# ZhangHH233/Retinal_OCT_Image_Segmentation_via_Deep_Learning

Measured on AMD Instinct MI355X. Metric: B-scans/sec (train fwd+bwd) at batch 32, 512x1024, higher is better.
Workload: dtype bf16; 1 GPU; SOTAS/Layers_Segment UNet(1,8,init_features=32) train step, 512x1024, batch 32/GPU (BASELINE configs[1]); global_batch=32, parallelism=dp1, hip_graph=False

## Files before the change

include/oct_hip.h:

```cpp
#ifndef OCT_HIP_H
#define OCT_HIP_H

#include <stddef.h>
#include <stdint.h>

#ifdef __cplusplus
extern "C" {
#endif

#define OCT_VERSION 220

#define OCT_DT_BF16 0
#define OCT_DT_F32 1

#define OCT_OK 0
#define OCT_IMG_SHIFT_ALL 2
#define OCT_E_INVALID (-22)
#define OCT_E_LAUNCH (-5)
#define OCT_E_NODEVICE (-19)

#define OCT_XF_NONE 0
#define OCT_XF_AFFINE_RELU 1
#define OCT_XF_AFFINE 2

#define OCT_IN_PLAIN 0
#define OCT_IN_S2D 1
#define OCT_OUT_PLAIN 0
#define OCT_OUT_D2S 1

#define OCT_PACK_CONV_FPROP 0
#define OCT_PACK_CONV_DGRAD 1
#define OCT_PACK_DECONV_FPROP 2
#define OCT_PACK_DECONV_DGRAD 3
#define OCT_PACK_1X1_DGRAD 4
#define OCT_PACK_1X1_FPROP 5
#define OCT_PACK_CONV3D_FPROP 6
#define OCT_PACK_CONV3D_DGRAD 7
#define OCT_PACK_DECONV3D_FPROP 8
#define OCT_PACK_DECONV3D_DGRAD 9

const char* oct_version_string(void);
int oct_version(void);
int oct_get_last_error(char* buf, size_t len);
int oct_device_count(void);

typedef struct OctConvDesc {
  int dtype;
  int n, h, w;
  int c0, c1;
  int cout;
  int taps;
  int xform0, xform1;
  int in_mode, out_mode;
  int split;
  int want_stats;
  int kh, kw;
  int depth;
  int out_img_mul, out_img_add;
} OctConvDesc;

typedef struct OctConvArgs {
  const void* x0; const void* x1;
  const float* scale0; const float* shift0;
  const float* scale1; const float* shift1;
  const void* wpacked;
  const float* bias;
  void* y0; void* y1;
  float* stat_partials;
} OctConvArgs;

int oct_conv_stat_blocks(const OctConvDesc* d);
size_t oct_packed_weight_elems(int rows, int taps, int kch);
int oct_pack_weights(int mode, int dtype, const float* w, void* wpacked, int cout, int cin, void* stream);
int oct_pack_weights_kk(int mode, int dtype, const float* w, void* wpacked, int cout, int cin, int kh, int kw,
                        void* stream);
int oct_pack_weights3d(int mode, int dtype, const float* w, void* wpacked, int cout, int cin, int kdi, void* stream);
#define OCT_PACK_BATCH_MAX 96
typedef struct OctPackJob {
  int mode, cout, cin, reserved;
  const float* w;
  void* wpacked;
} OctPackJob;
int oct_pack_weights_batch(int dtype, int count, const OctPackJob* jobs, void* stream);
int oct_conv_forward(const OctConvDesc* d, const OctConvArgs* a, void* stream);

typedef struct OctWgradDesc {
  int dtype;
  int n, h, w;
  int c0, c1;
  int cout;
  int taps;
  int xform0, xform1;
  int dy_mode;
  int kh, kw;
  int depth;
  int in_img_shift;
  int dy_img_mul, dy_img_add;
  int partials;
} OctWgradDesc;
typedef struct OctWgradArgs {
  const void* x0; const void* x1;
  const float* scale0; const float* shift0;
  const float* scale1; const float* shift1;
  const void* dy;
  float* dwp;
  float* dbias;
  const void* dy_y; const float* dy_coef; const float* dy_scale; const float* dy_shift;
  float* dbias_partials;
} OctWgradArgs;
int oct_conv_wgrad(const OctWgradDesc* d, const OctWgradArgs* a, void* stream);
int oct_conv_wgrad_partials(const OctWgradDesc* d);
int oct_reduce_bias_partials(const float* part, int nparts, int rows, int channels, float* dbias, int accumulate,
                             void* stream);
int oct_conv_wgrad_fused_apply_ok(const OctWgradDesc* d);
int oct_conv_wgrad_all_depth_taps_ok(const OctWgradDesc* d);
typedef struct OctConvBwdFusedArgs {
  const void* x;
  const float* scale; const float* shift;
  const float* mean; const float* invstd;
  const void* dy;
  const void* wpacked;
  void* dx;
  float* dwp;
  float* partials;
} OctConvBwdFusedArgs;
int oct_conv_backward_fused_ok(const OctWgradDesc* d);
int oct_conv_backward_fused_blocks(const OctWgradDesc* d);
int oct_conv_backward_fused(const OctWgradDesc* d, const OctConvBwdFusedArgs* a, void* stream);
int oct_unpack_wgrad(int mode, const float* dwp, float* grad, int cout, int cin, int accumulate, void* stream);
int oct_unpack_wgrad_kk(const float* dwp, float* grad, int cout, int cin, int kh, int kw, int accumulate, void* stream);
int oct_unpack_wgrad3d(int mode, const float* dwp, float* grad, int cout, int cin, int kdi, int accumulate, void* stream);
typedef struct OctUnpackJob {
  int mode, cout, cin, accumulate;
  int nparts, reserved;
  const float* dwp;
  float* grad;
} OctUnpackJob;
int oct_unpack_wgrad_batch(int count, const OctUnpackJob* jobs, void* stream);

int oct_bn_finalize(const float* partials, int nblocks, int c, double count,
                    const float* gamma, const float* beta, float eps, float momentum,
                    float* running_mean, float* running_var,
                    float* mean, float* invstd, float* scale, float* shift, const float* conv_bias,
                    void* stream);
int oct_bn_eval_coeffs(int c, const float* gamma, const float* beta, const float* running_mean,
                       const float* running_var, float eps, float* scale, float* shift,
                       const float* conv_bias, void* stream);

int oct_bn_relu_pool_fwd(int dtype, const void* y, const float* scale, const float* shift,
                         void* pooled, int n, int h, int w, int c, void* stream);
int oct_bn_relu_fwd(int dtype, const void* y, const float* scale, const float* shift,
                    void* out, size_t npix, int c, void* stream);

int oct_dact_bn_reduce(int dtype, const void* da, const void* dpool, const void* y,
                       const float* scale, const float* shift, const float* mean,
                       const float* invstd, void* g, float* partials, int n, int h, int w, int c,
                       void* stream);
int oct_dact_bn_reduce_blocks(int n, int h, int w, int c, int has_pool);
int oct_bn_bwd_apply_pool_ok(int dtype, int n, int h, int w, int c);
int oct_bn_bwd_apply_pool(int dtype, const void* da, const void* dpool, const void* y, const float* scale,
                          const float* shift, const float* coef, void* dy, int n, int h, int w, int c, void* stream);
int oct_bn_bwd_finalize(const float* partials, int nblocks, int c, double count,
                        const float* gamma, const float* mean, const float* invstd,
                        float* dgamma, float* dbeta, float* coef , int accumulate,
                        void* stream);
int oct_bn_bwd_apply(int dtype, void* g, const void* y, const float* coef, const float* scale,
                     const float* shift, size_t npix, int c, void* stream);
int oct_bn_bwd_apply_to(int dtype, void* dst, const void* g, const void* y, const float* coef, const float* scale,
                        const float* shift, size_t npix, int c, void* stream);
int oct_rowdot_ok(int c, int k);
int oct_rowdot_blocks(size_t npix, int c);
int oct_rowdot_fwd(int dtype, const void* x, const float* w, void* y, float* stats, size_t npix, int c, int k, void* stream);
int oct_rowdot_bwd_data(int dtype, const void* dy, const float* w, void* dx, size_t npix, int c, int k, void* stream);
int oct_rowdot_bwd_weight(int dtype, const void* dy, const void* x, float* dw, float* partials, size_t npix, int c, int k,
                          int accumulate, void* stream);
int oct_rowdot_bwd_weight_bias(int dtype, const void* dy, const void* x, float* dw, float* dbias, float* partials, size_t npix, int c,
                               int k, int accumulate, void* stream);

int oct_channel_sum(int dtype, const void* x, float* out, size_t npix, int c, int accumulate,
                    void* stream);

typedef struct OctHeadDesc {
  int dtype;
  int n, h, w;
  int feat;
  int classes;
} OctHeadDesc;
#define OCT_MAX_CLASSES 16
#define OCT_HEAD_LOSS_SLOTS (2 + 3 * OCT_MAX_CLASSES)
int oct_head_blocks(const OctHeadDesc* d);
int oct_head_forward(const OctHeadDesc* d, const void* y, const float* scale, const float* shift,
                     const float* w , const float* b, const int64_t* target,
                     float* probs, int64_t* argmax, float* logits ,
                     double* loss_partials, void* stream);
int oct_head_loss_finalize(const OctHeadDesc* d, const double* loss_partials, int nblocks,
                           float w_ce, float w_dice, float dice_eps, float* loss_out,
                           float* dice_coef, void* stream);
int oct_head_dlogits(const OctHeadDesc* d, const void* y, const float* scale, const float* shift,
                     const float* w, const float* b, const int64_t* target, const float* dice_coef,
                     float w_ce, const float* dprobs, void* dlogits, void* stream);

int oct_head_backward_fused(const OctHeadDesc* d, const void* y, const float* scale, const float* shift,
                            const float* mean, const float* invstd, const float* w, const float* b,
                            const int64_t* target, const float* dice_coef, float w_ce,
                            const float* dprobs, void* dlogits, void* da, float* partials,
                            float* dbias, float* dweight, double* loss_partials, void* stream);

#define OCT_SEG_NHWC 0
#define OCT_SEG_NCHW 1
int oct_seg_loss_blocks(size_t npix, int classes);
int oct_seg_loss_forward(const OctHeadDesc* d, int layout, const void* logits, const int64_t* target,
                         int64_t* argmax, double* loss_partials, void* stream);
int oct_seg_loss_backward(const OctHeadDesc* d, int layout, const void* logits, const int64_t* target,
                          const float* dice_coef, float w_ce, const float* dloss, void* dlogits,
                          double* loss_partials, void* stream);

int oct_seg_loss_weight_sum(const OctHeadDesc* d, const int64_t* target, const float* class_weight,
                            const float* pixel_weight, int has_ignore, int64_t ignore_index,
                            double* partials, double* wsum, void* stream);
int oct_seg_loss_forward_weighted(const OctHeadDesc* d, int layout, const void* logits,
                                  const int64_t* target, const float* class_weight,
                                  const float* pixel_weight, int has_ignore, int64_t ignore_index,
                                  double* loss_partials, void* stream);
int oct_seg_loss_backward_weighted(const OctHeadDesc* d, int layout, const void* logits,
                                   const int64_t* target, const float* class_weight,
                                   const float* pixel_weight, int has_ignore, int64_t ignore_index,
                                   const double* wsum, const float* dice_coef, float w_ce,
                                   const float* dloss, void* dlogits, double* loss_partials,
                                   void* stream);
int oct_seg_loss_finalize_weighted(const OctHeadDesc* d, const double* loss_partials, int nblocks,
                                   float w_ce, float w_dice, float dice_eps, float* loss_out,
                                   float* dice_coef, double* wsum_out, void* stream);

int oct_bce_loss_weight_sum(const OctHeadDesc* d, const uint8_t* target, const float* pixel_weight,
                            int has_ignore, int ignore_value, double* partials, double* wsum,
                            void* stream);
int oct_bce_loss_forward(const OctHeadDesc* d, int layout, const void* logits, const uint8_t* target,
                         const float* pos_weight, const float* pixel_weight, int has_ignore,
                         int ignore_value, int want_dice, float tau, uint8_t* mask,
                         double* loss_partials, void* stream);
int oct_bce_loss_backward(const OctHeadDesc* d, int layout, const void* logits, const uint8_t* target,
                          const float* pos_weight, const float* pixel_weight, int has_ignore,
                          int ignore_value, const double* wsum, const float* dice_coef, float w_bce,
                          const float* dloss, void* dlogits, double* loss_partials, void* stream);

int oct_nchw_to_nhwc(int dtype, const float* x, void* out, int n, int c, int h, int w, void* stream);
int oct_nhwc_to_nchw(int dtype, const void* x, float* out, int n, int c, int h, int w, void* stream);
int oct_sgd_step(float* p, const float* g, float* buf, size_t n, float lr, float momentum,
                 float weight_decay, float grad_scale, int first, void* stream);

int oct_adam_step(float* p, const float* g, float* m, float* v, size_t n, float lr, float beta1,
                  float beta2, float eps, float weight_decay, int decoupled, float step_size,
                  float inv_sqrt_bc2, float grad_scale, const float* dev_scale,
                  const uint8_t* decay_mask, void* stream);
int oct_sgd_step_scaled(float* p, const float* g, float* buf, size_t n, float lr, float momentum,
                        float weight_decay, float grad_scale, int first, const float* dev_scale,
                        const uint8_t* decay_mask, void* stream);
int oct_grad_norm_blocks(size_t n);
int oct_grad_norm(const float* g, size_t n, float grad_scale, float max_norm, double* partials,
                  float* out, void* stream);

#define OCT_ACT_NONE 0
#define OCT_ACT_RELU 1
#define OCT_ACT_SIGMOID 2
int oct_affine_act_fwd(int dtype, const void* y, const float* scale, const float* shift,
                       const void* res, int act, void* out, size_t npix, int c, void* stream);
int oct_affine_res_act_fwd(int dtype, const void* y, const float* scale, const float* shift, const void* res,
                           const float* res_shift, int act, void* out, size_t npix, int c, void* stream);
int oct_act_bwd(int dtype, const void* dout, const void* out, int act, void* dz, size_t n, void* stream);
int oct_maxpool_fwd(int dtype, const void* a, void* out, int n, int h, int w, int c, int k, void* stream);
int oct_maxpool_bwd(int dtype, const void* a, const void* dout, void* da, int n, int h, int w, int c,
                    int k, void* stream);
int oct_bilinear_up_fwd(int dtype, const void* x, void* out, int n, int h, int w, int c, int factor,
                        void* stream);
int oct_bilinear_up_bwd(int dtype, const void* dout, void* dx, int n, int h, int w, int c, int factor,
                        void* stream);
int oct_bilinear_resize_fwd(int dtype, const void* x, void* out, int n, int h, int w, int c, int ho, int wo,
                            void* stream);
int oct_bilinear_resize_bwd(int dtype, const void* dout, void* dx, int n, int h, int w, int c, int ho, int wo,
                            void* stream);
int oct_depth_to_space(int dtype, const void* in, const float* bias, void* out, int n, int h, int w,
                       int cout, int s, void* stream);
int oct_space_to_depth(int dtype, const void* in, void* out, int n, int h, int w, int cout, int s,
                       void* stream);
int oct_gate_fwd(int dtype, const void* x, const void* p, void* out, size_t npix, int c, void* stream);
int oct_gate_bwd(int dtype, const void* dout, const void* x, const void* p, void* dx, void* dp,
                 size_t npix, int c, void* stream);

int oct_affine_prelu_fwd(int dtype, const void* y, const float* scale, const float* shift, const float* alpha,
                         void* out, size_t npix, int c, void* stream);
int oct_affine_prelu_bwd(int dtype, const void* dout, const void* y, const float* scale, const float* shift,
                         const float* alpha, void* dz, float* dalpha, size_t npix, int c, void* stream);
int oct_prelu_bn_fused_ok(int dtype, int c);
int oct_dact_bn_reduce_prelu(int dtype, const void* da, const void* y, const float* scale, const float* shift, const float* alpha,
                             const float* mean, const float* invstd, float* partials, float* dalpha, int n, int h, int w, int c,
                             void* stream);
int oct_bn_bwd_apply_prelu_to(int dtype, void* dst, const void* da, const void* y, const float* coef, const float* scale,
                              const float* shift, const float* alpha, size_t npix, int c, void* stream);
int oct_maxpool_idx_fwd(int dtype, const void* a, void* out, int64_t* idx, int n, int h, int w, int c, int k, void* stream);
int oct_index_scatter(int dtype, const void* v, const int64_t* idx, void* out, int n, size_t npool, size_t plane, int c,
                      void* stream);
int oct_index_gather(int dtype, const void* x, const int64_t* idx, void* v, int n, size_t npool, size_t plane, int c,
                     void* stream);
int oct_maxpool_code_fwd(int dtype, const void* a, void* out, unsigned char* code, int n, int h, int w, int c, int k, void* stream);
int oct_window_scatter(int dtype, const void* v, const unsigned char* code, void* out, int n, int hp, int wp, int c, int k, void* stream);
int oct_window_gather(int dtype, const void* x, const unsigned char* code, void* v, int n, int hp, int wp, int c, int k, void* stream);

int oct_depth_pool_fwd(int dtype, const void* p2, void* out, size_t nslab, size_t m, void* stream);
int oct_depth_pool_bwd(int dtype, const void* p2, const void* dout, void* dp2, size_t nslab, size_t m, void* stream);

int oct_confusion_counts(const void* y_true, const void* y_pred, int elem, size_t n,
                         int64_t* out_i ,
                         double* out_f , void* stream);

int oct_class_confusion_counts(const void* y_true, const void* y_pred, int elem, size_t n, int classes,
                               int64_t* out , uint64_t* scratch ,
                               void* stream);

int oct_sqdiff_sum(const void* y_true, const void* y_pred, int elem, size_t n, double* out, void* stream);
int oct_column_absdiff_sum(const void* y_true, const void* y_pred, int elem, int unsigned_wrap, size_t rows,
                           size_t cols, double* out, void* stream);

#define OCT_EVAL_PRED_U8 0
#define OCT_EVAL_PRED_I64 1
#define OCT_EVAL_PRED_NHWC_BF16 2
#define OCT_EVAL_PRED_NHWC_F32 3
#define OCT_EVAL_PRED_NCHW_F32 4
#define OCT_EVAL_STATE_EXTRA 4
typedef struct {
  int images, h, w, classes;
  int target_elem;
  int pred_kind;
  int has_ignore;
  int64_t ignore_index;
} OctSegEvalDesc;
int oct_seg_eval_update(const OctSegEvalDesc* d, const void* target, const void* pred, int64_t* state, void* stream);

#ifdef __cplusplus
}
#endif
#endif
```

retinal_oct_image_segmentation_via_deep_learning_amd/_lib.py:

```python
from __future__ import annotations

import ctypes as C
import os
import subprocess
import threading

PKG_DIR = os.path.dirname(os.path.abspath(__file__))
LIB_PATH = os.environ.get("OCT_HIP_LIB") or os.path.join(PKG_DIR, "liboct_hip.so")
CSRC_DIR = os.path.join(PKG_DIR, "csrc")

DT_BF16, DT_F32 = 0, 1
XF_NONE, XF_AFFINE_RELU, XF_AFFINE = 0, 1, 2
IN_PLAIN, IN_S2D = 0, 1
IMG_SHIFT_ALL = 2
ACT_NONE, ACT_RELU, ACT_SIGMOID = 0, 1, 2
ACT_PRELU = 3
OUT_PLAIN, OUT_D2S = 0, 1
PACK_CONV_FPROP, PACK_CONV_DGRAD, PACK_DECONV_FPROP, PACK_DECONV_DGRAD, PACK_1X1_DGRAD, PACK_1X1_FPROP = range(6)
PACK_CONV3D_FPROP, PACK_CONV3D_DGRAD, PACK_DECONV3D_FPROP, PACK_DECONV3D_DGRAD = 6, 7, 8, 9
MAX_CLASSES = 16
HEAD_LOSS_SLOTS = 2 + 3 * MAX_CLASSES
SEG_NHWC, SEG_NCHW = 0, 1

c_void_p, c_int, c_size_t, c_float, c_double = C.c_void_p, C.c_int, C.c_size_t, C.c_float, C.c_double


class PackJob(C.Structure):
    _fields_ = [("mode", c_int), ("cout", c_int), ("cin", c_int), ("reserved", c_int), ("w", c_void_p),
                ("wpacked", c_void_p)]


class UnpackJob(C.Structure):
    _fields_ = [("mode", c_int), ("cout", c_int), ("cin", c_int), ("accumulate", c_int), ("nparts", c_int),
                ("reserved", c_int), ("dwp", c_void_p), ("grad", c_void_p)]


PACK_BATCH_MAX = 96


class ConvDesc(C.Structure):
    _fields_ = [(k, c_int) for k in (
        "dtype", "n", "h", "w", "c0", "c1", "cout", "taps", "xform0", "xform1", "in_mode", "out_mode",
        "split", "want_stats", "kh", "kw", "depth", "out_img_mul", "out_img_add")]


class ConvArgs(C.Structure):
    _fields_ = [(k, c_void_p) for k in (
        "x0", "x1", "scale0", "shift0", "scale1", "shift1", "wpacked", "bias", "y0", "y1", "stat_partials")]


class WgradDesc(C.Structure):
    _fields_ = [(k, c_int) for k in (
        "dtype", "n", "h", "w", "c0", "c1", "cout", "taps", "xform0", "xform1", "dy_mode", "kh", "kw", "depth",
        "in_img_shift", "dy_img_mul", "dy_img_add", "partials")]


class WgradArgs(C.Structure):
    _fields_ = [(k, c_void_p) for k in ("x0", "x1", "scale0", "shift0", "scale1", "shift1", "dy", "dwp", "dbias",
                                                "dy_y", "dy_coef", "dy_scale", "dy_shift", "dbias_partials")]


class ConvBwdFusedArgs(C.Structure):
    _fields_ = [(k, c_void_p) for k in ("x", "scale", "shift", "mean", "invstd", "dy", "wpacked", "dx", "dwp", "partials")]


class HeadDesc(C.Structure):
    _fields_ = [(k, c_int) for k in ("dtype", "n", "h", "w", "feat", "classes")]


class SegEvalDesc(C.Structure):
    _fields_ = [(k, c_int) for k in ("images", "h", "w", "classes", "target_elem", "pred_kind", "has_ignore")] + \
               [("ignore_index", C.c_int64)]


EVAL_PRED_U8, EVAL_PRED_I64, EVAL_PRED_NHWC_BF16, EVAL_PRED_NHWC_F32, EVAL_PRED_NCHW_F32 = range(5)
EVAL_STATE_EXTRA = 4


SIGNATURES = {
    "oct_version_string": (C.c_char_p, []),
    "oct_version": (c_int, []),
    "oct_get_last_error": (c_int, [C.c_char_p, c_size_t]),
    "oct_device_count": (c_int, []),
    "oct_conv_stat_blocks": (c_int, [C.POINTER(ConvDesc)]),
    "oct_packed_weight_elems": (c_size_t, [c_int, c_int, c_int]),
    "oct_pack_weights": (c_int, [c_int, c_int, c_void_p, c_void_p, c_int, c_int, c_void_p]),
    "oct_pack_weights3d": (c_int, [c_int, c_int, c_void_p, c_void_p, c_int, c_int, c_int, c_void_p]),
    "oct_unpack_wgrad3d": (c_int, [c_int, c_void_p, c_void_p, c_int, c_int, c_int, c_int, c_void_p]),
    "oct_depth_pool_fwd": (c_int, [c_int, c_void_p, c_void_p, c_size_t, c_size_t, c_void_p]),
    "oct_depth_pool_bwd": (c_int, [c_int, c_void_p, c_void_p, c_void_p, c_size_t, c_size_t, c_void_p]),
    "oct_pack_weights_kk": (c_int, [c_int, c_int, c_void_p, c_void_p, c_int, c_int, c_int, c_int, c_void_p]),
    "oct_unpack_wgrad_kk": (c_int, [c_void_p, c_void_p, c_int, c_int, c_int, c_int, c_int, c_void_p]),
    "oct_affine_prelu_fwd": (c_int, [c_int, c_void_p, c_void_p, c_void_p, c_void_p, c_void_p, c_size_t, c_int, c_void_p]),
    "oct_affine_prelu_bwd": (c_int, [c_int, c_void_p, c_void_p, c_void_p, c_void_p, c_void_p, c_void_p, c_void_p, c_size_t,
                                     c_int, c_void_p]),
    "oct_maxpool_idx_fwd": (c_int, [c_int, c_void_p, c_void_p, c_void_p, c_int, c_int, c_int, c_int, c_int, c_void_p]),
    "oct_index_scatter": (c_int, [c_int, c_void_p, c_void_p, c_void_p, c_int, c_size_t, c_size_t, c_int, c_void_p]),
    "oct_index_gather": (c_int, [c_int, c_void_p, c_void_p, c_void_p, c_int, c_size_t, c_size_t, c_int, c_void_p]),
    "oct_prelu_bn_fused_ok": (c_int, [c_int, c_int]),
    "oct_dact_bn_reduce_prelu": (c_int, [c_int, c_void_p, c_void_p, c_void_p, c_void_p, c_void_p, c_void_p, c_void_p, c_void_p, c_void_p,
                                         c_int, c_int, c_int, c_int, c_void_p]),
    "oct_bn_bwd_apply_prelu_to": (c_int, [c_int, c_void_p, c_void_p, c_void_p, c_void_p, c_void_p, c_void_p, c_void_p, c_size_t, c_int,
                                          c_void_p]),
    "oct_maxpool_code_fwd": (c_int, [c_int, c_void_p, c_void_p, c_void_p, c_int, c_int, c_int, c_int, c_int, c_void_p]),
    "oct_window_scatter": (c_int, [c_int, c_void_p, c_void_p, c_void_p, c_int, c_int, c_int, c_int, c_int, c_void_p]),
    "oct_window_gather": (c_int, [c_int, c_void_p, c_void_p, c_void_p, c_int, c_int, c_int, c_int, c_int, c_void_p]),
    "oct_pack_weights_batch": (c_int, [c_int, c_int, C.POINTER(PackJob), c_void_p]),
    "oct_conv_forward": (c_int, [C.POINTER(ConvDesc), C.POINTER(ConvArgs), c_void_p]),
    "oct_conv_wgrad": (c_int, [C.POINTER(WgradDesc), C.POINTER(WgradArgs), c_void_p]),
    "oct_conv_wgrad_fused_apply_ok": (c_int, [C.POINTER(WgradDesc)]),
    "oct_conv_wgrad_all_depth_taps_ok": (c_int, [C.POINTER(WgradDesc)]),
    "oct_conv_backward_fused_ok": (c_int, [C.POINTER(WgradDesc)]),
    "oct_conv_backward_fused_blocks": (c_int, [C.POINTER(WgradDesc)]),
    "oct_conv_backward_fused": (c_int, [C.POINTER(WgradDesc), C.POINTER(ConvBwdFusedArgs), c_void_p]),
    "oct_conv_wgrad_partials": (c_int, [C.POINTER(WgradDesc)]),
    "oct_reduce_bias_partials": (c_int, [c_void_p, c_int, c_int, c_int, c_void_p, c_int, c_void_p]),
    "oct_unpack_wgrad": (c_int, [c_int, c_void_p, c_void_p, c_int, c_int, c_int, c_void_p]),
    "oct_unpack_wgrad_batch": (c_int, [c_int, C.POINTER(UnpackJob), c_void_p]),
    "oct_bn_finalize": (c_int, [c_void_p, c_int, c_int, c_double, c_void_p, c_void_p, c_float, c_float,
                                c_void_p, c_void_p, c_void_p, c_void_p, c_void_p, c_void_p, c_void_p, c_void_p]),
    "oct_bn_eval_coeffs": (c_int, [c_int, c_void_p, c_void_p, c_void_p, c_void_p, c_float, c_void_p, c_void_p,
                                   c_void_p, c_void_p]),
    "oct_bn_relu_pool_fwd": (c_int, [c_int, c_void_p, c_void_p, c_void_p, c_void_p, c_int, c_int, c_int, c_int,
                                     c_void_p]),
    "oct_bn_relu_fwd": (c_int, [c_int, c_void_p, c_void_p, c_void_p, c_void_p, c_size_t, c_int, c_void_p]),
    "oct_dact_bn_reduce": (c_int, [c_int, c_void_p, c_void_p, c_void_p, c_void_p, c_void_p, c_void_p, c_void_p,
                                   c_void_p, c_void_p, c_int, c_int, c_int, c_int, c_void_p]),
    "oct_dact_bn_reduce_blocks": (c_int, [c_int, c_int, c_int, c_int, c_int]),
    "oct_bn_bwd_apply_pool_ok": (c_int, [c_int, c_int, c_int, c_int, c_int]),
    "oct_bn_bwd_apply_pool": (c_int, [c_int, c_void_p, c_void_p, c_void_p, c_void_p, c_void_p, c_void_p, c_void_p,
                                      c_int, c_int, c_int, c_int, c_void_p]),
    "oct_bn_bwd_finalize": (c_int, [c_void_p, c_int, c_int, c_double, c_void_p, c_void_p, c_void_p, c_void_p,
                                    c_void_p, c_void_p, c_int, c_void_p]),
    "oct_bn_bwd_apply": (c_int, [c_int, c_void_p, c_void_p, c_void_p, c_void_p, c_void_p, c_size_t, c_int,
                                 c_void_p]),
    "oct_bn_bwd_apply_to": (c_int, [c_int, c_void_p, c_void_p, c_void_p, c_void_p, c_void_p, c_void_p, c_size_t, c_int,
                                    c_void_p]),
    "oct_channel_sum": (c_int, [c_int, c_void_p, c_void_p, c_size_t, c_int, c_int, c_void_p]),
    "oct_rowdot_ok": (c_int, [c_int, c_int]),
    "oct_rowdot_blocks": (c_int, [c_size_t, c_int]),
    "oct_rowdot_fwd": (c_int, [c_int, c_void_p, c_void_p, c_void_p, c_void_p, c_size_t, c_int, c_int, c_void_p]),
    "oct_rowdot_bwd_data": (c_int, [c_int, c_void_p, c_void_p, c_void_p, c_size_t, c_int, c_int, c_void_p]),
    "oct_rowdot_bwd_weight": (c_int, [c_int, c_void_p, c_void_p, c_void_p, c_void_p, c_size_t, c_int, c_int, c_int, c_void_p]),
    "oct_rowdot_bwd_weight_bias": (c_int, [c_int, c_void_p, c_void_p, c_void_p, c_void_p, c_void_p, c_size_t, c_int, c_int, c_int,
                                           c_void_p]),
    "oct_head_blocks": (c_int, [C.POINTER(HeadDesc)]),
    "oct_head_forward": (c_int, [C.POINTER(HeadDesc), c_void_p, c_void_p, c_void_p, c_void_p, c_void_p, c_void_p,
                                 c_void_p, c_void_p, c_void_p, c_void_p, c_void_p]),
    "oct_head_loss_finalize": (c_int, [C.POINTER(HeadDesc), c_void_p, c_int, c_float, c_float, c_float, c_void_p,
                                       c_void_p, c_void_p]),
    "oct_head_dlogits": (c_int, [C.POINTER(HeadDesc), c_void_p, c_void_p, c_void_p, c_void_p, c_void_p, c_void_p,
                                 c_void_p, c_float, c_void_p, c_void_p, c_void_p]),
    "oct_head_backward_fused": (c_int, [C.POINTER(HeadDesc), c_void_p, c_void_p, c_void_p, c_void_p, c_void_p, c_void_p,
                                        c_void_p, c_void_p, c_void_p, c_float, c_void_p, c_void_p, c_void_p, c_void_p,
                                        c_void_p, c_void_p, c_void_p, c_void_p]),
    "oct_seg_loss_blocks": (c_int, [c_size_t, c_int]),
    "oct_seg_loss_forward": (c_int, [C.POINTER(HeadDesc), c_int, c_void_p, c_void_p, c_void_p, c_void_p, c_void_p]),
    "oct_seg_loss_backward": (c_int, [C.POINTER(HeadDesc), c_int, c_void_p, c_void_p, c_void_p, c_float, c_void_p, c_void_p,
                                      c_void_p, c_void_p]),
    "oct_seg_loss_weight_sum": (c_int, [C.POINTER(HeadDesc), c_void_p, c_void_p, c_void_p, c_int, C.c_int64, c_void_p, c_void_p,
                                        c_void_p]),
    "oct_seg_loss_forward_weighted": (c_int, [C.POINTER(HeadDesc), c_int, c_void_p, c_void_p, c_void_p, c_void_p, c_int,
                                              C.c_int64, c_void_p, c_void_p]),
    "oct_seg_loss_backward_weighted": (c_int, [C.POINTER(HeadDesc), c_int, c_void_p, c_void_p, c_void_p, c_void_p, c_int,
                                               C.c_int64, c_void_p, c_void_p, c_float, c_void_p, c_void_p, c_void_p, c_void_p]),
    "oct_seg_loss_finalize_weighted": (c_int, [C.POINTER(HeadDesc), c_void_p, c_int, c_float, c_float, c_float, c_void_p,
                                               c_void_p, c_void_p, c_void_p]),
    "oct_bce_loss_weight_sum": (c_int, [C.POINTER(HeadDesc), c_void_p, c_void_p, c_int, c_int, c_void_p, c_void_p, c_void_p]),
    "oct_bce_loss_forward": (c_int, [C.POINTER(HeadDesc), c_int, c_void_p, c_void_p, c_void_p, c_void_p, c_int, c_int, c_int,
                                     c_float, c_void_p, c_void_p, c_void_p]),
    "oct_bce_loss_backward": (c_int, [C.POINTER(HeadDesc), c_int, c_void_p, c_void_p, c_void_p, c_void_p, c_int, c_int,
                                      c_void_p, c_void_p, c_float, c_void_p, c_void_p, c_void_p, c_void_p]),
    "oct_nchw_to_nhwc": (c_int, [c_int, c_void_p, c_void_p, c_int, c_int, c_int, c_int, c_void_p]),
    "oct_nhwc_to_nchw": (c_int, [c_int, c_void_p, c_void_p, c_int, c_int, c_int, c_int, c_void_p]),
    "oct_sgd_step": (c_int, [c_void_p, c_void_p, c_void_p, c_size_t, c_float, c_float, c_float, c_float, c_int,
                             c_void_p]),
    "oct_adam_step": (c_int, [c_void_p, c_void_p, c_void_p, c_void_p, c_size_t, c_float, c_float, c_float, c_float, c_float,
                              c_int, c_float, c_float, c_float, c_void_p, c_void_p, c_void_p]),
    "oct_sgd_step_scaled": (c_int, [c_void_p, c_void_p, c_void_p, c_size_t, c_float, c_float, c_float, c_float, c_int,
                                    c_void_p, c_void_p, c_void_p]),
    "oct_grad_norm_blocks": (c_int, [c_size_t]),
    "oct_grad_norm": (c_int, [c_void_p, c_size_t, c_float, c_float, c_void_p, c_void_p, c_void_p]),
    "oct_affine_act_fwd": (c_int, [c_int, c_void_p, c_void_p, c_void_p, c_void_p, c_int, c_void_p, c_size_t, c_int,
                                   c_void_p]),
    "oct_affine_res_act_fwd": (c_int, [c_int, c_void_p, c_void_p, c_void_p, c_void_p, c_void_p, c_int, c_void_p, c_size_t,
                                       c_int, c_void_p]),
    "oct_act_bwd": (c_int, [c_int, c_void_p, c_void_p, c_int, c_void_p, c_size_t, c_void_p]),
    "oct_maxpool_fwd": (c_int, [c_int, c_void_p, c_void_p, c_int, c_int, c_int, c_int, c_int, c_void_p]),
    "oct_maxpool_bwd": (c_int, [c_int, c_void_p, c_void_p, c_void_p, c_int, c_int, c_int, c_int, c_int, c_void_p]),
    "oct_bilinear_up_fwd": (c_int, [c_int, c_void_p, c_void_p, c_int, c_int, c_int, c_int, c_int, c_void_p]),
    "oct_bilinear_up_bwd": (c_int, [c_int, c_void_p, c_void_p, c_int, c_int, c_int, c_int, c_int, c_void_p]),
    "oct_bilinear_resize_fwd": (c_int, [c_int, c_void_p, c_void_p, c_int, c_int, c_int, c_int, c_int, c_int, c_void_p]),
    "oct_bilinear_resize_bwd": (c_int, [c_int, c_void_p, c_void_p, c_int, c_int, c_int, c_int, c_int, c_int, c_void_p]),
    "oct_depth_to_space": (c_int, [c_int, c_void_p, c_void_p, c_void_p, c_int, c_int, c_int, c_int, c_int, c_void_p]),
    "oct_space_to_depth": (c_int, [c_int, c_void_p, c_void_p, c_int, c_int, c_int, c_int, c_int, c_void_p]),
    "oct_gate_fwd": (c_int, [c_int, c_void_p, c_void_p, c_void_p, c_size_t, c_int, c_void_p]),
    "oct_gate_bwd": (c_int, [c_int, c_void_p, c_void_p, c_void_p, c_void_p, c_void_p, c_size_t, c_int, c_void_p]),
    "oct_confusion_counts": (c_int, [c_void_p, c_void_p, c_int, c_size_t, c_void_p, c_void_p, c_void_p]),
    "oct_class_confusion_counts": (c_int, [c_void_p, c_void_p, c_int, c_size_t, c_int, c_void_p, c_void_p, c_void_p]),
    "oct_sqdiff_sum": (c_int, [c_void_p, c_void_p, c_int, c_size_t, c_void_p, c_void_p]),
    "oct_column_absdiff_sum": (c_int, [c_void_p, c_void_p, c_int, c_int, c_size_t, c_size_t, c_void_p, c_void_p]),
    "oct_seg_eval_update": (c_int, [C.POINTER(SegEvalDesc), c_void_p, c_void_p, c_void_p, c_void_p]),
}

_lib = None
_lock = threading.Lock()
param_generation = [0]


class OctError(RuntimeError):
    pass


def build(verbose: bool = False) -> str:
    cmd = ["make", "-C", CSRC_DIR, "-j8"]
    res = subprocess.run(cmd, capture_output=True, text=True)
    if verbose or res.returncode != 0:
        print(res.stdout[-4000:])
        print(res.stderr[-4000:])
    if res.returncode != 0:
        raise OctError("building liboct_hip.so failed (see output above)")
    return LIB_PATH


def lib():
    global _lib
    if _lib is not None:
        return _lib
    with _lock:
        if _lib is None:
            if not os.path.exists(LIB_PATH):
                raise OctError(
                    f"{LIB_PATH} is missing: the HIP extension has not been built "
                    "(run `python __graft_entry__.py` or `make -C .../csrc`). There is no CPU fallback.")
            handle = C.CDLL(LIB_PATH)
            for name, (res, args) in SIGNATURES.items():
                fn = getattr(handle, name)
                fn.restype = res
                fn.argtypes = args
            _lib = handle
    return _lib


def last_error() -> str:
    buf = C.create_string_buffer(512)
    lib().oct_get_last_error(buf, 512)
    return buf.value.decode("utf-8", "replace")


def check(rc: int, what: str = "") -> None:
    if rc != 0:
        raise OctError(f"{what or 'liboct_hip'} failed with code {rc}: {last_error()}")


def ptr(t) -> int | None:
    return None if t is None else t.data_ptr()
```

retinal_oct_image_segmentation_via_deep_learning_amd/csrc/common.h:

```cpp
#pragma once
#include <hip/hip_runtime.h>
#include <stdint.h>
#include <stddef.h>
#include "../../include/oct_hip.h"

typedef __bf16 bf16_t;
typedef float f32x16 __attribute__((ext_vector_type(16)));
typedef float f32x4 __attribute__((ext_vector_type(4)));
typedef __bf16 bf16x8 __attribute__((ext_vector_type(8)));
typedef __bf16 bf16x4 __attribute__((ext_vector_type(4)));

void oct_set_error(const char* fmt, ...);
#define OCT_CHECK(cond, ...)            \
  do {                                  \
    if (!(cond)) {                      \
      oct_set_error(__VA_ARGS__);       \
      return OCT_E_INVALID;             \
    }                                   \
  } while (0)
int oct_check_launch(const char* what);
int oct_lds_optin(const void* kernel, int bytes);

enum ConvPath { CONV_FIRST, CONV_ROLL3D, CONV_GEMM1, CONV_IGEMM2, CONV_IGEMM };
struct ConvPlan {
  ConvPath path;
  int kernel;
  int grid;
  int stat_rows;
  int th, nt, nblk, nitems, per_wg, interleave;
  bool wres;
};
bool first_plan(const OctConvDesc* d, ConvPlan* pl);
bool roll3d_plan(const OctConvDesc* d, ConvPlan* pl);
bool igemm2_plan(const OctConvDesc* d, ConvPlan* pl);
bool gemm1_plan(const OctConvDesc* d, ConvPlan* pl);
void igemm_plan(const OctConvDesc* d, ConvPlan* pl);
int launch_first(const ConvPlan& pl, const OctConvDesc* d, const OctConvArgs* a, hipStream_t s);
int launch_roll3d(const ConvPlan& pl, const OctConvDesc* d, const OctConvArgs* a, hipStream_t s);
int launch_igemm2(const ConvPlan& pl, const OctConvDesc* d, const OctConvArgs* a, hipStream_t s);
int launch_gemm1(const ConvPlan& pl, const OctConvDesc* d, const OctConvArgs* a, hipStream_t s);
int launch_igemm(const ConvPlan& pl, const OctConvDesc* d, const OctConvArgs* a, hipStream_t s);
bool igemm2_fused_plan(const OctWgradDesc* d, ConvPlan* pl);
int launch_igemm2_fused(const ConvPlan& pl, const OctWgradDesc* d, const OctConvBwdFusedArgs* a, hipStream_t s);

enum WgradPath { WGRAD_FIRST, WGRAD_W2, WGRAD_GENERIC };
struct WgradPlan {
  WgradPath path;
  int kernel;
  int cb, ib, th;
  int grid;
  int slabs;
  bool all_depth_taps;
};
bool first_wgrad_plan(const OctWgradDesc* d, bool dbias, bool dy_coef, WgradPlan* pl);
bool wgrad2_plan(const OctWgradDesc* d, WgradPlan* pl);
void wgrad_plan(const OctWgradDesc* d, WgradPlan* pl);
int launch_first_wgrad(const WgradPlan& pl, const OctWgradDesc* d, const OctWgradArgs* a, hipStream_t s);
int launch_wgrad2(const WgradPlan& pl, const OctWgradDesc* d, const OctWgradArgs* a, hipStream_t s);
int launch_wgrad(const WgradPlan& pl, const OctWgradDesc* d, const OctWgradArgs* a, hipStream_t s);

__device__ __forceinline__ float xf_floor(int xf) { return xf == 2 ? -__builtin_inff() : 0.f; }
__device__ __forceinline__ float to_f32(float v) { return v; }
__device__ __forceinline__ float to_f32(bf16_t v) { return (float)v; }
template <typename T> __device__ __forceinline__ T from_f32(float v);
template <> __device__ __forceinline__ float from_f32<float>(float v) { return v; }
template <> __device__ __forceinline__ bf16_t from_f32<bf16_t>(float v) { return (bf16_t)v; }

template <typename T, int V> struct alignas((sizeof(T) * V) > 16 ? 16 : (sizeof(T) * V)) VecT { T v[V]; };

template <typename T, int V>
__device__ __forceinline__ void load_vec(const T* p, float (&out)[V]) {
  VecT<T, V> t = *reinterpret_cast<const VecT<T, V>*>(p);
#pragma unroll
  for (int i = 0; i < V; ++i) out[i] = to_f32(t.v[i]);
}
template <typename T, int V>
__device__ __forceinline__ void store_vec(T* p, const float (&in)[V]) {
  VecT<T, V> t;
#pragma unroll
  for (int i = 0; i < V; ++i) t.v[i] = from_f32<T>(in[i]);
  *reinterpret_cast<VecT<T, V>*>(p) = t;
}

template <typename T, int V>
__device__ __forceinline__ void load_vec_nt(const T* p, float (&out)[V]) {
  typedef unsigned int nt_u4 __attribute__((ext_vector_type(4)));
  constexpr int NQ = (sizeof(T) * V) / 16;
  static_assert(NQ >= 1 && (sizeof(T) * V) % 16 == 0, "16-B multiples only");
  VecT<T, V> t;
  nt_u4* q = reinterpret_cast<nt_u4*>(&t);
#pragma unroll
  for (int i = 0; i < NQ; ++i) q[i] = __builtin_nontemporal_load(reinterpret_cast<const nt_u4*>(p) + i);
#pragma unroll
  for (int i = 0; i < V; ++i) out[i] = to_f32(t.v[i]);
}
template <typename T, int V>
__device__ __forceinline__ void store_vec_nt(T* p, const float (&in)[V]) {
  typedef unsigned int nt_u4 __attribute__((ext_vector_type(4)));
  constexpr int NQ = (sizeof(T) * V) / 16;
  static_assert(NQ >= 1 && (sizeof(T) * V) % 16 == 0, "16-B multiples only");
  VecT<T, V> t;
#pragma unroll
  for (int i = 0; i < V; ++i) t.v[i] = from_f32<T>(in[i]);
  const nt_u4* q = reinterpret_cast<const nt_u4*>(&t);
#pragma unroll
  for (int i = 0; i < NQ; ++i) __builtin_nontemporal_store(q[i], reinterpret_cast<nt_u4*>(p) + i);
}

template <typename T> struct Mma;
template <> struct Mma<bf16_t> {
  typedef bf16x8 Frag;
  static __device__ __forceinline__ void mma(f32x16& acc, const Frag& a, const Frag& b) {
    acc = __builtin_amdgcn_mfma_f32_32x32x16_bf16(a, b, acc, 0, 0, 0);
  }
  static __device__ __forceinline__ void mma0(f32x16& acc, const Frag& a, const Frag& b) {
    const f32x16 z = {0.f, 0.f, 0.f, 0.f, 0.f, 0.f, 0.f, 0.f, 0.f, 0.f, 0.f, 0.f, 0.f, 0.f, 0.f, 0.f};
    acc = __builtin_amdgcn_mfma_f32_32x32x16_bf16(a, b, z, 0, 0, 0);
  }
  template <int S>
  static __device__ __forceinline__ void mma16(f32x16& acc, const Frag& a, const Frag& b) {
    f32x4 v = {acc[4 * S], acc[4 * S + 1], acc[4 * S + 2], acc[4 * S + 3]};
    v = __builtin_amdgcn_mfma_f32_16x16x32_bf16(a, b, v, 0, 0, 0);
    acc[4 * S] = v[0]; acc[4 * S + 1] = v[1]; acc[4 * S + 2] = v[2]; acc[4 * S + 3] = v[3];
  }
  static __device__ __forceinline__ Frag load(const void* p) { return *reinterpret_cast<const Frag*>(p); }
  static __device__ __forceinline__ Frag zero() {
    Frag f;
#pragma unroll
    for (int i = 0; i < 8; ++i) f[i] = (bf16_t)0.0f;
    return f;
  }
  static __device__ __forceinline__ void set(Frag& f, int j, bf16_t v) { f[j] = v; }
};
struct F32Frag { f32x4 lo, hi; };
template <> struct Mma<float> {
  typedef F32Frag Frag;
  static __device__ __forceinline__ void mma(f32x16& acc, const Frag& a, const Frag& b) {
#pragma unroll
    for (int j = 0; j < 4; ++j) acc = __builtin_amdgcn_mfma_f32_32x32x2f32(a.lo[j], b.lo[j], acc, 0, 0, 0);
#pragma unroll
    for (int j = 0; j < 4; ++j) acc = __builtin_amdgcn_mfma_f32_32x32x2f32(a.hi[j], b.hi[j], acc, 0, 0, 0);
  }
  static __device__ __forceinline__ Frag load(const void* p) {
    Frag f;
    f.lo = reinterpret_cast<const f32x4*>(p)[0];
    f.hi = reinterpret_cast<const f32x4*>(p)[1];
    return f;
  }
  static __device__ __forceinline__ Frag zero() {
    Frag f;
    f.lo = f32x4{0, 0, 0, 0};
    f.hi = f32x4{0, 0, 0, 0};
    return f;
  }
  static __device__ __forceinline__ void set(Frag& f, int j, float v) {
    if (j < 4) f.lo[j] = v; else f.hi[j - 4] = v;
  }
};

typedef short s16x4 __attribute__((ext_vector_type(4)));
__device__ __forceinline__ bf16x8 tr_frag(const unsigned char* base_lo) {
  typedef __attribute__((address_space(3))) s16x4 lds_s16x4;
  const s16x4 a = __builtin_amdgcn_ds_read_tr16_b64_v4i16((lds_s16x4*)(base_lo));
  const s16x4 b = __builtin_amdgcn_ds_read_tr16_b64_v4i16((lds_s16x4*)(base_lo + 4 * 64));
  typedef short s16x8 __attribute__((ext_vector_type(8)));
  const s16x8 v = {a[0], a[1], a[2], a[3], b[0], b[1], b[2], b[3]};
  return __builtin_bit_cast(bf16x8, v);
}

__device__ __forceinline__ bf16x8 tr_frag2(const unsigned char* first, const unsigned char* second) {
  typedef __attribute__((address_space(3))) s16x4 lds_s16x4;
  const s16x4 a = __builtin_amdgcn_ds_read_tr16_b64_v4i16((lds_s16x4*)(first));
  const s16x4 b = __builtin_amdgcn_ds_read_tr16_b64_v4i16((lds_s16x4*)(second));
  typedef short s16x8 __attribute__((ext_vector_type(8)));
  const s16x8 v = {a[0], a[1], a[2], a[3], b[0], b[1], b[2], b[3]};
  return __builtin_bit_cast(bf16x8, v);
}

__device__ __forceinline__ float wave_sum(float v) {
#pragma unroll
  for (int o = 32; o > 0; o >>= 1) v += __shfl_xor(v, o);
  return v;
}
__device__ __forceinline__ double wave_sum(double v) {
#pragma unroll
  for (int o = 32; o > 0; o >>= 1) v += __shfl_xor(v, o);
  return v;
}

__device__ __forceinline__ float reduce32_scatter16(const float (&v)[16], int lane) {
  float t8[8], t4[4], t2[2];
  bool b = (lane & 16) != 0;
#pragma unroll
  for (int k = 0; k < 8; ++k) {
    float keep = b ? v[k + 8] : v[k];
    float send = b ? v[k] : v[k + 8];
    t8[k] = keep + __shfl_xor(send, 16);
  }
  b = (lane & 8) != 0;
#pragma unroll
  for (int k = 0; k < 4; ++k) {
    float keep = b ? t8[k + 4] : t8[k];
    float send = b ? t8[k] : t8[k + 4];
    t4[k] = keep + __shfl_xor(send, 8);
  }
  b = (lane & 4) != 0;
#pragma unroll
  for (int k = 0; k < 2; ++k) {
    float keep = b ? t4[k + 2] : t4[k];
    float send = b ? t4[k] : t4[k + 2];
    t2[k] = keep + __shfl_xor(send, 4);
  }
  b = (lane & 2) != 0;
  float keep = b ? t2[1] : t2[0];
  float send = b ? t2[0] : t2[1];
  float s = keep + __shfl_xor(send, 2);
  s += __shfl_xor(s, 1);
  return s;
}
__device__ __forceinline__ float reduce16_scatter8(const float (&v)[8], int lane) {
  float t4[4], t2[2];
  bool b = (lane & 8) != 0;
#pragma unroll
  for (int k = 0; k < 4; ++k) {
    float keep = b ? v[k + 4] : v[k];
    float send = b ? v[k] : v[k + 4];
    t4[k] = keep + __shfl_xor(send, 8);
  }
  b = (lane & 4) != 0;
#pragma unroll
  for (int k = 0; k < 2; ++k) {
    float keep = b ? t4[k + 2] : t4[k];
    float send = b ? t4[k] : t4[k + 2];
    t2[k] = keep + __shfl_xor(send, 4);
  }
  b = (lane & 2) != 0;
  float keep = b ? t2[1] : t2[0];
  float send = b ? t2[0] : t2[1];
  float s = keep + __shfl_xor(send, 2);
  s += __shfl_xor(s, 1);
  return s;
}
__device__ __forceinline__ int scatter16_reg_of_lane(int lane) {
  return ((lane >> 4) & 1) * 8 + ((lane >> 3) & 1) * 4 + ((lane >> 2) & 1) * 2 + ((lane >> 1) & 1);
}

static inline hipStream_t as_stream(void* s) { return reinterpret_cast<hipStream_t>(s); }
static inline int ceil_div(int a, int b) { return (a + b - 1) / b; }
```

retinal_oct_image_segmentation_via_deep_learning_amd/csrc/conv_dispatch.hip:

```cpp
#include "common.h"
#include <stdlib.h>

static bool v2_enabled() {
  static const bool on = [] { const char* e = getenv("OCT_DISABLE_V2"); return !(e && e[0] == '1'); }();
  return on;
}

static ConvPlan plan_conv_forward(const OctConvDesc* d) {
  ConvPlan pl = {};
  if (v2_enabled()) {
    if (first_plan(d, &pl) || roll3d_plan(d, &pl)) return pl;
    if (igemm2_plan(d, &pl)) {
      gemm1_plan(d, &pl);
      return pl;
    }
  }
  igemm_plan(d, &pl);
  return pl;
}

static WgradPlan plan_conv_wgrad(const OctWgradDesc* d, bool dbias, bool dy_coef) {
  WgradPlan pl = {};
  if (v2_enabled() && (first_wgrad_plan(d, dbias, dy_coef, &pl) || wgrad2_plan(d, &pl))) return pl;
  wgrad_plan(d, &pl);
  return pl;
}

static bool kernel_size(int taps, int kh_in, int kw_in, int* kh, int* kw) {
  if (kh_in == 0 && kw_in == 0) {
    if (taps == 9) { *kh = 3; *kw = 3; return true; }
    if (taps == 1) { *kh = 1; *kw = 1; return true; }
    return false;
  }
  *kh = kh_in; *kw = kw_in;
  return taps == kh_in * kw_in && ((kh_in == 3 && kw_in == 3) || (kh_in == 1 && kw_in == 1) || (kh_in == 7 && kw_in == 3));
}

extern "C" int oct_conv_stat_blocks(const OctConvDesc* d) { return d ? plan_conv_forward(d).stat_rows : 0; }

extern "C" int oct_conv_forward(const OctConvDesc* d, const OctConvArgs* a, void* stream) {
  OCT_CHECK(d && a, "oct_conv_forward: null descriptor");
  OCT_CHECK(d->dtype == OCT_DT_BF16 || d->dtype == OCT_DT_F32, "oct_conv_forward: bad dtype %d", d->dtype);
  int kh = 0, kw = 0;
  OCT_CHECK(kernel_size(d->taps, d->kh, d->kw, &kh, &kw),
            "oct_conv_forward: kernel must be 3x3 (taps 9), 1x1 (taps 1) or 7x3 (taps 21, kh=7, kw=3); got taps=%d kh=%d kw=%d",
            d->taps, d->kh, d->kw);
  OCT_CHECK(kh != 7 || (d->in_mode == OCT_IN_PLAIN && d->out_mode == OCT_OUT_PLAIN), "oct_conv_forward: 7x3 runs plain -> plain");
  OCT_CHECK(d->depth >= 0 && (d->depth == 0 || (d->n % d->depth) == 0), "oct_conv_forward: n=%d is not a whole number of depth-%d volumes", d->n, d->depth);
  OCT_CHECK(d->depth == 0 || kh != 7, "oct_conv_forward: depth taps go with the 3x3 (3x3x3) and 1x1 (2x2x2 transposed) kernels");
  OCT_CHECK(d->out_img_mul == 0 || d->out_mode == OCT_OUT_D2S, "oct_conv_forward: the output image map belongs to D2S");
  OCT_CHECK(d->n > 0 && d->h > 0 && d->w > 0 && d->c0 > 0 && d->c1 >= 0 && d->cout > 0,
            "oct_conv_forward: bad shape n=%d h=%d w=%d c0=%d c1=%d cout=%d", d->n, d->h, d->w, d->c0, d->c1, d->cout);
  OCT_CHECK(a->x0 && a->wpacked && a->y0, "oct_conv_forward: null tensor");
  OCT_CHECK(d->c1 == 0 || a->x1, "oct_conv_forward: c1 > 0 but x1 is null");
  OCT_CHECK(!(d->in_mode == OCT_IN_S2D && d->c1 != 0), "oct_conv_forward: S2D input takes one source");
  OCT_CHECK(!(d->out_mode == OCT_OUT_D2S && (d->cout & 3)), "oct_conv_forward: D2S needs cout %% 4 == 0");
  OCT_CHECK(d->split >= 0 && d->split < d->cout, "oct_conv_forward: bad split %d", d->split);
  OCT_CHECK(d->split == 0 || a->y1, "oct_conv_forward: split without y1");
  OCT_CHECK(d->xform0 >= 0 && d->xform0 <= OCT_XF_AFFINE && d->xform1 >= 0 && d->xform1 <= OCT_XF_AFFINE, "oct_conv_forward: bad xform");
  OCT_CHECK(!(d->xform0 && (!a->scale0 || !a->shift0)), "oct_conv_forward: xform0 without scale/shift");
  OCT_CHECK(!(d->xform1 && (!a->scale1 || !a->shift1)), "oct_conv_forward: xform1 without scale/shift");
  OCT_CHECK(!(d->want_stats && !a->stat_partials), "oct_conv_forward: want_stats without buffer");
  OCT_CHECK((size_t)d->n * d->h * d->w < (1u << 31), "oct_conv_forward: too many pixels");
  const ConvPlan pl = plan_conv_forward(d);
  hipStream_t s = as_stream(stream);
  switch (pl.path) {
    case CONV_FIRST: return launch_first(pl, d, a, s);
    case CONV_ROLL3D: return launch_roll3d(pl, d, a, s);
    case CONV_GEMM1: return launch_gemm1(pl, d, a, s);
    case CONV_IGEMM2: return launch_igemm2(pl, d, a, s);
    default: return launch_igemm(pl, d, a, s);
  }
}

extern "C" int oct_conv_wgrad_partials(const OctWgradDesc* d) {
  int kh, kw;
  if (!d || !kernel_size(d->taps, d->kh, d->kw, &kh, &kw)) return 0;
  return plan_conv_wgrad(d, false, false).slabs;
}

extern "C" int oct_conv_wgrad_fused_apply_ok(const OctWgradDesc* d) {
  return d && d->kh != 7 && plan_conv_wgrad(d, false, false).path == WGRAD_FIRST;
}

extern "C" int oct_conv_wgrad_all_depth_taps_ok(const OctWgradDesc* d) {
  if (!d) return 0;
  const WgradPlan pl = plan_conv_wgrad(d, false, false);
  return pl.path == WGRAD_FIRST && pl.all_depth_taps;
}

extern "C" int oct_conv_wgrad(const OctWgradDesc* d, const OctWgradArgs* a, void* stream) {
  OCT_CHECK(d && a, "oct_conv_wgrad: null descriptor");
  OCT_CHECK(d->dtype == OCT_DT_BF16 || d->dtype == OCT_DT_F32, "oct_conv_wgrad: bad dtype %d", d->dtype);
  int kh = 0, kw = 0;
  OCT_CHECK(kernel_size(d->taps, d->kh, d->kw, &kh, &kw),
            "oct_conv_wgrad: kernel must be 3x3 (taps 9), 1x1 (taps 1) or 7x3 (taps 21, kh=7, kw=3); got taps=%d kh=%d kw=%d",
            d->taps, d->kh, d->kw);
  OCT_CHECK(kh != 7 || (d->dy_mode == OCT_IN_PLAIN && !a->dy_coef), "oct_conv_wgrad: 7x3 takes a plain dY");
  OCT_CHECK(d->depth >= 0 && (d->depth == 0 || ((d->n % d->depth) == 0 && kh != 7)), "oct_conv_wgrad: bad depth %d for n=%d", d->depth, d->n);
  OCT_CHECK(((d->in_img_shift >= -1 && d->in_img_shift <= 1) || d->in_img_shift == OCT_IMG_SHIFT_ALL) && (d->in_img_shift == 0 || d->depth > 0),
            "oct_conv_wgrad: in_img_shift needs depth > 0");
  OCT_CHECK(d->in_img_shift != OCT_IMG_SHIFT_ALL || oct_conv_wgrad_all_depth_taps_ok(d),
            "oct_conv_wgrad: OCT_IMG_SHIFT_ALL is not available for this descriptor (oct_conv_wgrad_all_depth_taps_ok)");
  OCT_CHECK(d->dy_img_mul == 0 || d->dy_mode == OCT_IN_S2D, "oct_conv_wgrad: the dY image map belongs to S2D");
  OCT_CHECK(d->n > 0 && d->h > 0 && d->w > 0 && d->c0 > 0 && d->c1 >= 0 && d->cout > 0, "oct_conv_wgrad: bad shape");
  OCT_CHECK(a->x0 && a->dy && a->dwp, "oct_conv_wgrad: null tensor");
  OCT_CHECK(d->c1 == 0 || a->x1, "oct_conv_wgrad: c1 > 0 but x1 is null");
  OCT_CHECK(!(d->dy_mode == OCT_IN_S2D && (d->cout & 3)), "oct_conv_wgrad: S2D dy needs cout %% 4 == 0");
  OCT_CHECK(d->xform0 >= 0 && d->xform0 <= OCT_XF_AFFINE && d->xform1 >= 0 && d->xform1 <= OCT_XF_AFFINE, "oct_conv_wgrad: bad xform");
  OCT_CHECK(!(d->xform0 && (!a->scale0 || !a->shift0)), "oct_conv_wgrad: xform0 without scale/shift");
  OCT_CHECK(!(d->xform1 && (!a->scale1 || !a->shift1)), "oct_conv_wgrad: xform1 without scale/shift");
  OCT_CHECK(!d->partials || !a->dbias || a->dbias_partials, "oct_conv_wgrad: partials mode with a bias gradient needs dbias_partials");
  const WgradPlan pl = plan_conv_wgrad(d, a->dbias != nullptr, a->dy_coef != nullptr);
  OCT_CHECK(!a->dy_coef || pl.path == WGRAD_FIRST, "oct_conv_wgrad: the fused BN-backward apply is only implemented for the 1->F first layer in bf16");
  OCT_CHECK(!a->dy_coef || (a->dy_y && a->dy_scale && a->dy_shift), "oct_conv_wgrad: fused apply needs y, scale, shift");
  if (d->partials) {
    const int slabs = plan_conv_wgrad(d, false, false).slabs;
    OCT_CHECK(pl.slabs == slabs, "oct_conv_wgrad: with these arguments the launch writes %d partial slabs, oct_conv_wgrad_partials "
              "answered %d (first layer with a bias gradient?)", pl.slabs, slabs);
  }
  hipStream_t s = as_stream(stream);
  switch (pl.path) {
    case WGRAD_FIRST: return launch_first_wgrad(pl, d, a, s);
    case WGRAD_W2: return launch_wgrad2(pl, d, a, s);
    default: return launch_wgrad(pl, d, a, s);
  }
}

static bool plan_conv_backward_fused(const OctWgradDesc* d, ConvPlan* pl) {
  return d && v2_enabled() && igemm2_fused_plan(d, pl);
}

extern "C" int oct_conv_backward_fused_ok(const OctWgradDesc* d) {
  ConvPlan pl;
  return plan_conv_backward_fused(d, &pl) ? 1 : 0;
}

extern "C" int oct_conv_backward_fused_blocks(const OctWgradDesc* d) {
  ConvPlan pl;
  return plan_conv_backward_fused(d, &pl) ? pl.stat_rows : 0;
}

extern "C" int oct_conv_backward_fused(const OctWgradDesc* d, const OctConvBwdFusedArgs* a, void* stream) {
  OCT_CHECK(d && a, "oct_conv_backward_fused: null descriptor");
  ConvPlan pl;
  OCT_CHECK(plan_conv_backward_fused(d, &pl),
            "oct_conv_backward_fused: not available for this descriptor (oct_conv_backward_fused_ok): bf16, 2-D, 3x3, c0 = cout = 32, "
            "c1 = 0, BN + ReLU on load, w %% 32 == 0, h %% 8 == 0, atomics mode");
  OCT_CHECK(a->x && a->scale && a->shift && a->mean && a->invstd && a->dy && a->wpacked && a->dx && a->dwp && a->partials,
            "oct_conv_backward_fused: null tensor");
  return launch_igemm2_fused(pl, d, a, as_stream(stream));
}
```

retinal_oct_image_segmentation_via_deep_learning_amd/csrc/igemm2.hip:

```cpp
#include "common.h"
#include <stdlib.h>

struct Igemm2Params {
  const bf16_t* x0; const bf16_t* x1;
  const float* sc0; const float* sh0; const float* sc1; const float* sh1;
  const bf16_t* wp;
  bf16_t* y0; bf16_t* y1; float* stats; const float* bias;
  int n, h, w, c0, c1, cout, split, xf0, xf1, in_mode, out_mode;
  int tiles_x, tiles_y, nblk, nitems, per_wg, nch, nk16;
  int interleave;
  int depth, nchc, oimg_mul, oimg_add;
  const bf16_t* fx; const float* fsc; const float* fsh; const float* fmean; const float* finvstd;
  float* dwp; float* bnpart;
  unsigned long long* trace;
};

typedef unsigned int u32x4 __attribute__((ext_vector_type(4)));

#ifdef OCT_TRACE
#define TRACE(slot, idx)                                                                              \
  do {                                                                                                \
    if (p.trace && blockIdx.x == 0 && (threadIdx.x & 63) == 0 && (idx) < 256)                          \
      p.trace[(slot) * 256 + (idx)] = __builtin_amdgcn_s_memtime();                                    \
  } while (0)
static unsigned long long* g_trace = nullptr;
extern "C" void oct_debug_set_trace(void* buf) { g_trace = (unsigned long long*)buf; }
#else
#define TRACE(slot, idx) do {} while (0)
#endif

__device__ __forceinline__ unsigned pack_bf16x2(float a, float b) {
  typedef __bf16 bf16x2 __attribute__((ext_vector_type(2)));
  bf16x2 v;
  v[0] = (bf16_t)a;
  v[1] = (bf16_t)b;
  return __builtin_bit_cast(unsigned, v);
}
__device__ __forceinline__ float bf16lo(unsigned u) { return __uint_as_float(u << 16); }
__device__ __forceinline__ float bf16hi(unsigned u) { return __uint_as_float(u & 0xffff0000u); }

template <int TAPS, int NF, bool WRES> constexpr bool ig2_m16() { return TAPS != 1 && !WRES && NF == 2; }
template <int TAPS, int NF, bool WRES, bool DMA> constexpr int ig2_pixb() { return DMA ? 64 : (ig2_m16<TAPS, NF, WRES>() ? 96 : 80); }

__device__ __attribute__((aligned(16))) unsigned int g_zero16[4];

template <int TAPS, int WM, int WN, int MF, int NF, bool WRES, bool STATS, bool RAGGED = false, bool D3 = false, bool DMA = false,
          bool WLDS = false, bool FUSE = false>
__global__ void __launch_bounds__(512) igemm2_kernel(const Igemm2Params p) {
  static_assert(WM * WN == 4, "four MFMA waves");
  static_assert(!FUSE || (TAPS == 9 && WM == 4 && NF == 1 && WRES && !STATS && !RAGGED && !D3 && !DMA && !WLDS),
                "fused backward: resident weights, 32 -> 32 channels, whole tiles, 2-D");
  static_assert(!DMA || (!WRES && !STATS && !RAGGED && !D3), "DMA staging: streamed weights, whole tiles, 2-D, no BatchNorm sums");
  static_assert(!WLDS || (TAPS == 9 && !WRES && !D3 && !DMA && WN * NF == 1), "LDS-resident weights: 3x3, one 32-channel block");
  constexpr int TH = WM * MF, TW = 32;
  constexpr int HALO = (TAPS != 1) ? 1 : 0;
  constexpr int HALO_Y = (TAPS == 21) ? 3 : HALO;
  constexpr int LH = TH + 2 * HALO_Y, LW = TW + 2 * HALO;
  constexpr int NPIX = LH * LW;
  constexpr int NSLOT = (NPIX + 63) / 64;
  constexpr int PIXB = ig2_pixb<TAPS, NF, WRES, DMA>();
  constexpr int BUFB = DMA ? NSLOT * 4096 : NPIX * PIXB;
  constexpr int NBUF = DMA ? (TAPS != 1 ? 3 : 6) : 2;
  constexpr int NT = WN * NF * 32;
  constexpr int KSTEPS = TAPS * 2;
  constexpr bool M16 = ig2_m16<TAPS, NF, WRES>();
  typedef Mma<bf16_t> M;
  typedef M::Frag Frag;

  extern __shared__ __attribute__((aligned(16))) unsigned char smem[];
  unsigned char* const buf0 = smem;
  float* const wg_stats = reinterpret_cast<float*>(smem + NBUF * BUFB);

  const int tid = threadIdx.x, lane = tid & 63;
  const int wave = __builtin_amdgcn_readfirstlane(tid >> 6);
  const bool s2d = TAPS == 1 && p.in_mode == OCT_IN_S2D;
  const bool d2s = TAPS == 1 && p.out_mode == OCT_OUT_D2S;
  int t_first, nbi_first, nitems_wg, tstep;
  if (p.interleave) {
    if ((int)blockIdx.x >= p.nitems / p.nblk) return;
    t_first = blockIdx.x; nbi_first = 0; tstep = gridDim.x;
    nitems_wg = ((p.nitems / p.nblk - (int)blockIdx.x + (int)gridDim.x - 1) / (int)gridDim.x) * p.nblk;
  } else {
    const int it0 = blockIdx.x * p.per_wg;
    const int it1 = min(it0 + p.per_wg, p.nitems);
    if (it0 >= it1) return;
    t_first = it0 / p.nblk; nbi_first = it0 - t_first * p.nblk; tstep = 1; nitems_wg = it1 - it0;
  }
  const int sx = tstep % p.tiles_x, sy = (tstep / p.tiles_x) % p.tiles_y, simg = tstep / (p.tiles_x * p.tiles_y);
  const int nstage = nitems_wg * p.nch;
  const int nstage_pad = (nstage + 3) / 4 * 4;

  constexpr int SXF_N = WLDS ? 64 : 1024, OSCR_SLOTS = WLDS ? 1 : 2, SBIAS_N = WLDS ? 0 : 1024, WLDS_BYTES = WLDS ? 2 * 18 * 1024 : 0;
  float* const sxf = reinterpret_cast<float*>(smem + NBUF * BUFB) + (2 * WM * 2 * NT + 4);
  unsigned char* const oscr = smem + NBUF * BUFB + (2 * WM * 2 * NT + 4) * 4 + 2 * SXF_N * 4;
  static_assert((NBUF * BUFB + (2 * WM * 2 * NT + 4) * 4) % 16 == 0, "scratch must stay 16-B aligned");
  unsigned char* const wlds = oscr + OSCR_SLOTS * 4 * 32 * 80;
  float* const sbias = reinterpret_cast<float*>(wlds + WLDS_BYTES);
  float* const wgacc = sbias + SBIAS_N;
  constexpr int XTB = TH * TW * 64;
  unsigned char* const fxt = reinterpret_cast<unsigned char*>(sbias + SBIAS_N);
  unsigned char* const fxr = fxt + 2 * XTB;
  if (STATS && !WRES) {
    for (int i = tid; i < 2 * p.cout; i += 512) wgacc[i] = 0.f;
  }
  {
    const int kx = s2d ? p.c0 : p.c0 + p.c1;
    for (int i = tid; i < kx; i += 512) {
      const bool first = i < p.c0;
      const bool xf = first ? (p.xf0 != 0) : (p.xf1 != 0);
      sxf[i] = xf ? (first ? p.sc0[i] : p.sc1[i - p.c0]) : 1.f;
      sxf[kx + i] = xf ? (first ? p.sh0[i] : p.sh1[i - p.c0]) : 0.f;
    }
    if (d2s && p.bias)
      for (int i = tid; i < (p.cout >> 2); i += 512) sbias[i] = p.bias[i];
    if constexpr (FUSE) {
      if (tid < 32) *reinterpret_cast<f32x4*>(sxf + SXF_N + 4 * tid) = f32x4{p.fsc[tid], p.fsh[tid], p.fmean[tid], p.finvstd[tid]};
    }
    if constexpr (WLDS) {
      const u32x4* src = reinterpret_cast<const u32x4*>(p.wp);
      u32x4* dst = reinterpret_cast<u32x4*>(wlds);
      for (int i = tid; i < TAPS * p.nk16 * 64; i += 512) dst[i] = src[i];
    }
  }
  __syncthreads();

  if constexpr (DMA) {
   if (wave >= 4) {
    const int ptid = tid - 256, grp = ptid & 3, pbase = ptid >> 2;
    constexpr int KSH = M16 ? 1 : 2;
    const unsigned cs2 = 2u * (unsigned)p.c0;
    unsigned goff[NSLOT], code[NSLOT];
#pragma unroll
    for (int i = 0; i < NSLOT; ++i) {
      const int pix = pbase + 64 * i;
      const int ly = pix / LW, lx = pix - ly * LW;
      const int relp = s2d ? (2 * ly) * (2 * p.w) + 2 * lx : ly * p.w + lx;
      goff[i] = (unsigned)relp * cs2 + (unsigned)((grp ^ ((lx >> KSH) & 3)) * 16);
      unsigned c = pix >= NPIX ? 16u : 0u;
      if (HALO) c |= (ly < HALO_Y ? 1u : 0u) | (lx == 0 ? 4u : 0u) | (ly >= LH - HALO_Y ? 2u : 0u) | (lx == LW - 1 ? 8u : 0u);
      code[i] = c;
    }
    const int last = nstage - 1;
    int i_sidx = 0, i_ch = 0, i_nbi, i_txi, i_tyi, i_img;
    {
      int t = t_first;
      i_nbi = nbi_first;
      i_txi = t % p.tiles_x; t /= p.tiles_x;
      i_tyi = t % p.tiles_y; i_img = t / p.tiles_y;
    }
    typedef __attribute__((address_space(3))) void lds_void;
    typedef const __attribute__((address_space(1))) void gl_void;
    const unsigned char* const zsrc = reinterpret_cast<const unsigned char*>(g_zero16);
    const int pw = wave - 4;
    auto dma = [&](unsigned char* buf) {
      const int ch = i_ch, txi = i_txi, tyi = i_tyi, img = i_img;
      if (i_sidx < last) {
        ++i_sidx;
        if (++i_ch == p.nch) {
          i_ch = 0;
          if (++i_nbi == p.nblk) {
            i_nbi = 0;
            i_txi += sx; if (i_txi >= p.tiles_x) { i_txi -= p.tiles_x; ++i_tyi; }
            i_tyi += sy; if (i_tyi >= p.tiles_y) { i_tyi -= p.tiles_y; ++i_img; }
            i_img += simg;
          }
        }
      }
      const unsigned edge = 16u | (tyi == 0 ? 1u : 0u) | (tyi == p.tiles_y - 1 ? 2u : 0u) | (txi == 0 ? 4u : 0u) |
                            (txi == p.tiles_x - 1 ? 8u : 0u);
      const bf16_t* base;
      if (s2d) {
        const int dydx = (ch * 32) / p.c0;
        const int cc = ch * 32 - dydx * p.c0;
        const size_t o2 = ((size_t)img * (2 * p.h) + 2 * tyi * TH + (dydx >> 1)) * (size_t)(2 * p.w) + 2 * txi * TW + (dydx & 1);
        base = p.x0 + o2 * p.c0 + cc;
      } else {
        base = p.x0 + (((size_t)img * p.h + tyi * TH) * p.w + txi * TW) * p.c0 + ch * 32;
      }
      const unsigned char* const hb = reinterpret_cast<const unsigned char*>(base) - (size_t)(HALO_Y * p.w + HALO) * cs2;
      unsigned char* const dst = buf + pw * 1024;
#pragma unroll
      for (int i = 0; i < NSLOT; ++i) {
        const bool ok = (code[i] & edge) == 0;
        const unsigned char* src = ok ? hb + goff[i] : zsrc;
        __builtin_amdgcn_global_load_lds((gl_void*)src, (lds_void*)(dst + i * 4096), 16, 0, 0);
        constexpr int DMA_SLEEP = 6;
        if (TAPS != 1 && i + 1 < NSLOT) __builtin_amdgcn_s_sleep(NF == 2 ? DMA_SLEEP : DMA_SLEEP / 3);
      }
    };
    constexpr int NW = NSLOT * (NBUF - 2);
    static_assert(NW < 64, "vmcnt is a 6-bit counter");
    auto stage_barrier = [&]() {
      __builtin_amdgcn_s_waitcnt((NW & 15) | ((NW >> 4) << 14) | (7 << 4) | (15 << 8));
      asm volatile("s_barrier" ::: "memory");
    };
    int wb = 0;
#pragma unroll
    for (int j = 0; j < NBUF - 1; ++j) { dma(buf0 + wb * BUFB); wb = wb + 1 == NBUF ? 0 : wb + 1; }
    stage_barrier();
    for (int s0 = 0; s0 < nstage_pad; ++s0) {
      dma(buf0 + wb * BUFB); wb = wb + 1 == NBUF ? 0 : wb + 1;
      stage_barrier();
    }
    return;
   }
  } else
  if (wave >= 4) {
    const int ptid = tid - 256, grp = ptid & 3, pbase = ptid >> 2;
    constexpr int D = 2;
    u32x4 R[D][NSLOT];
    unsigned vmask[D];
    int relp[NSLOT];
    unsigned code[NSLOT];
#pragma unroll
    for (int i = 0; i < NSLOT; ++i) {
      const int pix = pbase + 64 * i;
      const int ly = pix / LW, lx = pix - ly * LW;
      relp[i] = s2d ? (2 * ly) * (2 * p.w) + 2 * lx : ly * p.w + lx;
      const int ylast = p.h - (p.tiles_y - 1) * TH + HALO_Y, xlast = p.w - (p.tiles_x - 1) * TW + HALO;
      unsigned c = pix >= NPIX ? 16u : 0u;
      if (HALO) c |= (ly < HALO_Y ? 1u : 0u) | (lx == 0 ? 4u : 0u);
      c |= (ly >= ylast ? 2u : 0u) | (lx >= xlast ? 8u : 0u);
      code[i] = c;
    }
    constexpr int XS = FUSE ? TH * TW * 4 / 256 : 1;
    u32x4 XR[D][XS];
    unsigned xrel[XS];
    float fs[8], fb[8];
    const unsigned char* x_next = nullptr;
    if constexpr (FUSE) {
#pragma unroll
      for (int i = 0; i < XS; ++i) {
        const int pix = pbase + 64 * i;
        xrel[i] = (unsigned)((pix >> 5) * p.w + (pix & 31)) * 64u;
      }
#pragma unroll
      for (int j = 0; j < 8; ++j) { fs[j] = p.fsc[grp * 8 + j]; fb[j] = p.fsh[grp * 8 + j]; }
      asm volatile("s_waitcnt vmcnt(0)" ::: "memory");
#pragma unroll
      for (int j = 0; j < 8; ++j) asm volatile("" : "+v"(fs[j]), "+v"(fb[j]));
    }
    const int last = nstage - 1;
    int i_sidx = 0, i_ch = 0, i_nbi, i_txi, i_tyi, i_img, c_sidx = 0, c_ch = 0;
    {
      int t = t_first;
      i_nbi = nbi_first;
      i_txi = t % p.tiles_x; t /= p.tiles_x;
      i_tyi = t % p.tiles_y; i_img = t / p.tiles_y;
    }
    struct IssueSt { const unsigned char* hb; unsigned edge, cs2, safe; bool zok; };
    auto issue_begin = [&]() -> IssueSt {
      const int ch = i_ch, txi = i_txi, tyi = i_tyi, img = i_img;
      if (i_sidx < last) {
        ++i_sidx;
        if (++i_ch == p.nch) {
          i_ch = 0;
          if (++i_nbi == p.nblk) {
            i_nbi = 0;
            i_txi += sx; if (i_txi >= p.tiles_x) { i_txi -= p.tiles_x; ++i_tyi; }
            i_tyi += sy; if (i_tyi >= p.tiles_y) { i_tyi -= p.tiles_y; ++i_img; }
            i_img += simg;
          }
        }
      }
      const unsigned edge = 16u | (tyi == 0 ? 1u : 0u) | (tyi == p.tiles_y - 1 ? 2u : 0u) | (txi == 0 ? 4u : 0u) |
                            (txi == p.tiles_x - 1 ? 8u : 0u);
      int chc = ch, srcimg = img;
      bool zok = true;
      if (D3 && !s2d) {
        const int kdi = ch / p.nchc;
        chc = ch - kdi * p.nchc;
        const int dz = img % p.depth + kdi - 1;
        zok = dz >= 0 && dz < p.depth;
        srcimg = zok ? img + kdi - 1 : img;
      }
      const size_t origin = ((size_t)srcimg * p.h + tyi * TH) * p.w + txi * TW;
      if constexpr (FUSE) x_next = reinterpret_cast<const unsigned char*>(p.fx + origin * 32 + grp * 8);
      const bool second = !s2d && chc * 32 >= p.c0;
      const int cs = second ? p.c1 : p.c0;
      const bf16_t* base;
      if (s2d) {
        int dydx = (ch * 32) / p.c0;
        const int cc = ch * 32 - dydx * p.c0;
        int img2 = img;
        if (D3) { img2 = 2 * img + (dydx >> 2); dydx &= 3; }
        const size_t o2 = ((size_t)img2 * (2 * p.h) + 2 * tyi * TH + (dydx >> 1)) * (size_t)(2 * p.w) + 2 * txi * TW + (dydx & 1);
        base = p.x0 + o2 * p.c0 + cc + grp * 8;
      } else {
        base = (second ? p.x1 + origin * p.c1 + (chc * 32 - p.c0) : p.x0 + origin * p.c0 + chc * 32) + grp * 8;
      }
      const unsigned cs2 = 2u * (unsigned)cs, safe = (unsigned)(HALO_Y * p.w + HALO) * cs2;
      const unsigned char* const hb = reinterpret_cast<const unsigned char*>(base) - safe;
      return IssueSt{hb, edge, cs2, safe, zok};
    };
    auto issue_slot = [&](const IssueSt& st, int i, u32x4& r, unsigned& vm) {
      const bool ok = (!D3 || st.zok) && (code[i] & st.edge) == 0;
      r = *reinterpret_cast<const u32x4*>(st.hb + (ok ? __umul24((unsigned)relp[i], st.cs2) : st.safe));
      vm |= ok ? (1u << i) : 0u;
    };
    auto issue = [&](u32x4 (&Rr)[NSLOT], unsigned& vm) {
      const IssueSt st = issue_begin();
      vm = 0;
#pragma unroll
      for (int i = 0; i < NSLOT; ++i) issue_slot(st, i, Rr[i], vm);
    };
    struct CommitSt { float s[8], b[8]; float flo; bool xf; };
    auto commit_begin = [&](bool always) -> CommitSt {
      CommitSt st;
      const int ch = c_ch;
      if (c_sidx < last) { ++c_sidx; if (++c_ch == p.nch) c_ch = 0; }
      const int chc = (D3 && !s2d) ? ch % p.nchc : ch;
      int cg = chc * 32 + grp * 8;
      if (s2d) cg -= ((ch * 32) / p.c0) * p.c0;
      const bool first = s2d || chc * 32 < p.c0;
      st.xf = first ? (p.xf0 != 0) : (p.xf1 != 0);
      st.flo = xf_floor(first ? p.xf0 : p.xf1);
      if (st.xf || always) {
        const int kx = s2d ? p.c0 : p.c0 + p.c1;
        const f32x4 s0 = *reinterpret_cast<const f32x4*>(sxf + cg), s1 = *reinterpret_cast<const f32x4*>(sxf + cg + 4);
        const f32x4 b0 = *reinterpret_cast<const f32x4*>(sxf + kx + cg), b1 = *reinterpret_cast<const f32x4*>(sxf + kx + cg + 4);
#pragma unroll
        for (int j = 0; j < 4; ++j) { st.s[j] = s0[j]; st.s[4 + j] = s1[j]; st.b[j] = b0[j]; st.b[4 + j] = b1[j]; }
      }
      return st;
    };
    auto commit_slot = [&](const CommitSt& st, unsigned char* buf, int i, const u32x4& r, unsigned vm, bool always) {
      const int pix = pbase + 64 * i;
      if (pix < NPIX) {
        u32x4 v = r;
#ifndef ABL_NO_XFORM
        if (always || st.xf)
#else
        if (st.xf && p.n == 12345)
#endif
        {
#pragma unroll
          for (int j = 0; j < 4; ++j) {
            const float lo = fmaxf(fmaf(bf16lo(v[j]), st.s[2 * j], st.b[2 * j]), st.flo);
            const float hi = fmaxf(fmaf(bf16hi(v[j]), st.s[2 * j + 1], st.b[2 * j + 1]), st.flo);
            v[j] = pack_bf16x2(lo, hi);
          }
        }
        const bool live = (vm & (1u << i)) != 0;
#pragma unroll
        for (int j = 0; j < 4; ++j) v[j] = live ? v[j] : 0u;
        *reinterpret_cast<u32x4*>(buf + pix * PIXB + grp * 16) = v;
      }
    };
    auto commit = [&](unsigned char* buf, const u32x4 (&Rr)[NSLOT], unsigned vm) {
      const CommitSt st = commit_begin(false);
#pragma unroll
      for (int i = 0; i < NSLOT; ++i) commit_slot(st, buf, i, Rr[i], vm, false);
    };
    auto issue_x = [&](u32x4 (&Xr)[XS]) {
#pragma unroll
      for (int i = 0; i < XS; ++i) Xr[i] = *reinterpret_cast<const u32x4*>(x_next + xrel[i]);
    };
    auto commit_x = [&](int bi, const u32x4 (&Xr)[XS]) {
#pragma unroll
      for (int i = 0; i < XS; ++i) {
        const int off = bi * XTB + (pbase + 64 * i) * 64 + grp * 16;
        u32x4 v = Xr[i];
        *reinterpret_cast<u32x4*>(fxr + off) = v;
#pragma unroll
        for (int j = 0; j < 4; ++j) {
          const float lo = fmaxf(fmaf(bf16lo(v[j]), fs[2 * j], fb[2 * j]), 0.f);
          const float hi = fmaxf(fmaf(bf16hi(v[j]), fs[2 * j + 1], fb[2 * j + 1]), 0.f);
          v[j] = pack_bf16x2(lo, hi);
        }
        *reinterpret_cast<u32x4*>(fxt + off) = v;
      }
    };
    f32x16 dwa[FUSE ? 3 : 1];
    const int pw = wave - 4;
    int f_trx = 0, f_trd = 0;
    if constexpr (FUSE) {
#pragma unroll
      for (int j = 0; j < 3; ++j)
#pragma unroll
        for (int i = 0; i < 16; ++i) dwa[j][i] = 0.f;
      const int g4 = lane >> 4, li = lane & 15;
      f_trx = (8 * (g4 >> 1) + (li >> 2)) * 64 + (16 * (g4 & 1) + 4 * (li & 3)) * 2;
      f_trd = (8 * (g4 >> 1) + (li >> 2)) * PIXB + (16 * (g4 & 1) + 4 * (li & 3)) * 2 + (pw < 3 ? (2 - pw) * LW * PIXB : 0);
    }
    auto dw_stage = [&](int bi) __attribute__((always_inline)) {
      const unsigned char* const xt = fxt + bi * XTB + f_trx;
      const unsigned char* const dt = buf0 + bi * BUFB + f_trd;
      constexpr int NKW = TH * 2;
      auto xfrag = [&](int k) { return tr_frag(xt + ((k >> 1) * TW + (k & 1) * 16) * 64); };
      auto dfrag = [&](int k, int j) {
        const unsigned char* const a = dt + ((k >> 1) * LW + (k & 1) * 16 + (2 - j)) * PIXB;
        return tr_frag2(a, a + 4 * PIXB);
      };
      Frag xq[2], dq[2][3];
      xq[0] = xfrag(0);
#pragma unroll
      for (int j = 0; j < 3; ++j) dq[0][j] = dfrag(0, j);
#pragma unroll
      for (int k = 0; k < NKW; ++k) {
        if (k + 1 < NKW) {
          xq[(k + 1) & 1] = xfrag(k + 1);
#pragma unroll
          for (int j = 0; j < 3; ++j) dq[(k + 1) & 1][j] = dfrag(k + 1, j);
        }
        __builtin_amdgcn_sched_barrier(0);
#pragma unroll
        for (int j = 0; j < 3; ++j) M::mma(dwa[j], dq[k & 1][j], xq[k & 1]);
        __builtin_amdgcn_sched_barrier(0);
      }
    };
#pragma unroll
    for (int j = 0; j < D; ++j) {
      issue(R[j], vmask[j]);
      if constexpr (FUSE) issue_x(XR[j]);
    }
    commit(buf0, R[0], vmask[0]);
    if constexpr (FUSE) commit_x(0, XR[0]);
    issue(R[0], vmask[0]);
    if constexpr (FUSE) issue_x(XR[0]);
    __syncthreads();
    const bool spread = TAPS != 1 && !D3 && !WRES && p.xf0 != 0 && (p.c1 == 0 || p.xf1 != 0);
    if (spread) {
      for (int s0 = 0; s0 < nstage_pad; s0 += D) {
#pragma unroll
        for (int j = 0; j < D; ++j) {
          const int nx = s0 + j + 1;
          if (wave == 4) TRACE(4, nx - 1);
          unsigned char* const buf = buf0 + (nx & 1) * BUFB;
          const CommitSt cst = commit_begin(true);
          const IssueSt ist = issue_begin();
          const unsigned vold = vmask[(j + 1) % D];
          unsigned vnew = 0;
#pragma unroll
          for (int i = 0; i < NSLOT; ++i) {
            commit_slot(cst, buf, i, R[(j + 1) % D][i], vold, true);
            __builtin_amdgcn_sched_barrier(0);
            issue_slot(ist, i, R[(j + 1) % D][i], vnew);
            __builtin_amdgcn_sched_barrier(0);
          }
          vmask[(j + 1) % D] = vnew;
          if (wave == 4) TRACE(6, nx - 1);
          __syncthreads();
          if (wave == 4) TRACE(7, nx - 1);
        }
      }
    } else
    for (int s0 = 0; s0 < nstage_pad; s0 += D) {
#pragma unroll
      for (int j = 0; j < D; ++j) {
        const int nx = s0 + j + 1;
        if (wave == 4) TRACE(4, nx - 1);
        commit(buf0 + (nx & 1) * BUFB, R[(j + 1) % D], vmask[(j + 1) % D]);
        if constexpr (FUSE) commit_x(nx & 1, XR[(j + 1) % D]);
        if (wave == 4) TRACE(5, nx - 1);
        issue(R[(j + 1) % D], vmask[(j + 1) % D]);
        if constexpr (FUSE) {
          issue_x(XR[(j + 1) % D]);
          if (pw < 3 && nx - 1 < nstage) dw_stage((nx - 1) & 1);
        }
        if (wave == 4) TRACE(6, nx - 1);
        __syncthreads();
        if (wave == 4) TRACE(7, nx - 1);
      }
    }
    if constexpr (FUSE) {
      if (pw < 3) {
        const int r = lane & 31, hh = lane >> 5;
#pragma unroll
        for (int j = 0; j < 3; ++j)
#pragma unroll
          for (int i = 0; i < 16; ++i) {
            const int co = (i & 3) + 8 * (i >> 2) + 4 * hh;
            atomicAdd(&p.dwp[((3 * pw + j) * 32 + co) * 32 + r], dwa[j][i]);
          }
      }
    }
    if (STATS || FUSE) __syncthreads();
    return;
  }

  __builtin_amdgcn_s_setprio(3);
  const int r = lane & 31, hh = lane >> 5;
  const int wm = wave / WN, wn = wave % WN;

  float bs1[FUSE ? 8 : 1], bs2[FUSE ? 8 : 1];
  if constexpr (FUSE) {
#pragma unroll
    for (int j = 0; j < 8; ++j) { bs1[j] = 0.f; bs2[j] = 0.f; }
  }
  Frag wres[WRES ? KSTEPS : 1][NF];
  if (WRES) {
#pragma unroll
    for (int s = 0; s < KSTEPS; ++s)
#pragma unroll
      for (int q = 0; q < NF; ++q) {
        const int nb = wn * NF + q;
        const int tap = s >> 1, k16 = s & 1;
        wres[s][q] = M::load(p.wp + ((size_t)(nb * TAPS + tap) * p.nk16 + k16) * 512 + lane * 8);
      }
    asm volatile("s_waitcnt vmcnt(0)" ::: "memory");
#pragma unroll
    for (int s = 0; s < KSTEPS; ++s)
#pragma unroll
      for (int q = 0; q < NF; ++q) asm volatile("" : "+v"(wres[s][q]));
  }

  constexpr int PF4 = 9, PF8 = 3;
  constexpr int PF = (KSTEPS == 2) ? 2 : ((MF * NF >= 8) ? PF8 : ((MF * NF >= 4) ? (TAPS == 21 ? 7 : PF4) : 9));
  static_assert(KSTEPS % PF == 0, "ring slots must line up across stages");
  Frag wring[(WRES || M16) ? 1 : PF][NF];
  constexpr bool WR3 = M16 && !RAGGED;
  constexpr int NWS = WR3 ? 3 : 2;
  Frag a16[M16 ? NWS : 1][M16 ? 2 * NF : 1];
  f32x16 acc[MF][NF];
  float s1[STATS ? NF : 1][16], s2[STATS ? NF : 1][16];
  if (STATS) {
#pragma unroll
    for (int q = 0; q < NF; ++q)
#pragma unroll
      for (int i = 0; i < 16; ++i) { s1[q][i] = 0.f; s2[q][i] = 0.f; }
  }

#ifdef OCT_TRACE
  if (p.trace && blockIdx.x == 0 && wave == 0) {
    f32x16 cacc[2];
    for (int i = 0; i < 16; ++i) { cacc[0][i] = 0.f; cacc[1][i] = 0.f; }
    Frag ca = M::load(p.wp + lane * 8), cb = M::load(p.wp + 512 + lane * 8);
    asm volatile("s_waitcnt vmcnt(0)" ::: "memory");
    const unsigned long long t0 = __builtin_amdgcn_s_memtime(), r0 = __builtin_amdgcn_s_memrealtime();
#pragma unroll
    for (int i = 0; i < 64; ++i) M::mma(cacc[i & 1], ca, cb);
    asm volatile("s_nop 15\n s_nop 15" ::: "memory");
    float sink = 0.f;
    for (int i = 0; i < 16; ++i) sink += cacc[0][i] + cacc[1][i];
    const unsigned long long t1 = __builtin_amdgcn_s_memtime(), r1 = __builtin_amdgcn_s_memrealtime();
    if (lane == 0) { p.trace[2040] = t1 - t0; p.trace[2041] = r1 - r0; p.trace[2042] = (unsigned long long)(sink != 12345.f); p.trace[2043] = r0; }
  }
#endif
  constexpr bool DEFER = !WRES && NF == 1 && !M16;
  constexpr int NFR = MF * NF;
  constexpr int ESTRIDE = (KSTEPS - 2) / NFR > 0 ? (KSTEPS - 2) / NFR : 1;
  constexpr int EHANDLED = ((KSTEPS - 1 + ESTRIDE - 1) / ESTRIDE) < NFR ? ((KSTEPS - 1 + ESTRIDE - 1) / ESTRIDE) : NFR;
  unsigned packed[DEFER ? MF : 1][DEFER ? NF : 1][8];
  bool pend = false;
  int e_tyi = 0, e_txi = 0;
  unsigned char* e_fb[NF];
  unsigned e_rowb[NF], e_pstep[NF];
#pragma unroll
  for (int q = 0; q < NF; ++q) { e_fb[q] = nullptr; e_rowb[q] = 0; e_pstep[q] = 0; }
  auto set_item = [&](int img, int tyi, int txi, int nbi) {
    e_tyi = tyi; e_txi = txi;
    const int oy0 = tyi * TH + wm * MF;
#pragma unroll
    for (int q = 0; q < NF; ++q) {
      const int cb0 = (nbi * (NT / 32) + wn * NF + q) * 32;
      bf16_t* dst; int cd, co, dydx = 0;
      if (d2s) { cd = p.cout >> 2; dydx = cb0 / cd; co = cb0 - dydx * cd; dst = p.y0; }
      else if (p.split > 0 && cb0 >= p.split) { dst = p.y1; cd = p.cout - p.split; co = cb0 - p.split; }
      else { dst = p.y0; cd = p.split > 0 ? p.split : p.cout; co = cb0; }
      const int oimg = (D3 && d2s) ? img * p.oimg_mul + p.oimg_add : img;
      const size_t pix0 = d2s ? ((size_t)oimg * (2 * p.h) + 2 * oy0 + (dydx >> 1)) * (size_t)(2 * p.w) + 2 * (txi * TW) + (dydx & 1)
                              : ((size_t)img * p.h + oy0) * p.w + txi * TW;
      e_fb[q] = reinterpret_cast<unsigned char*>(dst + pix0 * cd + co);
      e_rowb[q] = (d2s ? 8u : 2u) * (unsigned)p.w * (unsigned)cd;
      e_pstep[q] = (d2s ? 4u : 2u) * (unsigned)cd;
    }
  };
  typedef unsigned int u32x2 __attribute__((ext_vector_type(2)));
  auto frag_to_lds = [&](const unsigned (&pk)[8], int slot = 0) {
    unsigned char* sc = oscr + (slot * 4 + wave) * (32 * 80);
#pragma unroll
    for (int g = 0; g < 4; ++g) {
      const u32x2 v = {pk[2 * g], pk[2 * g + 1]};
      if (M16)
        *reinterpret_cast<u32x2*>(sc + (16 * (g >> 1) + (lane & 15)) * 80 + (16 * (g & 1) + 4 * (lane >> 4)) * 2) = v;
      else
        *reinterpret_cast<u32x2*>(sc + r * 80 + (8 * g + 4 * hh) * 2) = v;
    }
  };
  auto frag_from_lds = [&](u32x4 (&tv)[2], int slot = 0) {
    const unsigned char* sc = oscr + (slot * 4 + wave) * (32 * 80);
#pragma unroll
    for (int k = 0; k < 2; ++k) {
      const int chunk = lane + 64 * k;
      tv[k] = *reinterpret_cast<const u32x4*>(sc + (chunk >> 2) * 80 + (chunk & 3) * 16);
    }
  };
  auto frag_store = [&](int m, int q, const u32x4 (&tv)[2]) {
    if (RAGGED && e_tyi * TH + wm * MF + m >= p.h) return;
    const int wlim = (RAGGED && (e_txi + 1) * TW > p.w) ? p.w - e_txi * TW : TW;
    unsigned char* const fb = e_fb[q] + (size_t)m * e_rowb[q];
    const unsigned pstep = e_pstep[q];
#pragma unroll
    for (int k = 0; k < 2; ++k) {
      const int chunk = lane + 64 * k;
      const int px = chunk >> 2, part = chunk & 3;
      if (RAGGED && px >= wlim) continue;
#ifndef ABL_NO_STORE
      *reinterpret_cast<u32x4*>(fb + (__umul24((unsigned)px, pstep) + (unsigned)part * 16u)) = tv[k];
#else
      if (tv[k][0] == 0x12345678u && tv[k][1] == 0x9abcdef0u) *reinterpret_cast<u32x4*>(fb + (__umul24((unsigned)px, pstep) + (unsigned)part * 16u)) = tv[k];
#endif
    }
  };
  auto store_frag = [&](int m, int q) {
    u32x4 tv[2];
    frag_to_lds(packed[DEFER ? m : 0][DEFER ? q : 0]);
    frag_from_lds(tv);
    frag_store(m, q, tv);
  };

  __syncthreads();
  int cur = 0, pending_tile = -1, pending_nbi = 0, parity = 0;
  int item = 0, ch = 0;
  int tile_c = t_first, nbi_c = nbi_first;
  int txi_c = tile_c % p.tiles_x, tyi_c = (tile_c / p.tiles_x) % p.tiles_y, img_c = tile_c / (p.tiles_x * p.tiles_y);
  for (int sidx = 0; sidx < nstage_pad; ++sidx) {
    if (sidx >= nstage) { __syncthreads(); continue; }
    if (STATS && !WRES && pending_tile >= 0) {
      const float* ws = wg_stats + (parity ^ 1) * (WM * 2 * NT);
      for (int i = tid; i < 2 * NT; i += 256) {
        const int st = i / NT, cl = i - st * NT;
        float s = 0.f;
#pragma unroll
        for (int w_ = 0; w_ < WM; ++w_) s += ws[(w_ * 2 + st) * NT + cl];
        wgacc[st * p.cout + pending_nbi * NT + cl] += s;
      }
      pending_tile = -1;
    }

    const int tile = tile_c, nbi = nbi_c;
    if constexpr (WRES) {
      static_assert(!WRES || NF == 1, "resident-weight kernels hold one channel fragment per wave");
      if (wave == 0) TRACE(0, sidx);
      set_item(img_c, tyi_c, txi_c, nbi);
      const bool rag = RAGGED && STATS && ((tyi_c + 1) * TH > p.h || (txi_c + 1) * TW > p.w);
      const bool col_in = !RAGGED || (txi_c * TW + r) < p.w;
      const unsigned char* lb = buf0 + cur * BUFB + ((wm * MF) * LW + r) * PIXB + 8 * hh * 2;
      auto xoff = [](int s, int m) constexpr {
        const int tap = s >> 1, k16 = s & 1;
        return ((m + tap / 3) * LW + tap % 3) * PIXB + k16 * 32;
      };
      unsigned pk[8];
      u32x4 tv[2];
      u32x4 rv[FUSE ? 2 : 1];
      f32x4 co[FUSE ? 4 : 1];
      auto epi = [&](int mp, int s) __attribute__((always_inline)) {
        if (s == 1) {
          if (RAGGED && STATS) {
            const bool in = !rag || (col_in && (tyi_c * TH + wm * MF + mp) < p.h);
#pragma unroll
            for (int i = 0; i < 16; ++i) acc[mp][0][i] = in ? acc[mp][0][i] : 0.f;
          }
#pragma unroll
          for (int g = 0; g < 4; ++g) {
            pk[2 * g] = pack_bf16x2(acc[mp][0][4 * g], acc[mp][0][4 * g + 1]);
            pk[2 * g + 1] = pack_bf16x2(acc[mp][0][4 * g + 2], acc[mp][0][4 * g + 3]);
          }
          frag_to_lds(pk);
        }
        if (STATS && s >= 2 && s < 6) {
#pragma unroll
          for (int i = 4 * (s - 2); i < 4 * (s - 2) + 4; ++i) {
            s1[0][i] += acc[mp][0][i];
            s2[0][i] = fmaf(acc[mp][0][i], acc[mp][0][i], s2[0][i]);
            asm volatile("" : "+v"(s1[0][i]), "+v"(s2[0][i]));
          }
        }
        if (s == 6) frag_from_lds(tv);
        if constexpr (FUSE) {
          if (s == 6) {
            const unsigned char* const rt = fxr + cur * XTB + (wm * MF + mp) * (TW * 64) + lane * 16;
            rv[0] = *reinterpret_cast<const u32x4*>(rt);
            rv[1] = *reinterpret_cast<const u32x4*>(rt + 64 * 16);
          }
          if (s == 7 || s == 9) {
            const float* const ct = sxf + SXF_N + 4 * (8 * (lane & 3) + (s == 7 ? 0 : 4));
#pragma unroll
            for (int j = 0; j < 4; ++j) co[j] = *reinterpret_cast<const f32x4*>(ct + 4 * j);
          }
          if (s == 8 || s == 11) {
#pragma unroll
            for (int k = 0; k < 2; ++k)
#pragma unroll
              for (int e2 = 0; e2 < 2; ++e2) {
                const int e = (s == 8 ? 0 : 2) + e2;
                const f32x4 c0 = co[2 * e2], c1 = co[2 * e2 + 1];
                const float y0 = bf16lo(rv[k][e]), y1 = bf16hi(rv[k][e]);
                const float g0 = fmaf(y0, c0[0], c0[1]) > 0.f ? bf16lo(tv[k][e]) : 0.f;
                const float g1 = fmaf(y1, c1[0], c1[1]) > 0.f ? bf16hi(tv[k][e]) : 0.f;
                bs1[2 * e] += g0;
                bs1[2 * e + 1] += g1;
                bs2[2 * e] = fmaf(g0, (y0 - c0[2]) * c0[3], bs2[2 * e]);
                bs2[2 * e + 1] = fmaf(g1, (y1 - c1[2]) * c1[3], bs2[2 * e + 1]);
              }
          }
        }
        if (s == 10) frag_store(mp, 0, tv);
      };
      constexpr int LD = 2, KT = MF * KSTEPS;
      Frag xr[LD + 1];
#pragma unroll
      for (int k = 0; k < LD; ++k) xr[k] = M::load(lb + xoff(k % KSTEPS, k / KSTEPS));
#pragma unroll
      for (int m = 0; m < MF; ++m)
#pragma unroll
      for (int s = 0; s < KSTEPS; ++s) {
        const int k = m * KSTEPS + s;
        if (k + LD < KT) xr[(k + LD) % (LD + 1)] = M::load(lb + xoff((k + LD) % KSTEPS, (k + LD) / KSTEPS));
        __builtin_amdgcn_sched_barrier(0);
        if (s == 0) M::mma0(acc[m][0], wres[0][0], xr[k % (LD + 1)]);
        else M::mma(acc[m][0], wres[s][0], xr[k % (LD + 1)]);
        if (m > 0) epi(m - 1, s);
        __builtin_amdgcn_sched_barrier(0);
      }
      if (wave == 0) TRACE(1, sidx);
#pragma unroll
      for (int s = 1; s <= 11; ++s) epi(MF - 1, s);
    } else {
    if (ch == 0) {
#pragma unroll
      for (int m = 0; m < MF; ++m)
#pragma unroll
        for (int q = 0; q < NF; ++q)
#pragma unroll
          for (int i = 0; i < 16; ++i) acc[m][q][i] = 0.f;
    }

    if (wave == 0) TRACE(0, sidx);
    {
      const unsigned char* tb = buf0 + cur * BUFB;
      const bf16_t* wbase = nullptr; const bf16_t* wbase_n = nullptr;
      const bf16_t* wuni = nullptr; const bf16_t* wuni_n = nullptr;
      const size_t qstride = (size_t)TAPS * p.nk16 * 512, tstride = (size_t)p.nk16 * 512;
      if (!WRES) {
        const int nb0 = nbi * (NT / 32) + wn * NF;
        const bf16_t* const wsrc = WLDS ? reinterpret_cast<const bf16_t*>(wlds) : p.wp;
        wbase = wsrc + ((size_t)nb0 * TAPS * p.nk16 + ch * 2) * 512 + lane * 8;
        if constexpr (M16 && !STATS) wuni = p.wp + ((size_t)nb0 * TAPS * p.nk16 + ch * 2) * 512;
        int n_ch = ch + 1, n_item = item;
        if (n_ch == p.nch) { n_ch = 0; n_item = item + 1; }
        if (n_item >= nitems_wg) { n_item = item; n_ch = ch; }
        const int n_nbi = n_item == item ? nbi : (nbi + 1 == p.nblk ? 0 : nbi + 1);
        wbase_n = wsrc + ((size_t)(n_nbi * (NT / 32) + wn * NF) * TAPS * p.nk16 + n_ch * 2) * 512 + lane * 8;
        if constexpr (M16 && !STATS) wuni_n = p.wp + ((size_t)(n_nbi * (NT / 32) + wn * NF) * TAPS * p.nk16 + n_ch * 2) * 512;
        if (sidx == 0 && !M16) {
#pragma unroll
          for (int j = 0; j < PF; ++j)
#pragma unroll
            for (int q = 0; q < NF; ++q) wring[j][q] = M::load(wbase + q * qstride + (j >> 1) * tstride + (j & 1) * 512);
        }
      }
      const unsigned char* lb = tb + ((wm * MF) * LW + r) * PIXB + 8 * hh * 2;
      auto xoff = [](int s, int m) constexpr {
        const int tap = s >> 1, k16 = s & 1;
        const int ty = (TAPS != 1) ? tap / 3 : 0, tx = (TAPS != 1) ? tap % 3 : 0;
        return ((m + ty) * LW + tx) * PIXB + k16 * 32;
      };
      constexpr int NTX = (TAPS != 1) ? 3 : 1;
      unsigned lbs[DMA ? NTX : 1][2];
      if constexpr (DMA && !M16) {
#pragma unroll
        for (int tx = 0; tx < NTX; ++tx)
#pragma unroll
          for (int k16 = 0; k16 < 2; ++k16) {
            const int col = r + tx;
            lbs[tx][k16] = (unsigned)(cur * BUFB + ((wm * MF) * LW + col) * 64 + (((2 * k16 + hh) ^ ((col >> 2) & 3)) * 16));
          }
      }
      auto xptr = [&](int s, int m) -> const unsigned char* {
        if constexpr (DMA) {
          const int tap = s >> 1, k16 = s & 1;
          const int ty = (TAPS != 1) ? tap / 3 : 0, tx = (TAPS != 1) ? tap % 3 : 0;
          return smem + (lbs[tx][k16] + (unsigned)((m + ty) * LW * 64));
        } else return lb + xoff(s, m);
      };
      if constexpr (M16) {
        const int r16 = lane & 15, kg = lane >> 4;
        const unsigned char* lb16 = tb + ((wm * MF) * LW + r16) * PIXB + kg * 16;
        auto boff = [](int u, int m) constexpr { const int t = u >> 1; return ((m + t / 3) * LW + t % 3 + 16 * (u & 1)) * PIXB; };
        unsigned lbs16[DMA ? 3 : 1];
        if constexpr (DMA) {
#pragma unroll
          for (int tx = 0; tx < 3; ++tx) {
            const int col = r16 + tx;
            lbs16[tx] = (unsigned)(cur * BUFB + ((wm * MF) * LW + col) * 64 + ((kg ^ ((col >> 1) & 3)) * 16));
          }
        }
        auto bptr = [&](int u, int m) -> const unsigned char* {
          if constexpr (DMA) { const int t = u >> 1; return smem + (lbs16[t % 3] + (unsigned)(((m + t / 3) * LW + 16 * (u & 1)) * 64)); }
          else return lb16 + boff(u, m);
        };
        const unsigned wlane = (unsigned)(((kg >> 1) * 512 + ((kg & 1) * 32 + r16) * 8) * 2);
        const unsigned char* const wu = reinterpret_cast<const unsigned char*>(wuni);
        const unsigned char* const wun = reinterpret_cast<const unsigned char*>(wuni_n);
        constexpr bool WSB = !STATS;
        const int lpart = (kg >> 1) * 512 + ((kg & 1) * 32 + r16) * 8 - lane * 8;
        auto aoff = [&](int c) { return (size_t)(c >> 1) * qstride + (c & 1) * 128 + lpart; };
        auto wfrag = [&](bool next, int c, int tt) {
          if constexpr (WSB) {
            const size_t off = ((size_t)(c >> 1) * qstride + (size_t)tt * tstride) * 2 + (c & 1) * 256;
            return M::load((next ? wun : wu) + off + (size_t)wlane);
          } else {
            const bf16_t* wb = next ? wbase_n : wbase;
            return M::load(wb + aoff(c) + tt * tstride);
          }
        };
        if (sidx == 0) {
#pragma unroll
          for (int c = 0; c < 2 * NF; ++c) a16[0][c] = wfrag(false, c, 0);
          if constexpr (WR3) {
#pragma unroll
            for (int c = 0; c < 2 * NF; ++c) a16[1][c] = wfrag(false, c, 1);
          }
        } else if constexpr (!WR3) {
#pragma unroll
          for (int c = 0; c < 2 * NF; ++c) a16[0][c] = a16[1][c];
        }
        Frag b16[2][MF];
#pragma unroll
        for (int m = 0; m < MF; ++m) b16[0][m] = M::load(bptr(0, m));
#pragma unroll
        for (int s = 0; s < KSTEPS; ++s) {
          const int t = s >> 1;
          if (s + 1 < KSTEPS) {
#pragma unroll
            for (int m = 0; m < MF; ++m) b16[(s + 1) & 1][m] = M::load(bptr(s + 1, m));
          }
#ifndef ABL_NO_WLOAD
          if ((s & 1) == 0) {
            const int t2 = t + (WR3 ? 2 : 1);
            const int tt = t2 < TAPS ? t2 : t2 - TAPS;
#pragma unroll
            for (int c = 0; c < 2 * NF; ++c) a16[WR3 ? t2 % 3 : (t2 & 1)][c] = wfrag(t2 >= TAPS, c, tt);
          }
#endif
          __builtin_amdgcn_sched_barrier(0);
#pragma unroll
          for (int m = 0; m < MF; ++m)
#pragma unroll
            for (int c = 0; c < 2 * NF; ++c) {
              const Frag& wf = a16[WR3 ? t % 3 : (t & 1)][c];
              if (s & 1) { if (c & 1) M::template mma16<3>(acc[m][c >> 1], wf, b16[s & 1][m]); else M::template mma16<2>(acc[m][c >> 1], wf, b16[s & 1][m]); }
              else { if (c & 1) M::template mma16<1>(acc[m][c >> 1], wf, b16[s & 1][m]); else M::template mma16<0>(acc[m][c >> 1], wf, b16[s & 1][m]); }
            }
        }
      } else {
      constexpr int LD = (MF * NF >= 8) ? 1 : ((MF * NF >= 4) ? 2 : 3);
      Frag xr[LD + 1][MF];
#pragma unroll
      for (int j = 0; j < LD; ++j)
#pragma unroll
        for (int m = 0; m < MF; ++m) xr[j][m] = M::load(xptr(j, m));
#pragma unroll
      for (int s = 0; s < KSTEPS; ++s) {
        if (s + LD < KSTEPS) {
#pragma unroll
          for (int m = 0; m < MF; ++m) xr[(s + LD) % (LD + 1)][m] = M::load(xptr(s + LD, m));
        }
        __builtin_amdgcn_sched_barrier(0);
#pragma unroll
        for (int m = 0; m < MF; ++m)
#pragma unroll
          for (int q = 0; q < NF; ++q)
            M::mma(acc[m][q], WRES ? wres[s][q] : wring[s % PF][q], xr[s % (LD + 1)][m]);
#ifndef ABL_NO_WLOAD
        if (!WRES) {
          const int s2 = s + PF;
          const bf16_t* wb = s2 < KSTEPS ? wbase : wbase_n;
          const int s3 = s2 < KSTEPS ? s2 : s2 - KSTEPS;
#pragma unroll
          for (int q = 0; q < NF; ++q)
            wring[s % PF][q] = M::load(wb + q * qstride + (s3 >> 1) * tstride + (s3 & 1) * 512);
        }
#endif
        if (DEFER && s >= 1 && (s - 1) % ESTRIDE == 0 && (s - 1) / ESTRIDE < NFR) {
          if (pend) store_frag(((s - 1) / ESTRIDE) / NF, ((s - 1) / ESTRIDE) % NF);
        }
      }
      if (DEFER && pend) {
#pragma unroll
        for (int idx = EHANDLED; idx < NFR; ++idx) store_frag(idx / NF, idx % NF);
        pend = false;
      }
      }
    }

    if (wave == 0) TRACE(1, sidx);
    if (ch == p.nch - 1) {
      const int txi = txi_c, tyi = tyi_c, img = img_c;
      if (RAGGED && STATS && ((tyi + 1) * TH > p.h || (txi + 1) * TW > p.w)) {
        const bool col_in = (txi * TW + r) < p.w;
        const bool col_in0 = (txi * TW + (lane & 15)) < p.w, col_in1 = (txi * TW + 16 + (lane & 15)) < p.w;
#pragma unroll
        for (int m = 0; m < MF; ++m) {
          const bool rin = (tyi * TH + wm * MF + m) < p.h;
#pragma unroll
          for (int q = 0; q < NF; ++q)
#pragma unroll
            for (int i = 0; i < 16; ++i) {
              const bool in = rin && (M16 ? (i < 8 ? col_in0 : col_in1) : col_in);
              acc[m][q][i] = in ? acc[m][q][i] : 0.f;
            }
        }
      }
      if (!DEFER) set_item(img, tyi, txi, nbi);
      auto stats_to_ws = [&](int q) {
        float* ws = wg_stats + parity * (WM * 2 * NT);
        {
          if constexpr (M16) {
            float v1[8], v2[8];
#pragma unroll
            for (int k = 0; k < 8; ++k) { v1[k] = s1[q][k] + s1[q][8 + k]; v2[k] = s2[q][k] + s2[q][8 + k]; }
            const float t1 = reduce16_scatter8(v1, lane);
            const float t2 = reduce16_scatter8(v2, lane);
            if ((lane & 1) == 0) {
              const int reg = ((lane >> 3) & 1) * 4 + ((lane >> 2) & 1) * 2 + ((lane >> 1) & 1);
              const int cl = (wn * NF + q) * 32 + 16 * (reg >> 2) + 4 * (lane >> 4) + (reg & 3);
              ws[(wm * 2 + 0) * NT + cl] = t1;
              ws[(wm * 2 + 1) * NT + cl] = t2;
            }
          } else {
          const float t1 = reduce32_scatter16(s1[q], lane);
          const float t2 = reduce32_scatter16(s2[q], lane);
          if ((lane & 1) == 0) {
            const int reg = scatter16_reg_of_lane(lane);
            const int cl = (wn * NF + q) * 32 + (reg & 3) + 8 * (reg >> 2) + 4 * hh;
            ws[(wm * 2 + 0) * NT + cl] = t1;
            ws[(wm * 2 + 1) * NT + cl] = t2;
          }
          }
#pragma unroll
          for (int i = 0; i < 16; ++i) { s1[q][i] = 0.f; s2[q][i] = 0.f; }
        }
      };
      constexpr bool MRG = M16 && !DEFER && NF == 2 && TAPS != 1 && !RAGGED;
      constexpr bool mrg_done = MRG;
      if constexpr (MRG) {
        {
          constexpr int P2 = 144;
          unsigned char* const sc2 = oscr + wave * (32 * P2);
          static_assert(32 * P2 <= OSCR_SLOTS * 32 * 80, "the merged tile fits the wave's scratch");
          u32x4 tv4[4];
          int pm2 = -1;
          auto store4 = [&](int mm) {
            if (RAGGED && e_tyi * TH + wm * MF + mm >= p.h) return;
            const int wlim = (RAGGED && (e_txi + 1) * TW > p.w) ? p.w - e_txi * TW : TW;
            unsigned char* const fb = e_fb[0] + (size_t)mm * e_rowb[0];
#pragma unroll
            for (int k = 0; k < 4; ++k) {
              const int chunk = lane + 64 * k, px = chunk >> 3, part = chunk & 7;
              if (RAGGED && px >= wlim) continue;
              *reinterpret_cast<u32x4*>(fb + (__umul24((unsigned)px, e_pstep[0]) + (unsigned)part * 16u)) = tv4[k];
            }
          };
          if (STATS) {
            typedef float f32x2 __attribute__((ext_vector_type(2)));
#pragma unroll
            for (int q = 0; q < NF; ++q) {
#pragma unroll
              for (int m = 0; m < MF; ++m)
#pragma unroll
                for (int i = 0; i < 16; i += 2) {
                  const f32x2 av = {acc[m][q][i], acc[m][q][i + 1]};
                  f32x2 sv = {s1[q][i], s1[q][i + 1]}, tv = {s2[q][i], s2[q][i + 1]};
                  sv += av;
                  tv = __builtin_elementwise_fma(av, av, tv);
                  s1[q][i] = sv[0]; s1[q][i + 1] = sv[1]; s2[q][i] = tv[0]; s2[q][i + 1] = tv[1];
                }
              if (!WRES) stats_to_ws(q);
            }
          }
#pragma unroll
          for (int m = 0; m < MF; ++m) {
#pragma unroll
            for (int q = 0; q < NF; ++q) {
              unsigned pk[8];
#pragma unroll
              for (int g = 0; g < 4; ++g) {
                pk[2 * g] = pack_bf16x2(acc[m][q][4 * g], acc[m][q][4 * g + 1]);
                pk[2 * g + 1] = pack_bf16x2(acc[m][q][4 * g + 2], acc[m][q][4 * g + 3]);
              }
#pragma unroll
              for (int g = 0; g < 4; ++g) {
                const u32x2 v = {pk[2 * g], pk[2 * g + 1]};
                *reinterpret_cast<u32x2*>(sc2 + (16 * (g >> 1) + (lane & 15)) * P2 + q * 64 + (16 * (g & 1) + 4 * (lane >> 4)) * 2) = v;
              }
            }
            if (pm2 >= 0) store4(pm2);
#pragma unroll
            for (int k = 0; k < 4; ++k) {
              const int chunk = lane + 64 * k;
              tv4[k] = *reinterpret_cast<const u32x4*>(sc2 + (chunk >> 3) * P2 + (chunk & 7) * 16);
            }
            pm2 = m;
          }
          store4(pm2);
        }
      }
      u32x4 tvp[2];
      int pm_ = -1, pq_ = 0, fidx = 0;
      if constexpr (!mrg_done)
#pragma unroll
      for (int q = 0; q < NF; ++q) {
        const bool has_bias = d2s && p.bias != nullptr;
        float bv[16];
        if (has_bias) {
          const int cb0 = (nbi * (NT / 32) + wn * NF + q) * 32;
          const int co = cb0 % (p.cout >> 2);
#pragma unroll
          for (int g = 0; g < 4; ++g) {
            const f32x4 b4 = *reinterpret_cast<const f32x4*>(sbias + co + 8 * g + 4 * hh);
#pragma unroll
            for (int j = 0; j < 4; ++j) bv[4 * g + j] = b4[j];
          }
        }
#pragma unroll
        for (int m = 0; m < MF; ++m) {
          if (has_bias) {
#pragma unroll
            for (int g = 0; g < 4; ++g) {
              packed[DEFER ? m : 0][DEFER ? q : 0][2 * g] = pack_bf16x2(acc[m][q][4 * g] + bv[4 * g], acc[m][q][4 * g + 1] + bv[4 * g + 1]);
              packed[DEFER ? m : 0][DEFER ? q : 0][2 * g + 1] = pack_bf16x2(acc[m][q][4 * g + 2] + bv[4 * g + 2], acc[m][q][4 * g + 3] + bv[4 * g + 3]);
            }
          } else {
#pragma unroll
            for (int g = 0; g < 4; ++g) {
              packed[DEFER ? m : 0][DEFER ? q : 0][2 * g] = pack_bf16x2(acc[m][q][4 * g], acc[m][q][4 * g + 1]);
              packed[DEFER ? m : 0][DEFER ? q : 0][2 * g + 1] = pack_bf16x2(acc[m][q][4 * g + 2], acc[m][q][4 * g + 3]);
            }
          }
          if (!DEFER) {
            frag_to_lds(packed[0][0], fidx & 1);
            if (pm_ >= 0) { frag_from_lds(tvp, (fidx - 1) & 1); frag_store(pm_, pq_, tvp); }
            pm_ = m; pq_ = q; ++fidx;
          }
          if (STATS) {
            if constexpr (!DEFER) {
              typedef float f32x2 __attribute__((ext_vector_type(2)));
#pragma unroll
              for (int i = 0; i < 16; i += 2) {
                const f32x2 av = {acc[m][q][i], acc[m][q][i + 1]};
                f32x2 sv = {s1[q][i], s1[q][i + 1]}, tv = {s2[q][i], s2[q][i + 1]};
                sv += av;
                tv = __builtin_elementwise_fma(av, av, tv);
                s1[q][i] = sv[0]; s1[q][i + 1] = sv[1]; s2[q][i] = tv[0]; s2[q][i + 1] = tv[1];
              }
            } else {
#pragma unroll
            for (int i = 0; i < 16; ++i) {
              s1[q][i] += acc[m][q][i];
              s2[q][i] = fmaf(acc[m][q][i], acc[m][q][i], s2[q][i]);
            }
            }
          }
        }
      }
      if (!DEFER && !mrg_done) { frag_from_lds(tvp, (fidx - 1) & 1); frag_store(pm_, pq_, tvp); }
      if (DEFER) { set_item(img, tyi, txi, nbi); pend = true; }
      if (STATS && !WRES) {
        if constexpr (!mrg_done) {
#pragma unroll
          for (int q = 0; q < NF; ++q) stats_to_ws(q);
        }
        pending_tile = tile; pending_nbi = nbi; parity ^= 1;
      }
    }

    }
    if (wave == 0) TRACE(2, sidx);
    __syncthreads();
    if (wave == 0) TRACE(3, sidx);
#ifdef OCT_TRACE
    if (p.trace && blockIdx.x == 0 && wave == 0 && lane == 0 && sidx == nstage - 1) p.trace[2044] = __builtin_amdgcn_s_memrealtime();
#endif
    cur = DMA ? (cur + 1 == NBUF ? 0 : cur + 1) : (cur ^ 1);
    if (++ch == p.nch) {
      ch = 0; ++item;
      if (++nbi_c == p.nblk) {
        nbi_c = 0; tile_c += tstep;
        txi_c += sx; if (txi_c >= p.tiles_x) { txi_c -= p.tiles_x; ++tyi_c; }
        tyi_c += sy; if (tyi_c >= p.tiles_y) { tyi_c -= p.tiles_y; ++img_c; }
        img_c += simg;
      }
    }
  }

  if (DEFER && pend) {
#pragma unroll
    for (int idx = 0; idx < NFR; ++idx) store_frag(idx / NF, idx % NF);
  }

  if constexpr (FUSE) {
    float* const scr = reinterpret_cast<float*>(fxt);
    static_assert(4 * 64 * 16 * 4 <= 2 * XTB || !FUSE, "the reduction scratch fits the x tiles");
    float* const mine = scr + (wave * 64 + lane) * 16;
#pragma unroll
    for (int j = 0; j < 8; j += 4) {
      *reinterpret_cast<f32x4*>(mine + j) = f32x4{bs1[j], bs1[j + 1], bs1[j + 2], bs1[j + 3]};
      *reinterpret_cast<f32x4*>(mine + 8 + j) = f32x4{bs2[j], bs2[j + 1], bs2[j + 2], bs2[j + 3]};
    }
    __syncthreads();
    if (tid < 64) {
      const int st = tid >> 5, c = tid & 31;
      float s = 0.f;
      for (int w_ = 0; w_ < 4; ++w_)
        for (int l = 0; l < 16; ++l) s += scr[(w_ * 64 + 4 * l + (c >> 3)) * 16 + st * 8 + (c & 7)];
      p.bnpart[((size_t)blockIdx.x * 2 + st) * 32 + c] = s;
    }
  }

  if (STATS) {
    if (WRES) {
      float* ws = wg_stats;
#pragma unroll
      for (int q = 0; q < NF; ++q) {
        const float t1 = reduce32_scatter16(s1[q], lane);
        const float t2 = reduce32_scatter16(s2[q], lane);
        if ((lane & 1) == 0) {
          const int reg = scatter16_reg_of_lane(lane);
          const int cl = (wn * NF + q) * 32 + (reg & 3) + 8 * (reg >> 2) + 4 * hh;
          ws[(wm * 2 + 0) * NT + cl] = t1;
          ws[(wm * 2 + 1) * NT + cl] = t2;
        }
      }
      __syncthreads();
      for (int i = tid; i < 2 * NT; i += 256) {
        const int st = i / NT, cl = i - st * NT;
        float s = 0.f;
#pragma unroll
        for (int w_ = 0; w_ < WM; ++w_) s += ws[(w_ * 2 + st) * NT + cl];
        if (cl < p.cout) p.stats[((size_t)blockIdx.x * 2 + st) * p.cout + cl] = s;
      }
    } else {
      if (pending_tile >= 0) {
        const float* ws = wg_stats + (parity ^ 1) * (WM * 2 * NT);
        for (int i = tid; i < 2 * NT; i += 256) {
          const int st = i / NT, cl = i - st * NT;
          float s = 0.f;
#pragma unroll
          for (int w_ = 0; w_ < WM; ++w_) s += ws[(w_ * 2 + st) * NT + cl];
          wgacc[st * p.cout + pending_nbi * NT + cl] += s;
        }
      }
      __syncthreads();
      for (int i = tid; i < 2 * p.cout; i += 256) p.stats[(size_t)blockIdx.x * 2 * p.cout + i] = wgacc[i];
    }
  }
}

enum { IG2_TILE, IG2_1X1, IG2_WLDS, IG2_DMA };

bool igemm2_plan(const OctConvDesc* d, ConvPlan* out) {
  if (d->kh == 7) {
    const int rem = d->h % 8;
    if (d->taps != 21 || d->kw != 3 || d->depth > 0 || d->out_img_mul != 0 || rem == 1 || rem == 2 || (d->cout % 64) != 0) return false;
  }
  if ((d->depth > 0 || d->out_img_mul != 0) && ((d->w % 32) != 0 || (d->h % 16) != 0)) return false;
  const int cin = d->in_mode == OCT_IN_S2D ? (d->depth > 0 ? 8 : 4) * d->c0 : d->c0 + d->c1;
  const bool whole = (d->w % 32) == 0 && (d->h % 8) == 0;
  const bool plain = d->in_mode == OCT_IN_PLAIN && d->out_mode == OCT_OUT_PLAIN;
  bool ok = d->dtype == OCT_DT_BF16 && (whole || plain) && (d->c0 % 32) == 0 &&
            (d->c1 % 32) == 0 && (d->cout % 32) == 0 && (d->split % 32) == 0;
  ok = ok && (d->c0 + d->c1) <= 1024 && d->cout <= 4096;
  if (d->taps != 1) ok = ok && plain;
  else ok = ok && (plain ||
            (!d->want_stats && d->split == 0 &&
             ((d->in_mode == OCT_IN_PLAIN && d->out_mode == OCT_OUT_D2S && ((d->cout >> 2) % 32) == 0) ||
              (d->in_mode == OCT_IN_S2D && d->out_mode == OCT_OUT_PLAIN && d->c1 == 0))));
  if (!ok) return false;
  ConvPlan pl = {};
  pl.path = CONV_IGEMM2;
  pl.nt = d->cout == 32 ? 32 : (d->cout % 128 == 0 ? 128 : (d->cout % 64 == 0 ? 64 : 0));
  if (pl.nt == 128 && d->split > 0 && (d->split % 64) != 0) pl.nt = 64;
  if (pl.nt == 0) return false;
  pl.wres = (d->taps == 9) && (cin == 32) && (d->cout == pl.nt) && pl.nt <= 64 && d->depth == 0;
  pl.nblk = d->cout / pl.nt;
  pl.th = (d->taps == 9 && (pl.nt == 32 || (pl.nt == 64 && !pl.wres && (d->split % 64) == 0)) && (d->h % 16) == 0) ? 16 : 8;
  const int ntiles = ((d->w + 31) / 32) * ((d->h + pl.th - 1) / pl.th) * d->n;
  pl.nitems = ntiles * pl.nblk;
  int target = 256;
  if (target > pl.nitems) target = pl.nitems;
  pl.per_wg = (pl.nitems + target - 1) / target;
  pl.grid = (pl.nitems + pl.per_wg - 1) / pl.per_wg;
  pl.interleave = 0;
  if (ntiles >= 2 * target) {
    pl.grid = target;
    pl.interleave = 1;
  }
  pl.stat_rows = pl.grid;
  const bool dma = !d->xform0 && !d->xform1 && d->c1 == 0 && !d->want_stats && !pl.wres && pl.th == 8 &&
                   d->depth == 0 && d->out_img_mul == 0 && (d->w % 32) == 0 && (d->h % 8) == 0 && pl.nt >= 64 &&
                   ((d->taps == 9) || (d->in_mode == OCT_IN_S2D && d->out_mode == OCT_OUT_PLAIN));
  const bool wlds = d->taps == 9 && pl.nt == 32 && pl.th == 16 && !pl.wres && (d->c0 + d->c1) <= 64 && d->depth == 0 &&
                    d->out_img_mul == 0 && (d->w % 32) == 0;
  pl.kernel = dma ? IG2_DMA : d->taps == 1 ? IG2_1X1 : wlds ? IG2_WLDS : IG2_TILE;
  *out = pl;
  return true;
}

template <int WM, int WN, int MF, int NF, bool WRES, int TAPS = 9>
static int launch_v2(const Igemm2Params& p, int grid, hipStream_t s) {
  constexpr int TH = WM * MF;
  constexpr int LH = TH + (TAPS == 21 ? 6 : 2);
  const int lds = 2 * LH * 34 * ig2_pixb<TAPS, NF, WRES, false>() + (2 * WM * 2 * (WN * NF * 32) + 4 + 2 * 1024) * (int)sizeof(float) + 2 * 4 * 32 * 80 + 1024 * (int)sizeof(float) +
                  (p.stats ? 2 * p.cout * (int)sizeof(float) : 0);
  const bool ragged = (p.w % 32) != 0 || (p.h % TH) != 0;
  void (*kern)(Igemm2Params) = nullptr;
  if (p.depth > 0) {
    if constexpr (!WRES && TAPS == 9)
      kern = p.stats ? igemm2_kernel<TAPS, WM, WN, MF, NF, false, true, false, true> : igemm2_kernel<TAPS, WM, WN, MF, NF, false, false, false, true>;
  } else if (ragged) {
    kern = p.stats ? igemm2_kernel<TAPS, WM, WN, MF, NF, WRES, true, true> : igemm2_kernel<TAPS, WM, WN, MF, NF, WRES, false, true>;
  } else {
    kern = p.stats ? igemm2_kernel<TAPS, WM, WN, MF, NF, WRES, true> : igemm2_kernel<TAPS, WM, WN, MF, NF, WRES, false>;
  }
  if (!kern) { oct_set_error("igemm2: no depth-tap instantiation of this tiling"); return OCT_E_INVALID; }
  if (const int rc = oct_lds_optin(reinterpret_cast<const void*>(kern), 160 * 1024)) return rc;
  hipLaunchKernelGGL(kern, dim3(grid), dim3(512), lds, s, p);
  return OCT_OK;
}
template <int WM, int WN, int MF, int NF>
static int launch_v2_1x1(const Igemm2Params& p, int grid, hipStream_t s) {
  constexpr int TH = WM * MF;
  const int lds = 2 * TH * 32 * 80 + (2 * WM * 2 * (WN * NF * 32) + 4 + 2 * 1024) * (int)sizeof(float) + 2 * 4 * 32 * 80 + 1024 * (int)sizeof(float) +
                  (p.stats ? 2 * p.cout * (int)sizeof(float) : 0);
  const bool ragged = (p.w % 32) != 0 || (p.h % TH) != 0;
  if (p.in_mode == OCT_IN_PLAIN && p.out_mode == OCT_OUT_PLAIN && (p.stats || ragged)) {
    if (ragged) {
      if (p.stats) hipLaunchKernelGGL((igemm2_kernel<1, WM, WN, MF, NF, false, true, true>), dim3(grid), dim3(512), lds, s, p);
      else hipLaunchKernelGGL((igemm2_kernel<1, WM, WN, MF, NF, false, false, true>), dim3(grid), dim3(512), lds, s, p);
    } else hipLaunchKernelGGL((igemm2_kernel<1, WM, WN, MF, NF, false, true>), dim3(grid), dim3(512), lds, s, p);
  } else if (p.depth > 0 || p.oimg_mul)
    hipLaunchKernelGGL((igemm2_kernel<1, WM, WN, MF, NF, false, false, false, true>), dim3(grid), dim3(512), lds, s, p);
  else
    hipLaunchKernelGGL((igemm2_kernel<1, WM, WN, MF, NF, false, false>), dim3(grid), dim3(512), lds, s, p);
  return OCT_OK;
}
template <int WM, int MF>
static int launch_v2_wlds(const Igemm2Params& p, int grid, hipStream_t s) {
  constexpr int TH = WM * MF;
  const int lds = 2 * (TH + 2) * 34 * 80 + (2 * WM * 2 * 32 + 4) * (int)sizeof(float) + 2 * 64 * (int)sizeof(float) + 4 * 32 * 80 + 2 * 18 * 1024 +
                  (p.stats ? 2 * p.cout * (int)sizeof(float) : 0);
  const auto kern = p.stats ? igemm2_kernel<9, WM, 1, MF, 1, false, true, false, false, false, true> : igemm2_kernel<9, WM, 1, MF, 1, false, false, false, false, false, true>;
  if (const int rc = oct_lds_optin(reinterpret_cast<const void*>(kern), 160 * 1024)) return rc;
  hipLaunchKernelGGL(kern, dim3(grid), dim3(512), lds, s, p);
  return OCT_OK;
}
template <int TAPS, int WM, int WN, int MF, int NF>
static int launch_v2_dma(const Igemm2Params& p, int grid, hipStream_t s) {
  constexpr int TH = WM * MF, HALO = TAPS != 1 ? 1 : 0, HALO_Y = TAPS == 21 ? 3 : HALO;
  constexpr int NSLOT = ((TH + 2 * HALO_Y) * (32 + 2 * HALO) + 63) / 64, NBUF = TAPS != 1 ? 3 : 6;
  constexpr int lds = NBUF * NSLOT * 4096 + (2 * WM * 2 * (WN * NF * 32) + 4 + 2 * 1024) * (int)sizeof(float) + 2 * 4 * 32 * 80 + 1024 * (int)sizeof(float);
  static_assert(lds <= 160 * 1024, "LDS budget");
  if (const int rc = oct_lds_optin(reinterpret_cast<const void*>(&igemm2_kernel<TAPS, WM, WN, MF, NF, false, false, false, false, true>), lds)) return rc;
  hipLaunchKernelGGL((igemm2_kernel<TAPS, WM, WN, MF, NF, false, false, false, false, true>), dim3(grid), dim3(512), lds, s, p);
  return OCT_OK;
}

int launch_igemm2(const ConvPlan& pl, const OctConvDesc* d, const OctConvArgs* a, hipStream_t s) {
  Igemm2Params p;
  p.x0 = (const bf16_t*)a->x0; p.x1 = (const bf16_t*)a->x1;
  p.sc0 = a->scale0; p.sh0 = a->shift0; p.sc1 = a->scale1; p.sh1 = a->shift1;
  p.wp = (const bf16_t*)a->wpacked; p.y0 = (bf16_t*)a->y0; p.y1 = (bf16_t*)a->y1;
  p.stats = d->want_stats ? a->stat_partials : nullptr;
  p.bias = a->bias; p.in_mode = d->in_mode; p.out_mode = d->out_mode;
#ifdef OCT_TRACE
  p.trace = g_trace;
#else
  p.trace = nullptr;
#endif
  p.n = d->n; p.h = d->h; p.w = d->w; p.c0 = d->c0; p.c1 = d->c1; p.cout = d->cout; p.split = d->split;
  p.xf0 = d->xform0; p.xf1 = d->xform1;
  p.tiles_x = (d->w + 31) / 32; p.tiles_y = (d->h + pl.th - 1) / pl.th; p.nblk = pl.nblk; p.nitems = pl.nitems; p.per_wg = pl.per_wg;
  p.interleave = pl.interleave;
  const int ktot = d->in_mode == OCT_IN_S2D ? (d->depth > 0 ? 8 : 4) * d->c0 : (d->depth > 0 ? 3 : 1) * (d->c0 + d->c1);
  p.nch = ktot / 32; p.nk16 = ktot / 16;
  p.depth = d->depth; p.nchc = (d->c0 + d->c1) / 32; p.oimg_mul = d->out_img_mul; p.oimg_add = d->out_img_add;
  if (p.depth > 0 && p.oimg_mul == 0) p.oimg_mul = 1;
  const int g = pl.grid;
  int rc;
  if (pl.kernel == IG2_DMA) {
    if (d->taps == 9) rc = pl.nt == 64 ? launch_v2_dma<9, 2, 2, 4, 1>(p, g, s) : launch_v2_dma<9, 2, 2, 4, 2>(p, g, s);
    else rc = pl.nt == 64 ? launch_v2_dma<1, 2, 2, 4, 1>(p, g, s) : launch_v2_dma<1, 2, 2, 4, 2>(p, g, s);
  } else if (pl.kernel == IG2_1X1) {
    rc = pl.nt == 32 ? launch_v2_1x1<4, 1, 2, 1>(p, g, s) : pl.nt == 64 ? launch_v2_1x1<2, 2, 4, 1>(p, g, s) : launch_v2_1x1<2, 2, 4, 2>(p, g, s);
  } else if (pl.kernel == IG2_WLDS) {
    rc = launch_v2_wlds<4, 4>(p, g, s);
  } else if (d->taps == 21) {
    rc = pl.nt == 64 ? launch_v2<2, 2, 4, 1, false, 21>(p, g, s) : launch_v2<2, 2, 4, 2, false, 21>(p, g, s);
  } else if (pl.nt == 32 && pl.th == 16) {
    rc = pl.wres ? launch_v2<4, 1, 4, 1, true>(p, g, s) : launch_v2<4, 1, 4, 1, false>(p, g, s);
  } else if (pl.nt == 32) {
    rc = pl.wres ? launch_v2<4, 1, 2, 1, true>(p, g, s) : launch_v2<4, 1, 2, 1, false>(p, g, s);
  } else if (pl.nt == 64 && pl.th == 16) {
    rc = launch_v2<4, 1, 4, 2, false>(p, g, s);
  } else if (pl.nt == 64) {
    rc = pl.wres ? launch_v2<2, 2, 4, 1, true>(p, g, s) : launch_v2<2, 2, 4, 1, false>(p, g, s);
  } else {
    rc = launch_v2<2, 2, 4, 2, false>(p, g, s);
  }
  return rc ? rc : oct_check_launch("igemm2");
}

bool igemm2_fused_plan(const OctWgradDesc* d, ConvPlan* out) {
  const bool ok = d->dtype == OCT_DT_BF16 && d->depth == 0 && d->taps == 9 && (d->kh == 0 || d->kh == 3) && (d->kw == 0 || d->kw == 3) &&
                  d->c0 == 32 && d->c1 == 0 && d->cout == 32 && d->xform0 == OCT_XF_AFFINE_RELU && d->dy_mode == OCT_IN_PLAIN &&
                  d->in_img_shift == 0 && d->dy_img_mul == 0 && d->partials == 0 && d->n > 0 && d->h > 0 && d->w > 0 &&
                  (d->w % 32) == 0 && (d->h % 8) == 0 && (size_t)d->n * d->h * d->w < (1u << 31);
  if (!ok) return false;
  ConvPlan pl = {};
  pl.path = CONV_IGEMM2;
  pl.kernel = IG2_TILE;
  pl.nt = 32; pl.wres = true; pl.nblk = 1; pl.th = 8;
  const int ntiles = (d->w / 32) * (d->h / 8) * d->n;
  pl.nitems = ntiles;
  const int target = ntiles < 256 ? ntiles : 256;
  pl.per_wg = (ntiles + target - 1) / target;
  pl.grid = (ntiles + pl.per_wg - 1) / pl.per_wg;
  pl.interleave = 0;
  if (ntiles >= 2 * target) { pl.grid = target; pl.interleave = 1; }
  pl.stat_rows = pl.grid;
  *out = pl;
  return true;
}

int launch_igemm2_fused(const ConvPlan& pl, const OctWgradDesc* d, const OctConvBwdFusedArgs* a, hipStream_t s) {
  Igemm2Params p = {};
  p.x0 = (const bf16_t*)a->dy; p.wp = (const bf16_t*)a->wpacked; p.y0 = (bf16_t*)a->dx;
  p.in_mode = OCT_IN_PLAIN; p.out_mode = OCT_OUT_PLAIN;
  p.n = d->n; p.h = d->h; p.w = d->w; p.c0 = 32; p.cout = 32;
  p.tiles_x = d->w / 32; p.tiles_y = d->h / pl.th; p.nblk = 1; p.nitems = pl.nitems; p.per_wg = pl.per_wg;
  p.interleave = pl.interleave;
  p.nch = 1; p.nk16 = 2; p.nchc = 1;
  p.fx = (const bf16_t*)a->x; p.fsc = a->scale; p.fsh = a->shift; p.fmean = a->mean; p.finvstd = a->invstd;
  p.dwp = a->dwp; p.bnpart = a->partials;
#ifdef OCT_TRACE
  p.trace = g_trace;
#endif
  constexpr int TH = 8;
  constexpr int lds = 2 * (TH + 2) * 34 * ig2_pixb<9, 1, true, false>() + (2 * 4 * 2 * 32 + 4 + 2 * 1024) * (int)sizeof(float) + 2 * 4 * 32 * 80 +
                      1024 * (int)sizeof(float) + 4 * TH * 32 * 64;
  static_assert(lds <= 160 * 1024, "LDS budget");
  const auto kern = igemm2_kernel<9, 4, 1, 2, 1, true, false, false, false, false, false, true>;
  if (const int rc = oct_lds_optin(reinterpret_cast<const void*>(kern), 160 * 1024)) return rc;
  hipLaunchKernelGGL(kern, dim3(pl.grid), dim3(512), lds, s, p);
  return oct_check_launch("igemm2 (fused backward)");
}
```

retinal_oct_image_segmentation_via_deep_learning_amd/engine.py:

```python
from __future__ import annotations

import ctypes as C
import os
from dataclasses import dataclass, field

import torch

from . import _lib as L

BN_EPS = 1e-5
BN_MOMENTUM = 0.1

@dataclass
class ConvKeys:
    w: str
    bn: str
    b: str | None = None


@dataclass
class BlockSpec:
    name: str
    c1: ConvKeys
    c2: ConvKeys
    cout: int


@dataclass
class NetSpec:
    cin: int
    ncls: int
    enc: list
    ups: list
    dec: list
    head_w: str
    head_b: str
    dec_first: bool
    softmax_out: bool

    @property
    def divisor(self) -> int:
        return 1 << (len(self.enc) - 1)

    @property
    def head_feat(self) -> int:
        return self.dec[-1].cout


def ynet_unet_spec(cin: int, ncls: int, f: int) -> NetSpec:
    def blk(mod, pre, cout):
        return BlockSpec(pre, ConvKeys(f"{mod}.{pre}conv1.weight", f"{mod}.{pre}norm1"),
                         ConvKeys(f"{mod}.{pre}conv2.weight", f"{mod}.{pre}norm2"), cout)
    enc = [blk(f"encoder{i + 1}", f"enc{i + 1}", f << i) for i in range(4)] + [blk("bottleneck", "bottleneck", f * 16)]
    ups = [(f"upconv{k}.weight", f"upconv{k}.bias", f << (k - 1)) for k in (4, 3, 2, 1)]
    dec = [blk(f"decoder{k}", f"dec{k}", f << (k - 1)) for k in (4, 3, 2, 1)]
    return NetSpec(cin, ncls, enc, ups, dec, "conv.weight", "conv.bias", dec_first=True, softmax_out=True)


def bionet_unet_spec(cin: int, ncls: int) -> NetSpec:
    def blk(mod, cout):
        return BlockSpec(mod, ConvKeys(f"{mod}.0.weight", f"{mod}.1", f"{mod}.0.bias"),
                         ConvKeys(f"{mod}.3.weight", f"{mod}.4", f"{mod}.3.bias"), cout)
    enc = [blk("enc1", 64), blk("enc2", 128), blk("enc3", 256), blk("enc4", 512)]
    ups = [(f"up{k}.weight", f"up{k}.bias", c) for k, c in ((4, 256), (3, 128), (2, 64))]
    dec = [blk("dec4", 256), blk("dec3", 128), blk("dec2", 64)]
    return NetSpec(cin, ncls, enc, ups, dec, "final.weight", "final.bias", dec_first=False, softmax_out=False)


def _stream() -> int:
    return torch.cuda.current_stream().cuda_stream


@dataclass
class Src:
    x0: torch.Tensor
    c0: int
    bn0: "BNState | None" = None
    x1: torch.Tensor | None = None
    c1: int = 0
    bn1: "BNState | None" = None

    @property
    def channels(self) -> int:
        return self.c0 + self.c1


@dataclass
class BNState:
    scale: torch.Tensor
    shift: torch.Tensor
    mean: torch.Tensor | None = None
    invstd: torch.Tensor | None = None
    relu: bool = True
    frozen: bool = False


def _xf(bn) -> int:
    return L.XF_NONE if bn is None else (L.XF_AFFINE_RELU if bn.relu else L.XF_AFFINE)


@dataclass
class ConvRec:
    wkey: str
    gkey: str
    bkey: str
    cbkey: str | None
    src: Src
    y: torch.Tensor
    bn: BNState
    cout: int
    n: int
    h: int
    w: int


@dataclass
class Ctx:
    n: int = 0
    h: int = 0
    w: int = 0
    convs: dict = field(default_factory=dict)
    ups: dict = field(default_factory=dict)
    head_in: ConvRec | None = None
    target: torch.Tensor | None = None
    dice_coef: torch.Tensor | None = None
    loss: torch.Tensor | None = None
    loss_cfg: tuple = (1.0, 0.0, 1e-7)
    loss_partials: torch.Tensor | None = None


class UNetEngine:
    def __init__(self, in_channels: int, out_channels: int, features: int = 32, dtype: str = "bf16",
                 spec: NetSpec | None = None):
        if out_channels > L.MAX_CLASSES:
            raise L.OctError(f"out_channels={out_channels} exceeds the head kernel's limit {L.MAX_CLASSES}")
        self.spec = spec if spec is not None else ynet_unet_spec(in_channels, out_channels, features)
        self.cin, self.ncls, self.f = self.spec.cin, self.spec.ncls, self.spec.head_feat
        self.set_dtype(dtype)
        self._packed = {}
        self._arena, self._arena_on, self._arena_off, self._arena_short = None, False, 0, False
        self._unpack_jobs = []
        self._nbt = []
        self._frozen_bwd = False
        self.supports_frozen_bwd = True
        self._consts = {}
        self.rowdot_off = os.environ.get("OCT_ROWDOT", "1") == "0"
        self.deterministic = os.environ.get("OCT_DETERMINISTIC", "0") == "1"
        self.fused_bwd_off = False
        self.debug = None
        self.prof = None
        self.prof_labels = None

    def set_dtype(self, dtype: str) -> None:
        if dtype not in ("bf16", "f32"):
            raise ValueError("dtype must be 'bf16' or 'f32'")
        self.dtype = dtype
        self.dt = L.DT_BF16 if dtype == "bf16" else L.DT_F32
        self.tdt = torch.bfloat16 if dtype == "bf16" else torch.float32
        self._packed = {}
        self._pack_plan = {}

    def _prof_begin(self):
        if self.prof is None:
            return None
        ev = torch.cuda.Event(enable_timing=True)
        ev.record()
        return ev

    def _prof_end(self, ev, kind, label=None):
        if ev is not None:
            end = torch.cuda.Event(enable_timing=True)
            end.record()
            self.prof.append((kind, ev, end))
            if self.prof_labels is not None:
                self.prof_labels.append(label)

    def _const(self, value: float, n: int, dev):
        key = (float(value), int(n), str(dev))
        t = self._consts.get(key)
        if t is None:
            t = self._consts[key] = torch.full((n,), float(value), dtype=torch.float32, device=dev)
        return t

    def _act(self, n, h, w, c, dev):
        return torch.empty((n, h, w, c), dtype=self.tdt, device=dev)

    def _pack(self, key: str, wt: torch.Tensor, mode: int, cout: int, cin: int, kdi: int = 0) -> torch.Tensor:
        ver = (wt._version, L.param_generation[0])
        hit = self._packed.get((key, mode))
        if hit is not None and hit[0] == ver and hit[2] == wt.data_ptr():
            return hit[1]
        self._pack_plan[(key, mode)] = (cout, cin)
        rows, taps, kch = {
            L.PACK_CONV_FPROP: (cout, 9, cin), L.PACK_CONV_DGRAD: (cin, 9, cout),
            L.PACK_DECONV_FPROP: (4 * cout, 1, cin), L.PACK_DECONV_DGRAD: (cin, 1, 4 * cout),
            L.PACK_1X1_DGRAD: (cin, 1, cout), L.PACK_1X1_FPROP: (cout, 1, cin),
            L.PACK_CONV3D_FPROP: (cout, 9, 3 * cin), L.PACK_CONV3D_DGRAD: (cin, 9, 3 * cout),
            L.PACK_DECONV3D_FPROP: (4 * cout, 1, cin), L.PACK_DECONV3D_DGRAD: (cin, 1, 8 * cout)}[mode]
        elems = L.lib().oct_packed_weight_elems(rows, taps, kch)
        out = hit[1] if hit is not None else torch.empty(elems, dtype=self.tdt, device=wt.device)
        if mode >= L.PACK_CONV3D_FPROP:
            self._pack_plan.pop((key, mode), None)
            L.check(L.lib().oct_pack_weights3d(mode, self.dt, wt.data_ptr(), out.data_ptr(), cout, cin, kdi, _stream()),
                    "oct_pack_weights3d")
        else:
            L.check(L.lib().oct_pack_weights(mode, self.dt, wt.data_ptr(), out.data_ptr(), cout, cin, _stream()),
                    "oct_pack_weights")
        self._packed[(key, mode)] = (ver, out, wt.data_ptr())
        return out

    def _prepack(self, P: dict) -> None:
        jobs, news = [], []
        for (key, mode), (cout, cin) in self._pack_plan.items():
            wt = P.get(key) if isinstance(key, str) else None
            hit = self._packed.get((key, mode))
            if wt is None or hit is None or hit[2] != wt.data_ptr():
                continue
            ver = (wt._version, L.param_generation[0])
            if hit[0] != ver:
                jobs.append(L.PackJob(mode, cout, cin, 0, wt.data_ptr(), hit[1].data_ptr()))
                news.append(((key, mode), (ver, hit[1], hit[2])))
        if jobs:
            arr = (L.PackJob * len(jobs))(*jobs)
            L.check(L.lib().oct_pack_weights_batch(self.dt, len(jobs), arr, _stream()), "oct_pack_weights_batch")
            self._packed.update(news)

    def _conv(self, src: Src, wpacked, cout, taps, n, h, w, y0, *, y1=None, split=0, in_mode=L.IN_PLAIN,
              out_mode=L.OUT_PLAIN, bias=None, stats=None, kh=0, kw=0, depth=0, oimg=(0, 0)):
        d = L.ConvDesc(self.dt, n, h, w, src.c0, src.c1, cout, taps,
                       _xf(src.bn0), _xf(src.bn1),
                       in_mode, out_mode, split, 1 if stats is not None else 0, kh, kw, depth, oimg[0], oimg[1])
        a = L.ConvArgs(L.ptr(src.x0), L.ptr(src.x1),
                       L.ptr(src.bn0.scale) if src.bn0 else None, L.ptr(src.bn0.shift) if src.bn0 else None,
                       L.ptr(src.bn1.scale) if src.bn1 else None, L.ptr(src.bn1.shift) if src.bn1 else None,
                       L.ptr(wpacked), L.ptr(bias), L.ptr(y0), L.ptr(y1), L.ptr(stats))
        ev = self._prof_begin()
        L.check(L.lib().oct_conv_forward(C.byref(d), C.byref(a), _stream()), "oct_conv_forward")
        self._prof_end(ev, "igemm", (taps, src.channels, cout, n, h, w, in_mode, out_mode))

    def _stat_blocks(self, cout, n, h, w, src: Src, taps=9, kh=0, kw=0, depth=0):
        d = L.ConvDesc(self.dt, n, h, w, src.c0, src.c1, cout, taps,
                       _xf(src.bn0), _xf(src.bn1), 0, 0, 0, 1, kh, kw, depth, 0, 0)
        return L.lib().oct_conv_stat_blocks(C.byref(d))

    def _wgrad(self, src: Src, dy, cout, taps, n, h, w, dy_mode=L.IN_PLAIN, dbias=None, fused_apply=None, kh=0, kw=0,
               depth=0, in_shift=0, dy_img=(0, 0), dwp=None, partials_ok=True):
        ktot = src.channels
        parts = 1 if (self.deterministic and partials_ok and dwp is None and depth == 0) else 0
        d = L.WgradDesc(self.dt, n, h, w, src.c0, src.c1, cout, taps,
                        _xf(src.bn0), _xf(src.bn1), dy_mode, kh, kw, depth, in_shift,
                        dy_img[0], dy_img[1], parts)
        bias_parts = None
        if parts:
            nparts = L.lib().oct_conv_wgrad_partials(C.byref(d))
            dwp = torch.empty((nparts, taps, cout, ktot), dtype=torch.float32, device=dy.device)
            dwp._oct_nparts = nparts
            if dbias is not None:
                bias_parts = torch.empty((nparts, cout), dtype=torch.float32, device=dy.device)
        elif dwp is None:
            dwp = self._dwp_take(taps * cout * ktot, dy.device).view(taps, cout, ktot)
        a = L.WgradArgs(L.ptr(src.x0), L.ptr(src.x1),
                        L.ptr(src.bn0.scale) if src.bn0 else None, L.ptr(src.bn0.shift) if src.bn0 else None,
                        L.ptr(src.bn1.scale) if src.bn1 else None, L.ptr(src.bn1.shift) if src.bn1 else None,
                        L.ptr(dy), L.ptr(dwp), L.ptr(dbias), *([L.ptr(t) for t in fused_apply] if fused_apply
                                                                 else [None, None, None, None]), L.ptr(bias_parts))
        ev = self._prof_begin()
        L.check(L.lib().oct_conv_wgrad(C.byref(d), C.byref(a), _stream()), "oct_conv_wgrad")
        self._prof_end(ev, "wgrad", (taps, ktot, cout, n, h, w, dy_mode, 0))
        if bias_parts is not None:
            L.check(L.lib().oct_reduce_bias_partials(bias_parts.data_ptr(), nparts, cout,
                                                     cout // 4 if dy_mode == L.IN_S2D else cout, dbias.data_ptr(), 1,
                                                     _stream()), "oct_reduce_bias_partials")
        return dwp

    def _dwp_take(self, numel: int, dev) -> torch.Tensor:
        if self._arena_on:
            lo = self._arena_off
            self._arena_off = lo + (numel + 63) // 64 * 64
            if self._arena is not None and self._arena_off <= self._arena.numel() and self._arena.device == dev:
                return self._arena[lo:lo + numel]
            self._arena_short = True
        return torch.zeros(numel, dtype=torch.float32, device=dev)

    def _arena_begin(self, dev):
        self._arena_on, self._arena_off, self._arena_short = True, 0, False
        self._unpack_jobs = []
        if self._arena is not None and self._arena.device == dev:
            self._arena.zero_()

    def _flush_unpack(self):
        if self._unpack_jobs:
            arr = (L.UnpackJob * len(self._unpack_jobs))(*[j[0] for j in self._unpack_jobs])
            L.check(L.lib().oct_unpack_wgrad_batch(len(self._unpack_jobs), arr, _stream()), "oct_unpack_wgrad_batch")
            self._unpack_jobs = []

    def _arena_end(self, dev):
        self._flush_unpack()
        if self._arena_short or self._arena is None:
            self._arena = torch.empty(self._arena_off, dtype=torch.float32, device=dev)
        self._arena_on = False

    def _unpack(self, mode, dwp, grad, cout, cin, accumulate):
        job = L.UnpackJob(mode, cout, cin, int(accumulate), getattr(dwp, "_oct_nparts", 1), 0, dwp.data_ptr(), grad.data_ptr())
        if self._arena_on:
            self._unpack_jobs.append((job, dwp, grad))
            return
        arr = (L.UnpackJob * 1)(job)
        L.check(L.lib().oct_unpack_wgrad_batch(1, arr, _stream()), "oct_unpack_wgrad_batch")

    def _conv_bn(self, P, keys: ConvKeys, src: Src, cout, n, h, w, train: bool) -> ConvRec:
        wkey, nk = keys.w, keys.bn
        wt = P[wkey]
        dev = wt.device
        cbias = L.ptr(P[keys.b]) if keys.b else None
        wp = self._pack(wkey, wt, L.PACK_CONV_FPROP, cout, src.channels)
        y = self._act(n, h, w, cout, dev)
        scale = torch.empty(cout, dtype=torch.float32, device=dev)
        shift = torch.empty_like(scale)
        if train:
            nblk = self._stat_blocks(cout, n, h, w, src)
            partials = torch.empty((nblk, 2, cout), dtype=torch.float32, device=dev)
            self._conv(src, wp, cout, 9, n, h, w, y, stats=partials)
            mean = torch.empty_like(scale)
            invstd = torch.empty_like(scale)
            L.check(L.lib().oct_bn_finalize(
                partials.data_ptr(), nblk, cout, float(n * h * w), P[nk + ".weight"].data_ptr(),
                P[nk + ".bias"].data_ptr(), BN_EPS, BN_MOMENTUM, P[nk + ".running_mean"].data_ptr(),
                P[nk + ".running_var"].data_ptr(), mean.data_ptr(), invstd.data_ptr(), scale.data_ptr(),
                shift.data_ptr(), cbias, _stream()), "oct_bn_finalize")
            self._nbt.append(P[nk + ".num_batches_tracked"])
            bn = BNState(scale, shift, mean, invstd)
        else:
            self._conv(src, wp, cout, 9, n, h, w, y)
            L.check(L.lib().oct_bn_eval_coeffs(
                cout, P[nk + ".weight"].data_ptr(), P[nk + ".bias"].data_ptr(),
                P[nk + ".running_mean"].data_ptr(), P[nk + ".running_var"].data_ptr(), BN_EPS,
                scale.data_ptr(), shift.data_ptr(), cbias, _stream()), "oct_bn_eval_coeffs")
            if self._frozen_bwd:
                invstd = torch.rsqrt(P[nk + ".running_var"] + BN_EPS)
                mean = P[nk + ".running_mean"] - P[keys.b] if keys.b else P[nk + ".running_mean"]
                bn = BNState(scale, shift, mean, invstd, frozen=True)
            else:
                bn = BNState(scale, shift)
        return ConvRec(wkey, nk + ".weight", nk + ".bias", keys.b, src, y, bn, cout, n, h, w)

    def _block(self, P, blk: BlockSpec, src, n, h, w, train, ctx):
        r1 = self._conv_bn(P, blk.c1, src, blk.cout, n, h, w, train)
        r2 = self._conv_bn(P, blk.c2, Src(r1.y, blk.cout, r1.bn), blk.cout, n, h, w, train)
        ctx.convs[blk.name] = [r1, r2]
        return r2

    def forward(self, P: dict, x: torch.Tensor, train: bool, target: torch.Tensor | None = None,
                loss_cfg=(1.0, 0.0, 1e-7), want_probs=True, want_argmax=False, want_logits=False, defer_loss=False,
                frozen_bwd=False):
        lib = L.lib()
        if x.dim() != 4 or x.shape[1] != self.cin:
            raise RuntimeError(f"expected input (B,{self.cin},H,W), got {tuple(x.shape)}")
        n, _, h, w = x.shape
        sp = self.spec
        if h % sp.divisor or w % sp.divisor:
            raise RuntimeError(
                f"Sizes of tensors must match except in dimension 1. Input {h}x{w} is not divisible by {sp.divisor} "
                f"({len(sp.enc) - 1} 2x2 poolings followed by as many 2x up-samplings)")
        dev = x.device
        if dev.type != "cuda":
            raise L.OctError("the HIP path needs a device tensor (there is no CPU fallback)")
        xf = x.detach().to(torch.float32).contiguous()
        if train or frozen_bwd:
            self._prepack(P)
        self._frozen_bwd = bool(frozen_bwd) and not train
        ctx = Ctx(n=n, h=h, w=w, loss_cfg=tuple(loss_cfg))
        self._nbt = []
        xt = self._act(n, h, w, self.cin, dev)
        L.check(lib.oct_nchw_to_nhwc(self.dt, xf.data_ptr(), xt.data_ptr(), n, self.cin, h, w, _stream()),
                "oct_nchw_to_nhwc")
        src = Src(xt, self.cin)
        hh, ww = h, w
        skips = []
        prev = None
        for li, blk in enumerate(sp.enc):
            prev = self._block(P, blk, src, n, hh, ww, train, ctx)
            if li == len(sp.enc) - 1:
                break
            skips.append(prev)
            pooled = self._act(n, hh // 2, ww // 2, blk.cout, dev)
            L.check(lib.oct_bn_relu_pool_fwd(self.dt, prev.y.data_ptr(), prev.bn.scale.data_ptr(),
                                             prev.bn.shift.data_ptr(), pooled.data_ptr(), n, hh, ww, blk.cout,
                                             _stream()), "oct_bn_relu_pool_fwd")
            hh //= 2
            ww //= 2
            src = Src(pooled, blk.cout)
        for di, ((wkey, bkey, cout_d), blk) in enumerate(zip(sp.ups, sp.dec)):
            cin_d = prev.cout
            wp = self._pack(wkey, P[wkey], L.PACK_DECONV_FPROP, cout_d, cin_d)
            u = self._act(n, hh * 2, ww * 2, cout_d, dev)
            self._conv(Src(prev.y, cin_d, prev.bn), wp, 4 * cout_d, 1, n, hh, ww, u, out_mode=L.OUT_D2S, bias=P[bkey])
            ctx.ups[di] = (prev, u)
            hh *= 2
            ww *= 2
            sk = skips[len(skips) - 1 - di]
            src = (Src(u, cout_d, None, sk.y, sk.cout, sk.bn) if sp.dec_first
                   else Src(sk.y, sk.cout, sk.bn, u, cout_d, None))
            prev = self._block(P, blk, src, n, hh, ww, train, ctx)
        ctx.head_in = prev
        if self._nbt:
            torch._foreach_add_(self._nbt, 1)
            self._nbt = []
        self._frozen_bwd = False
        hd = L.HeadDesc(self.dt, n, h, w, self.f, self.ncls)
        probs = torch.empty((n, self.ncls, h, w), dtype=torch.float32, device=dev) if want_probs else None
        amax = torch.empty((n, h, w), dtype=torch.int64, device=dev) if want_argmax else None
        logits = torch.empty((n, self.ncls, h, w), dtype=torch.float32, device=dev) if want_logits else None
        partials = None
        if target is not None:
            if target.shape != (n, h, w):
                raise RuntimeError(f"target must be (B,H,W)={n, h, w}, got {tuple(target.shape)}")
            target = target.to(device=dev, dtype=torch.int64).contiguous()
            nb = lib.oct_head_blocks(C.byref(hd))
            partials = torch.empty((nb, L.HEAD_LOSS_SLOTS), dtype=torch.float64, device=dev)
            if (defer_loss and loss_cfg[1] == 0.0 and self.f == 32 and self.ncls <= 8
                    and not (want_probs or want_argmax or want_logits)):
                ctx.target = target
                ctx.loss = torch.empty(3, dtype=torch.float32, device=dev)
                ctx.dice_coef = torch.zeros(2 * L.MAX_CLASSES, dtype=torch.float32, device=dev)
                ctx.loss_partials = partials
                return ctx, None, None, None
        L.check(lib.oct_head_forward(C.byref(hd), prev.y.data_ptr(), prev.bn.scale.data_ptr(),
                                     prev.bn.shift.data_ptr(), P[sp.head_w].data_ptr(),
                                     P[sp.head_b].data_ptr(), L.ptr(target), L.ptr(probs), L.ptr(amax),
                                     L.ptr(logits), L.ptr(partials), _stream()), "oct_head_forward")
        if target is not None:
            w_ce, w_dice, eps = loss_cfg
            ctx.target = target
            ctx.loss = torch.empty(3, dtype=torch.float32, device=dev)
            ctx.dice_coef = torch.zeros(2 * L.MAX_CLASSES, dtype=torch.float32, device=dev)
            L.check(lib.oct_head_loss_finalize(C.byref(hd), partials.data_ptr(), partials.shape[0], w_ce, w_dice,
                                               eps, ctx.loss.data_ptr(), ctx.dice_coef.data_ptr(), _stream()),
                    "oct_head_loss_finalize")
        return ctx, probs, amax, logits

    def _bn_backward(self, rec: ConvRec, da, dpool, G, accumulate, partials=None, defer_apply=False):
        lib = L.lib()
        n, h, w, c = rec.n, rec.h, rec.w, rec.cout
        dev = rec.y.device
        pooled = dpool is not None
        g = da if da is not None else self._act(n, h, w, c, dev)
        pool_fused = pooled and partials is None and self.debug is None and bool(lib.oct_bn_bwd_apply_pool_ok(self.dt, n, h, w, c))
        if partials is not None:
            nblk = partials.shape[0]
        else:
            nblk = lib.oct_dact_bn_reduce_blocks(n, h, w, c, 1 if pooled else 0)
            partials = torch.empty((nblk, 2, c), dtype=torch.float32, device=dev)
            L.check(lib.oct_dact_bn_reduce(self.dt, L.ptr(da), L.ptr(dpool), rec.y.data_ptr(), rec.bn.scale.data_ptr(),
                                           rec.bn.shift.data_ptr(), rec.bn.mean.data_ptr(), rec.bn.invstd.data_ptr(),
                                           g.data_ptr() if (pooled and not pool_fused) else None, partials.data_ptr(),
                                           n, h, w, c, _stream()),
                    "oct_dact_bn_reduce")
        coef = torch.empty((3, c), dtype=torch.float32, device=dev)
        L.check(lib.oct_bn_bwd_finalize(partials.data_ptr(), nblk, c, float(n * h * w), self._P[rec.gkey].data_ptr(),
                                        rec.bn.mean.data_ptr(), rec.bn.invstd.data_ptr(), G[rec.gkey].data_ptr(),
                                        G[rec.bkey].data_ptr(), coef.data_ptr(), int(accumulate), _stream()),
                "oct_bn_bwd_finalize")
        if self.debug is not None:
            self.debug["g:" + rec.wkey] = g.float().clone()
        if rec.bn.frozen:
            coef[1:].zero_()
            if rec.cbkey:
                gb = coef[0] * partials[:, 0, :].sum(0)
                G[rec.cbkey].add_(gb) if accumulate else G[rec.cbkey].copy_(gb)
        if defer_apply and not pooled:
            return g, coef
        if pool_fused:
            L.check(lib.oct_bn_bwd_apply_pool(self.dt, L.ptr(da), dpool.data_ptr(), rec.y.data_ptr(), rec.bn.scale.data_ptr(),
                                              rec.bn.shift.data_ptr(), coef.data_ptr(), g.data_ptr(), n, h, w, c, _stream()),
                    "oct_bn_bwd_apply_pool")
            return g
        L.check(lib.oct_bn_bwd_apply(self.dt, g.data_ptr(), rec.y.data_ptr(), coef.data_ptr(),
                                     None if pooled else rec.bn.scale.data_ptr(),
                                     None if pooled else rec.bn.shift.data_ptr(), n * h * w, c, _stream()),
                "oct_bn_bwd_apply")
        if self.debug is not None:
            self.debug["dy:" + rec.wkey] = g.float().clone()
            self.debug["y:" + rec.wkey] = rec.y.float().clone()
            self.debug["coef:" + rec.wkey] = coef.clone()
        return g

    def _conv_backward(self, rec: ConvRec, dy, G, accumulate, need_dx=True):
        n, h, w = rec.n, rec.h, rec.w
        src = rec.src
        cin = src.channels
        dwp = self._wgrad(src, dy, rec.cout, 9, n, h, w)
        self._unpack(L.PACK_CONV_FPROP, dwp, G[rec.wkey], rec.cout, cin, accumulate)
        if not need_dx:
            return None, None
        wp = self._pack(rec.wkey, self._P[rec.wkey], L.PACK_CONV_DGRAD, rec.cout, cin)
        d0 = self._act(n, h, w, src.c0, dy.device)
        d1 = self._act(n, h, w, src.c1, dy.device) if src.c1 else None
        self._conv(Src(dy, rec.cout), wp, cin, 9, n, h, w, d0, y1=d1, split=src.c0 if src.c1 else 0)
        if self.debug is not None:
            def bnc(b):
                return None if b is None else (b.scale.clone(), b.shift.clone())
            self.debug["layer:" + rec.wkey] = dict(
                x0=src.x0.float().clone(), bn0=bnc(src.bn0), x1=None if src.x1 is None else src.x1.float().clone(),
                bn1=bnc(src.bn1), dy=dy.float().clone(), d0=d0.float().clone(), d1=None if d1 is None else d1.float().clone(),
                y=rec.y.float().clone())
        return d0, d1

    def _conv_backward_fused(self, r1: ConvRec, r2: ConvRec, dy2, G, accumulate):
        src = r2.src
        if self.fused_bwd_off or self.debug is not None or self.deterministic or src.c1 or src.bn0 is None or src.bn0 is not r1.bn or src.x0 is not r1.y:
            return None
        lib = L.lib()
        n, h, w, cin, cout = r2.n, r2.h, r2.w, src.c0, r2.cout
        d = L.WgradDesc(self.dt, n, h, w, cin, 0, cout, 9, _xf(src.bn0), L.XF_NONE, L.IN_PLAIN, 0, 0, 0, 0, 0, 0, 0)
        if not lib.oct_conv_backward_fused_ok(C.byref(d)):
            return None
        dev = dy2.device
        wp = self._pack(r2.wkey, self._P[r2.wkey], L.PACK_CONV_DGRAD, cout, cin)
        da1 = self._act(n, h, w, cin, dev)
        dwp = self._dwp_take(9 * cout * cin, dev).view(9, cout, cin)
        parts = torch.empty((lib.oct_conv_backward_fused_blocks(C.byref(d)), 2, cin), dtype=torch.float32, device=dev)
        a = L.ConvBwdFusedArgs(L.ptr(r1.y), L.ptr(r1.bn.scale), L.ptr(r1.bn.shift), L.ptr(r1.bn.mean), L.ptr(r1.bn.invstd),
                               L.ptr(dy2), L.ptr(wp), L.ptr(da1), L.ptr(dwp), L.ptr(parts))
        ev = self._prof_begin()
        L.check(lib.oct_conv_backward_fused(C.byref(d), C.byref(a), _stream()), "oct_conv_backward_fused")
        self._prof_end(ev, "igemm", (9, cout, cin, n, h, w, L.IN_PLAIN, L.OUT_PLAIN))
        self._unpack(L.PACK_CONV_FPROP, dwp, G[r2.wkey], cout, cin, accumulate)
        return da1, parts

    def _block_backward(self, name, da, dpool, G, accumulate, need_dx=True, partials=None):
        r1, r2 = self._ctx.convs[name]
        for r in (r1, r2):
            if r.cbkey and not accumulate and not r.bn.frozen:
                G[r.cbkey].zero_()
        dy2 = self._bn_backward(r2, da, dpool, G, accumulate, partials=partials)
        fused = self._conv_backward_fused(r1, r2, dy2, G, accumulate)
        if fused is not None:
            da1, parts1 = fused
        else:
            (da1, _), parts1 = self._conv_backward(r2, dy2, G, accumulate), None
        first_fused = False
        if not need_dx and r1.src.c1 == 0 and r1.src.bn0 is None:
            qd = L.WgradDesc(self.dt, r1.n, r1.h, r1.w, r1.src.c0, 0, r1.cout, 9, L.XF_NONE, L.XF_NONE, L.IN_PLAIN)
            first_fused = bool(L.lib().oct_conv_wgrad_fused_apply_ok(C.byref(qd)))
        if first_fused:
            da1, coef = self._bn_backward(r1, da1, None, G, accumulate, partials=parts1, defer_apply=True)
            dwp = self._wgrad(r1.src, da1, r1.cout, 9, r1.n, r1.h, r1.w,
                              fused_apply=(r1.y, coef, r1.bn.scale, r1.bn.shift))
            self._unpack(L.PACK_CONV_FPROP, dwp, G[r1.wkey], r1.cout, 1, accumulate)
            return None, None
        dy1 = self._bn_backward(r1, da1, None, G, accumulate, partials=parts1)
        return self._conv_backward(r1, dy1, G, accumulate, need_dx=need_dx)

    def backward_stages(self):
        sp = self.spec

        def blk_keys(b: BlockSpec):
            ks = []
            for c in (b.c1, b.c2):
                ks += [c.w, c.bn + ".weight", c.bn + ".bias"] + ([c.b] if c.b else [])
            return ks
        nd = len(sp.dec)
        stages = []
        for di in range(nd - 1, -1, -1):
            ks = ([sp.head_w, sp.head_b] if di == nd - 1 else []) + blk_keys(sp.dec[di]) + list(sp.ups[di][:2])
            stages.append((f"dec{di}", ks))
        for li in range(len(sp.enc) - 1, -1, -1):
            stages.append((f"enc{li}", blk_keys(sp.enc[li])))
        return stages

    def _stage_done(self, hook, idx):
        if hook is not None and idx in hook.flush_stages:
            self._flush_unpack()
            hook.stage_done(idx)

    def backward(self, P: dict, ctx: Ctx, G: dict, dprobs: torch.Tensor | None = None, accumulate=False,
                 dlogits: torch.Tensor | None = None, stage_hook=None):
        lib = L.lib()
        sp = self.spec
        self._P, self._ctx = P, ctx
        n, h, w, f, ncls = ctx.n, ctx.h, ctx.w, self.f, self.ncls
        rec = ctx.head_in
        dev = rec.y.device
        self._arena_begin(dev)
        hd = L.HeadDesc(self.dt, n, h, w, f, ncls)
        if dprobs is not None:
            dprobs = dprobs.to(torch.float32).contiguous()
            tgt, dc, w_ce = None, None, 0.0
        elif dlogits is None:
            if ctx.target is None:
                raise RuntimeError("backward without an output gradient needs forward(target=...)")
            tgt, dc, w_ce = ctx.target, ctx.dice_coef, ctx.loss_cfg[0]
        hsrc = Src(rec.y, f, rec.bn)
        head_partials = None
        hw, hb = P[sp.head_w], P[sp.head_b]
        bgrad, wgrad_t = G[sp.head_b], G[sp.head_w]
        fused_dw = False
        dl = None
        if f == 32 and dlogits is None:
            fused_dw = ncls <= 8
            if not accumulate:
                bgrad.zero_()
                if fused_dw:
                    wgrad_t.zero_()
            if not fused_dw:
                dl = self._act(n, h, w, ncls, dev)
            da = self._act(n, h, w, f, dev)
            nb = lib.oct_head_blocks(C.byref(hd))
            head_partials = torch.empty((nb, 2, f), dtype=torch.float32, device=dev)
            L.check(lib.oct_head_backward_fused(
                C.byref(hd), rec.y.data_ptr(), rec.bn.scale.data_ptr(), rec.bn.shift.data_ptr(),
                rec.bn.mean.data_ptr(), rec.bn.invstd.data_ptr(), hw.data_ptr(),
                hb.data_ptr(), L.ptr(tgt), L.ptr(dc), w_ce, L.ptr(dprobs), L.ptr(dl), da.data_ptr(),
                head_partials.data_ptr(), bgrad.data_ptr(), wgrad_t.data_ptr() if fused_dw else None,
                L.ptr(ctx.loss_partials) if dprobs is None else None, _stream()),
                "oct_head_backward_fused")
            if ctx.loss_partials is not None and dprobs is None:
                w_ce_, w_dice_, eps_ = ctx.loss_cfg
                L.check(lib.oct_head_loss_finalize(C.byref(hd), ctx.loss_partials.data_ptr(), ctx.loss_partials.shape[0],
                                                   w_ce_, w_dice_, eps_, ctx.loss.data_ptr(), ctx.dice_coef.data_ptr(),
                                                   _stream()), "oct_head_loss_finalize")
        else:
            dl = self._act(n, h, w, ncls, dev)
            if dlogits is not None:
                dlf = dlogits.to(torch.float32).contiguous()
                L.check(lib.oct_nchw_to_nhwc(self.dt, dlf.data_ptr(), dl.data_ptr(), n, ncls, h, w, _stream()),
                        "oct_nchw_to_nhwc")
            else:
                L.check(lib.oct_head_dlogits(C.byref(hd), rec.y.data_ptr(), rec.bn.scale.data_ptr(),
                                             rec.bn.shift.data_ptr(), hw.data_ptr(), hb.data_ptr(), L.ptr(tgt),
                                             L.ptr(dc), w_ce, L.ptr(dprobs), dl.data_ptr(), _stream()),
                        "oct_head_dlogits")
            L.check(lib.oct_channel_sum(self.dt, dl.data_ptr(), bgrad.data_ptr(), n * h * w, ncls, int(accumulate),
                                        _stream()), "oct_channel_sum")
            wp = self._pack(sp.head_w, hw, L.PACK_1X1_DGRAD, ncls, f)
            da = self._act(n, h, w, f, dev)
            self._conv(Src(dl, ncls), wp, f, 1, n, h, w, da)
        if not fused_dw:
            dwp = self._wgrad(hsrc, dl, ncls, 1, n, h, w)
            self._unpack(L.PACK_1X1_FPROP, dwp, wgrad_t, ncls, f, accumulate)
        nd = len(sp.dec)
        dskip = [None] * nd
        for di in range(nd - 1, -1, -1):
            d0, d1 = self._block_backward(sp.dec[di].name, da, None, G, accumulate,
                                          partials=head_partials if di == nd - 1 else None)
            du, dskip[di] = (d0, d1) if sp.dec_first else (d1, d0)
            wkey, bkey, cout_d = sp.ups[di]
            prev, u = ctx.ups[di]
            cin_d = prev.cout
            hl, wl = prev.h, prev.w
            bgrad = G[bkey]
            if not accumulate:
                bgrad.zero_()
            dwp = self._wgrad(Src(prev.y, cin_d, prev.bn), du, 4 * cout_d, 1, n, hl, wl, dy_mode=L.IN_S2D,
                              dbias=bgrad)
            self._unpack(L.PACK_DECONV_FPROP, dwp, G[wkey], cout_d, cin_d, accumulate)
            wp = self._pack(wkey, P[wkey], L.PACK_DECONV_DGRAD, cout_d, cin_d)
            da = self._act(n, hl, wl, cin_d, dev)
            self._conv(Src(du, cout_d), wp, cin_d, 1, n, hl, wl, da, in_mode=L.IN_S2D)
            if self.debug is not None:
                self.debug["up:" + wkey] = dict(x=prev.y.float().clone(), bn=(prev.bn.scale.clone(), prev.bn.shift.clone()),
                                                u=u.float().clone(), du=du.float().clone(), da=da.float().clone(), bkey=bkey)
            self._stage_done(stage_hook, nd - 1 - di)
        dpool, _ = self._block_backward(sp.enc[-1].name, da, None, G, accumulate)
        self._stage_done(stage_hook, nd)
        for li in range(len(sp.enc) - 2, -1, -1):
            dpool, _ = self._block_backward(sp.enc[li].name, dskip[nd - 1 - li], dpool, G, accumulate,
                                            need_dx=(li != 0))
            if li:
                self._stage_done(stage_hook, nd + len(sp.enc) - 1 - li)
        self._arena_end(dev)
        self._stage_done(stage_hook, nd + len(sp.enc) - 1)
        self._P = self._ctx = None
        return G
```

Baseline: 1230 B-scans/s.

## Fuse BatchNorm-backward reductions into the 3x3 data-gradient DMA kernel epilogue

Adds a BNS variant of the DMA igemm2 data-gradient kernel. While computing dx for the second conv of a block, it also reads the previous conv's output y, applies the ReLU mask, and accumulates per-channel BN-backward sums (sum of dy and sum of dy*xhat) into per-block partials. This removes the separate full-tensor reduction pass over da1 and y in the following BN backward for blocks with 128+ channels. The cost is extra LDS use, an extra y stream overlapped with the DMA pipeline, extra barriers, and a forced 8-row tile.

```diff
diff --git a/include/oct_hip.h b/include/oct_hip.h
--- a/include/oct_hip.h
+++ b/include/oct_hip.h
@@ -127,6 +127,18 @@
 int oct_conv_backward_fused_ok(const OctWgradDesc* d);
 int oct_conv_backward_fused_blocks(const OctWgradDesc* d);
 int oct_conv_backward_fused(const OctWgradDesc* d, const OctConvBwdFusedArgs* a, void* stream);
+typedef struct OctConvDgradBnsumsArgs {
+  const void* dy;
+  const void* wpacked;
+  void* dx;
+  const void* y;
+  const float* scale; const float* shift;
+  const float* mean; const float* invstd;
+  float* partials;
+} OctConvDgradBnsumsArgs;
+int oct_conv_dgrad_bnsums_ok(const OctConvDesc* d);
+int oct_conv_dgrad_bnsums_blocks(const OctConvDesc* d);
+int oct_conv_dgrad_bnsums(const OctConvDesc* d, const OctConvDgradBnsumsArgs* a, void* stream);
 int oct_unpack_wgrad(int mode, const float* dwp, float* grad, int cout, int cin, int accumulate, void* stream);
 int oct_unpack_wgrad_kk(const float* dwp, float* grad, int cout, int cin, int kh, int kw, int accumulate, void* stream);
 int oct_unpack_wgrad3d(int mode, const float* dwp, float* grad, int cout, int cin, int kdi, int accumulate, void* stream);
diff --git a/retinal_oct_image_segmentation_via_deep_learning_amd/_lib.py b/retinal_oct_image_segmentation_via_deep_learning_amd/_lib.py
--- a/retinal_oct_image_segmentation_via_deep_learning_amd/_lib.py
+++ b/retinal_oct_image_segmentation_via_deep_learning_amd/_lib.py
@@ -62,6 +62,10 @@
 
 class ConvBwdFusedArgs(C.Structure):
     _fields_ = [(k, c_void_p) for k in ("x", "scale", "shift", "mean", "invstd", "dy", "wpacked", "dx", "dwp", "partials")]
+
+
+class ConvDgradBnsumsArgs(C.Structure):
+    _fields_ = [(k, c_void_p) for k in ("dy", "wpacked", "dx", "y", "scale", "shift", "mean", "invstd", "partials")]
 
 
 class HeadDesc(C.Structure):
@@ -113,6 +117,9 @@
     "oct_conv_backward_fused_ok": (c_int, [C.POINTER(WgradDesc)]),
     "oct_conv_backward_fused_blocks": (c_int, [C.POINTER(WgradDesc)]),
     "oct_conv_backward_fused": (c_int, [C.POINTER(WgradDesc), C.POINTER(ConvBwdFusedArgs), c_void_p]),
+    "oct_conv_dgrad_bnsums_ok": (c_int, [C.POINTER(ConvDesc)]),
+    "oct_conv_dgrad_bnsums_blocks": (c_int, [C.POINTER(ConvDesc)]),
+    "oct_conv_dgrad_bnsums": (c_int, [C.POINTER(ConvDesc), C.POINTER(ConvDgradBnsumsArgs), c_void_p]),
     "oct_conv_wgrad_partials": (c_int, [C.POINTER(WgradDesc)]),
     "oct_reduce_bias_partials": (c_int, [c_void_p, c_int, c_int, c_int, c_void_p, c_int, c_void_p]),
     "oct_unpack_wgrad": (c_int, [c_int, c_void_p, c_void_p, c_int, c_int, c_int, c_void_p]),
diff --git a/retinal_oct_image_segmentation_via_deep_learning_amd/csrc/common.h b/retinal_oct_image_segmentation_via_deep_learning_amd/csrc/common.h
--- a/retinal_oct_image_segmentation_via_deep_learning_amd/csrc/common.h
+++ b/retinal_oct_image_segmentation_via_deep_learning_amd/csrc/common.h
@@ -42,6 +42,8 @@
 int launch_igemm(const ConvPlan& pl, const OctConvDesc* d, const OctConvArgs* a, hipStream_t s);
 bool igemm2_fused_plan(const OctWgradDesc* d, ConvPlan* pl);
 int launch_igemm2_fused(const ConvPlan& pl, const OctWgradDesc* d, const OctConvBwdFusedArgs* a, hipStream_t s);
+bool igemm2_bns_plan(const OctConvDesc* d, ConvPlan* pl);
+int launch_igemm2_bns(const ConvPlan& pl, const OctConvDesc* d, const OctConvDgradBnsumsArgs* a, hipStream_t s);
 
 enum WgradPath { WGRAD_FIRST, WGRAD_W2, WGRAD_GENERIC };
 struct WgradPlan {
diff --git a/retinal_oct_image_segmentation_via_deep_learning_amd/csrc/conv_dispatch.hip b/retinal_oct_image_segmentation_via_deep_learning_amd/csrc/conv_dispatch.hip
--- a/retinal_oct_image_segmentation_via_deep_learning_amd/csrc/conv_dispatch.hip
+++ b/retinal_oct_image_segmentation_via_deep_learning_amd/csrc/conv_dispatch.hip
@@ -151,3 +151,28 @@
             "oct_conv_backward_fused: null tensor");
   return launch_igemm2_fused(pl, d, a, as_stream(stream));
 }
+
+static bool plan_conv_dgrad_bnsums(const OctConvDesc* d, ConvPlan* pl) {
+  return d && v2_enabled() && igemm2_bns_plan(d, pl);
+}
+
+extern "C" int oct_conv_dgrad_bnsums_ok(const OctConvDesc* d) {
+  ConvPlan pl;
+  return plan_conv_dgrad_bnsums(d, &pl) ? 1 : 0;
+}
+
+extern "C" int oct_conv_dgrad_bnsums_blocks(const OctConvDesc* d) {
+  ConvPlan pl;
+  return plan_conv_dgrad_bnsums(d, &pl) ? pl.stat_rows : 0;
+}
+
+extern "C" int oct_conv_dgrad_bnsums(const OctConvDesc* d, const OctConvDgradBnsumsArgs* a, void* stream) {
+  OCT_CHECK(d && a, "oct_conv_dgrad_bnsums: null descriptor");
+  ConvPlan pl;
+  OCT_CHECK(plan_conv_dgrad_bnsums(d, &pl),
+            "oct_conv_dgrad_bnsums: not available for this descriptor (oct_conv_dgrad_bnsums_ok): bf16, 2-D, 3x3, plain in and out, "
+            "one source, no transform, no split, no statistics, c0 %% 64 == 0, cout %% 64 == 0, cout <= 512, w %% 32 == 0, h %% 8 == 0");
+  OCT_CHECK(a->dy && a->wpacked && a->dx && a->y && a->scale && a->shift && a->mean && a->invstd && a->partials,
+            "oct_conv_dgrad_bnsums: null tensor");
+  return launch_igemm2_bns(pl, d, a, as_stream(stream));
+}
diff --git a/retinal_oct_image_segmentation_via_deep_learning_amd/csrc/igemm2.hip b/retinal_oct_image_segmentation_via_deep_learning_amd/csrc/igemm2.hip
--- a/retinal_oct_image_segmentation_via_deep_learning_amd/csrc/igemm2.hip
+++ b/retinal_oct_image_segmentation_via_deep_learning_amd/csrc/igemm2.hip
@@ -1,5 +1,6 @@
 #include "common.h"
 #include <stdlib.h>
+#include <type_traits>
 
 struct Igemm2Params {
   const bf16_t* x0; const bf16_t* x1;
@@ -45,9 +46,10 @@
 __device__ __attribute__((aligned(16))) unsigned int g_zero16[4];
 
 template <int TAPS, int WM, int WN, int MF, int NF, bool WRES, bool STATS, bool RAGGED = false, bool D3 = false, bool DMA = false,
-          bool WLDS = false, bool FUSE = false>
+          bool WLDS = false, bool FUSE = false, bool BNS = false>
 __global__ void __launch_bounds__(512) igemm2_kernel(const Igemm2Params p) {
   static_assert(WM * WN == 4, "four MFMA waves");
+  static_assert(!BNS || (DMA && TAPS == 9 && WM == 2 && WN == 2 && MF == 4), "BatchNorm-backward sums: the 3x3 DMA data gradients");
   static_assert(!FUSE || (TAPS == 9 && WM == 4 && NF == 1 && WRES && !STATS && !RAGGED && !D3 && !DMA && !WLDS),
                 "fused backward: resident weights, 32 -> 32 channels, whole tiles, 2-D");
   static_assert(!DMA || (!WRES && !STATS && !RAGGED && !D3), "DMA staging: streamed weights, whole tiles, 2-D, no BatchNorm sums");
@@ -100,10 +102,18 @@
   constexpr int XTB = TH * TW * 64;
   unsigned char* const fxt = reinterpret_cast<unsigned char*>(sbias + SBIAS_N);
   unsigned char* const fxr = fxt + 2 * XTB;
+  constexpr int BNS_P2 = 144, BNS_SLOT = NF == 2 ? 32 * BNS_P2 : 32 * 80, BNS_OTB = 4 * MF * BNS_SLOT;
+  unsigned char* const otile = smem + NBUF * BUFB;
+  float* const bcoef = reinterpret_cast<float*>(otile + BNS_OTB);
+  float* const bacc = bcoef + 4 * p.cout;
+  float* const bpart = bacc + 2 * p.cout;
   if (STATS && !WRES) {
     for (int i = tid; i < 2 * p.cout; i += 512) wgacc[i] = 0.f;
   }
-  {
+  if constexpr (BNS) {
+    for (int i = tid; i < p.cout; i += 512) *reinterpret_cast<f32x4*>(bcoef + 4 * i) = f32x4{p.fsc[i], p.fsh[i], p.fmean[i], p.finvstd[i]};
+    for (int i = tid; i < 2 * p.cout; i += 512) bacc[i] = 0.f;
+  } else {
     const int kx = s2d ? p.c0 : p.c0 + p.c1;
     for (int i = tid; i < kx; i += 512) {
       const bool first = i < p.c0;
@@ -198,6 +208,134 @@
 #pragma unroll
     for (int j = 0; j < NBUF - 1; ++j) { dma(buf0 + wb * BUFB); wb = wb + 1 == NBUF ? 0 : wb + 1; }
     stage_barrier();
+    if constexpr (BNS) {
+      constexpr int CG = NT / 8, PP = 256 / CG, NY = CG;
+      constexpr int CO = NF == 1 ? 1 : 0;
+      constexpr int NWY = NW + NY;
+      static_assert(NWY < 64, "vmcnt is a 6-bit counter");
+      const int cg = ptid % CG, pp = ptid / CG;
+      const unsigned ocs2 = 2u * (unsigned)p.cout;
+      const unsigned ylane = (unsigned)pp * ocs2 + (unsigned)cg * 16u;
+      const unsigned llane = NF == 2 ? (unsigned)((cg >> 3) * MF * BNS_SLOT + pp * BNS_P2 + (cg & 7) * 16)
+                                     : (unsigned)((cg >> 2) * BNS_SLOT + pp * 80 + (cg & 3) * 16);
+      u32x4 yr[NY];
+      int y_nbi = nbi_first, y_txi, y_tyi, y_img;
+      {
+        int t = t_first;
+        y_txi = t % p.tiles_x; t /= p.tiles_x;
+        y_tyi = t % p.tiles_y; y_img = t / p.tiles_y;
+      }
+      int c_nbi = 0;
+      int a_nbi = -1;
+      auto yload = [&]() {
+        const unsigned char* const yb = reinterpret_cast<const unsigned char*>(
+            p.fx + (((size_t)y_img * p.h + y_tyi * TH) * p.w + y_txi * TW) * p.cout + y_nbi * NT);
+        c_nbi = y_nbi;
+        if (++y_nbi == p.nblk) {
+          y_nbi = 0;
+          y_txi += sx; if (y_txi >= p.tiles_x) { y_txi -= p.tiles_x; ++y_tyi; }
+          y_tyi += sy; if (y_tyi >= p.tiles_y) { y_tyi -= p.tiles_y; ++y_img; }
+          y_img += simg;
+        }
+#pragma unroll
+        for (int i = 0; i < NY; ++i) {
+          const int row = (PP * i) >> 5, pxc = (PP * i) & 31;
+          yr[i] = *reinterpret_cast<const u32x4*>(yb + (ylane + (unsigned)(row * p.w + pxc) * ocs2));
+          if (i + 1 < NY) __builtin_amdgcn_s_sleep(1);
+        }
+      };
+      auto consume = [&]() {
+        f32x4 cf[8];
+        const float* const ct = bcoef + 4 * (c_nbi * NT + cg * 8);
+#pragma unroll
+        for (int j = 0; j < 8; ++j) cf[j] = *reinterpret_cast<const f32x4*>(ct + 4 * j);
+        float a1[8], a2[8];
+#pragma unroll
+        for (int j = 0; j < 8; ++j) { a1[j] = 0.f; a2[j] = 0.f; }
+#pragma unroll
+        for (int i = 0; i < NY; ++i) {
+          const int row = (PP * i) >> 5, pxc = (PP * i) & 31, wm_ = row >> 2, m_ = row & 3;
+          const int loff = NF == 2 ? (wm_ * 2 * MF + m_) * BNS_SLOT + pxc * BNS_P2 : (m_ * 4 + wm_ * 2) * BNS_SLOT + pxc * 80;
+          const u32x4 dv = *reinterpret_cast<const u32x4*>(otile + (llane + (unsigned)loff));
+          const u32x4 yv = yr[i];
+#pragma unroll
+          for (int j = 0; j < 4; ++j) {
+            const f32x4 c0 = cf[2 * j], c1 = cf[2 * j + 1];
+            const float y0 = bf16lo(yv[j]), y1 = bf16hi(yv[j]);
+            const float g0 = fmaf(y0, c0[0], c0[1]) > 0.f ? bf16lo(dv[j]) : 0.f;
+            const float g1 = fmaf(y1, c1[0], c1[1]) > 0.f ? bf16hi(dv[j]) : 0.f;
+            a1[2 * j] += g0;
+            a1[2 * j + 1] += g1;
+            a2[2 * j] = fmaf(g0, (y0 - c0[2]) * c0[3], a2[2 * j]);
+            a2[2 * j + 1] = fmaf(g1, (y1 - c1[2]) * c1[3], a2[2 * j + 1]);
+          }
+        }
+#pragma unroll
+        for (int j = 0; j < 8; ++j)
+#pragma unroll
+          for (int off = CG; off < 64; off <<= 1) {
+            a1[j] += __shfl_xor(a1[j], off);
+            a2[j] += __shfl_xor(a2[j], off);
+          }
+        if (lane < CG) {
+          float* const bp = bpart + (pw * 2) * NT + cg * 8;
+          *reinterpret_cast<f32x4*>(bp) = f32x4{a1[0], a1[1], a1[2], a1[3]};
+          *reinterpret_cast<f32x4*>(bp + 4) = f32x4{a1[4], a1[5], a1[6], a1[7]};
+          *reinterpret_cast<f32x4*>(bp + NT) = f32x4{a2[0], a2[1], a2[2], a2[3]};
+          *reinterpret_cast<f32x4*>(bp + NT + 4) = f32x4{a2[4], a2[5], a2[6], a2[7]};
+        }
+        a_nbi = c_nbi;
+      };
+      auto accumulate = [&]() {
+        if (a_nbi >= 0) {
+          if (ptid < 2 * NT) {
+            const int st = ptid / NT, c = ptid % NT;
+            float s = bpart[st * NT + c];
+#pragma unroll
+            for (int w_ = 1; w_ < 4; ++w_) s += bpart[(w_ * 2 + st) * NT + c];
+            bacc[st * p.cout + a_nbi * NT + c] += s;
+          }
+          a_nbi = -1;
+        }
+      };
+      auto bns_barrier = [&](auto cnt) {
+        constexpr int N = decltype(cnt)::value;
+        __builtin_amdgcn_s_waitcnt((N & 15) | ((N >> 4) << 14) | (7 << 4) | (0 << 8));
+        asm volatile("s_barrier" ::: "memory");
+      };
+      int ycnt = CO, yitem = 0;
+      for (int s0 = 0; s0 < nstage_pad; ++s0) {
+        accumulate();
+        const bool trig = ycnt == 0 && yitem < nitems_wg;
+        if (ycnt == 0) ycnt = p.nch;
+        --ycnt;
+        if (trig) {
+          if (yitem > 0) {
+            __builtin_amdgcn_s_waitcnt((7 << 4) | (15 << 8));
+            consume();
+          }
+          dma(buf0 + wb * BUFB); wb = wb + 1 == NBUF ? 0 : wb + 1;
+          yload();
+          ++yitem;
+          bns_barrier(std::integral_constant<int, NWY>{});
+        } else {
+          dma(buf0 + wb * BUFB); wb = wb + 1 == NBUF ? 0 : wb + 1;
+          bns_barrier(std::integral_constant<int, NW>{});
+        }
+      }
+      __syncthreads();
+      accumulate();
+      __syncthreads();
+      consume();
+      __syncthreads();
+      accumulate();
+      if (ptid < 2 * NT) {
+        const int st = ptid / NT, c = ptid % NT;
+        float* const rowp = p.bnpart + (size_t)blockIdx.x * 2 * p.cout + st * p.cout + c;
+        for (int nb = 0; nb < p.nblk; ++nb) rowp[nb * NT] = bacc[st * p.cout + nb * NT + c];
+      }
+      return;
+    }
     for (int s0 = 0; s0 < nstage_pad; ++s0) {
       dma(buf0 + wb * BUFB); wb = wb + 1 == NBUF ? 0 : wb + 1;
       stage_barrier();
@@ -568,7 +706,7 @@
   };
   typedef unsigned int u32x2 __attribute__((ext_vector_type(2)));
   auto frag_to_lds = [&](const unsigned (&pk)[8], int slot = 0) {
-    unsigned char* sc = oscr + (slot * 4 + wave) * (32 * 80);
+    unsigned char* sc = (BNS ? otile : oscr) + (slot * 4 + wave) * (32 * 80);
 #pragma unroll
     for (int g = 0; g < 4; ++g) {
       const u32x2 v = {pk[2 * g], pk[2 * g + 1]};
@@ -579,7 +717,7 @@
     }
   };
   auto frag_from_lds = [&](u32x4 (&tv)[2], int slot = 0) {
-    const unsigned char* sc = oscr + (slot * 4 + wave) * (32 * 80);
+    const unsigned char* sc = (BNS ? otile : oscr) + (slot * 4 + wave) * (32 * 80);
 #pragma unroll
     for (int k = 0; k < 2; ++k) {
       const int chunk = lane + 64 * k;
@@ -605,8 +743,8 @@
   };
   auto store_frag = [&](int m, int q) {
     u32x4 tv[2];
-    frag_to_lds(packed[DEFER ? m : 0][DEFER ? q : 0]);
-    frag_from_lds(tv);
+    frag_to_lds(packed[DEFER ? m : 0][DEFER ? q : 0], BNS ? m : 0);
+    frag_from_lds(tv, BNS ? m : 0);
     frag_store(m, q, tv);
   };
 
@@ -939,7 +1077,8 @@
       if constexpr (MRG) {
         {
           constexpr int P2 = 144;
-          unsigned char* const sc2 = oscr + wave * (32 * P2);
+          static_assert(P2 == BNS_P2, "the producers' view of the merged tile");
+          unsigned char* const sc2b = BNS ? otile + wave * (MF * 32 * P2) : oscr + wave * (32 * P2);
           static_assert(32 * P2 <= OSCR_SLOTS * 32 * 80, "the merged tile fits the wave's scratch");
           u32x4 tv4[4];
           int pm2 = -1;
@@ -973,6 +1112,7 @@
           }
 #pragma unroll
           for (int m = 0; m < MF; ++m) {
+            unsigned char* const sc2 = sc2b + (BNS ? m * (32 * P2) : 0);
 #pragma unroll
             for (int q = 0; q < NF; ++q) {
               unsigned pk[8];
@@ -1090,6 +1230,11 @@
 #pragma unroll
     for (int idx = 0; idx < NFR; ++idx) store_frag(idx / NF, idx % NF);
   }
+  if constexpr (BNS) {
+    __syncthreads();
+    __syncthreads();
+    __syncthreads();
+  }
 
   if constexpr (FUSE) {
     float* const scr = reinterpret_cast<float*>(fxt);
@@ -1151,7 +1296,7 @@
 
 enum { IG2_TILE, IG2_1X1, IG2_WLDS, IG2_DMA };
 
-bool igemm2_plan(const OctConvDesc* d, ConvPlan* out) {
+static bool igemm2_plan_impl(const OctConvDesc* d, ConvPlan* out, bool th8) {
   if (d->kh == 7) {
     const int rem = d->h % 8;
     if (d->taps != 21 || d->kw != 3 || d->depth > 0 || d->out_img_mul != 0 || rem == 1 || rem == 2 || (d->cout % 64) != 0) return false;
@@ -1176,7 +1321,7 @@
   if (pl.nt == 0) return false;
   pl.wres = (d->taps == 9) && (cin == 32) && (d->cout == pl.nt) && pl.nt <= 64 && d->depth == 0;
   pl.nblk = d->cout / pl.nt;
-  pl.th = (d->taps == 9 && (pl.nt == 32 || (pl.nt == 64 && !pl.wres && (d->split % 64) == 0)) && (d->h % 16) == 0) ? 16 : 8;
+  pl.th = (!th8 && d->taps == 9 && (pl.nt == 32 || (pl.nt == 64 && !pl.wres && (d->split % 64) == 0)) && (d->h % 16) == 0) ? 16 : 8;
   const int ntiles = ((d->w + 31) / 32) * ((d->h + pl.th - 1) / pl.th) * d->n;
   pl.nitems = ntiles * pl.nblk;
   int target = 256;
@@ -1195,6 +1340,21 @@
   const bool wlds = d->taps == 9 && pl.nt == 32 && pl.th == 16 && !pl.wres && (d->c0 + d->c1) <= 64 && d->depth == 0 &&
                     d->out_img_mul == 0 && (d->w % 32) == 0;
   pl.kernel = dma ? IG2_DMA : d->taps == 1 ? IG2_1X1 : wlds ? IG2_WLDS : IG2_TILE;
+  *out = pl;
+  return true;
+}
+
+bool igemm2_plan(const OctConvDesc* d, ConvPlan* out) { return igemm2_plan_impl(d, out, false); }
+
+bool igemm2_bns_plan(const OctConvDesc* d, ConvPlan* out) {
+  const bool ok = d->dtype == OCT_DT_BF16 && d->depth == 0 && d->out_img_mul == 0 && d->taps == 9 && (d->kh == 0 || d->kh == 3) &&
+                  (d->kw == 0 || d->kw == 3) && d->in_mode == OCT_IN_PLAIN && d->out_mode == OCT_OUT_PLAIN && d->c1 == 0 &&
+                  d->xform0 == 0 && d->xform1 == 0 && d->split == 0 && !d->want_stats && d->n > 0 && d->h > 0 && d->w > 0 &&
+                  (d->w % 32) == 0 && (d->h % 8) == 0 && d->cout > 0 && (d->cout % 64) == 0 && d->cout <= 512 && d->c0 > 0 &&
+                  (d->c0 % 64) == 0 && (size_t)d->n * d->h * d->w < (1u << 31);
+  if (!ok) return false;
+  ConvPlan pl;
+  if (!igemm2_plan_impl(d, &pl, true) || pl.kernel != IG2_DMA || pl.th != 8 || pl.stat_rows != pl.grid) return false;
   *out = pl;
   return true;
 }
@@ -1243,6 +1403,16 @@
   const int lds = 2 * (TH + 2) * 34 * 80 + (2 * WM * 2 * 32 + 4) * (int)sizeof(float) + 2 * 64 * (int)sizeof(float) + 4 * 32 * 80 + 2 * 18 * 1024 +
                   (p.stats ? 2 * p.cout * (int)sizeof(float) : 0);
   const auto kern = p.stats ? igemm2_kernel<9, WM, 1, MF, 1, false, true, false, false, false, true> : igemm2_kernel<9, WM, 1, MF, 1, false, false, false, false, false, true>;
+  if (const int rc = oct_lds_optin(reinterpret_cast<const void*>(kern), 160 * 1024)) return rc;
+  hipLaunchKernelGGL(kern, dim3(grid), dim3(512), lds, s, p);
+  return OCT_OK;
+}
+template <int NF>
+static int launch_v2_dma_bns(const Igemm2Params& p, int grid, hipStream_t s) {
+  constexpr int NT = 64 * NF;
+  const int lds = 3 * 6 * 4096 + 16 * 32 * (NF == 2 ? 144 : 80) + 24 * p.cout + 4 * 2 * NT * (int)sizeof(float);
+  if (lds > 160 * 1024) { oct_set_error("igemm2: %d output channels do not fit the LDS of the BatchNorm-sums data gradient", p.cout); return OCT_E_INVALID; }
+  const auto kern = igemm2_kernel<9, 2, 2, 4, NF, false, false, false, false, true, false, false, true>;
   if (const int rc = oct_lds_optin(reinterpret_cast<const void*>(kern), 160 * 1024)) return rc;
   hipLaunchKernelGGL(kern, dim3(grid), dim3(512), lds, s, p);
   return OCT_OK;
@@ -1303,6 +1473,23 @@
   return rc ? rc : oct_check_launch("igemm2");
 }
 
+int launch_igemm2_bns(const ConvPlan& pl, const OctConvDesc* d, const OctConvDgradBnsumsArgs* a, hipStream_t s) {
+  Igemm2Params p = {};
+  p.x0 = (const bf16_t*)a->dy; p.wp = (const bf16_t*)a->wpacked; p.y0 = (bf16_t*)a->dx;
+  p.in_mode = OCT_IN_PLAIN; p.out_mode = OCT_OUT_PLAIN;
+  p.n = d->n; p.h = d->h; p.w = d->w; p.c0 = d->c0; p.cout = d->cout;
+  p.tiles_x = d->w / 32; p.tiles_y = d->h / pl.th; p.nblk = pl.nblk; p.nitems = pl.nitems; p.per_wg = pl.per_wg;
+  p.interleave = pl.interleave;
+  p.nch = d->c0 / 32; p.nk16 = d->c0 / 16; p.nchc = p.nch;
+  p.fx = (const bf16_t*)a->y; p.fsc = a->scale; p.fsh = a->shift; p.fmean = a->mean; p.finvstd = a->invstd;
+  p.bnpart = a->partials;
+#ifdef OCT_TRACE
+  p.trace = g_trace;
+#endif
+  const int rc = pl.nt == 64 ? launch_v2_dma_bns<1>(p, pl.grid, s) : launch_v2_dma_bns<2>(p, pl.grid, s);
+  return rc ? rc : oct_check_launch("igemm2 (data gradient + BatchNorm sums)");
+}
+
 bool igemm2_fused_plan(const OctWgradDesc* d, ConvPlan* out) {
   const bool ok = d->dtype == OCT_DT_BF16 && d->depth == 0 && d->taps == 9 && (d->kh == 0 || d->kh == 3) && (d->kw == 0 || d->kw == 3) &&
                   d->c0 == 32 && d->c1 == 0 && d->cout == 32 && d->xform0 == OCT_XF_AFFINE_RELU && d->dy_mode == OCT_IN_PLAIN &&
diff --git a/retinal_oct_image_segmentation_via_deep_learning_amd/engine.py b/retinal_oct_image_segmentation_via_deep_learning_amd/engine.py
--- a/retinal_oct_image_segmentation_via_deep_learning_amd/engine.py
+++ b/retinal_oct_image_segmentation_via_deep_learning_amd/engine.py
@@ -147,6 +147,7 @@
         self.rowdot_off = os.environ.get("OCT_ROWDOT", "1") == "0"
         self.deterministic = os.environ.get("OCT_DETERMINISTIC", "0") == "1"
         self.fused_bwd_off = False
+        self.dgrad_bnsums_off = False
         self.debug = None
         self.prof = None
         self.prof_labels = None
@@ -528,6 +529,29 @@
         self._unpack(L.PACK_CONV_FPROP, dwp, G[r2.wkey], cout, cin, accumulate)
         return da1, parts
 
+    def _conv_backward_bnsums(self, r1: ConvRec, r2: ConvRec, dy2, G, accumulate):
+        src = r2.src
+        if src.c0 % 128 or self.dgrad_bnsums_off or self.debug is not None or src.c1 or src.bn0 is None or src.bn0 is not r1.bn or src.x0 is not r1.y \
+                or not src.bn0.relu or r1.bn.mean is None or r1.bn.invstd is None:
+            return None
+        lib = L.lib()
+        n, h, w, cin, cout = r2.n, r2.h, r2.w, src.c0, r2.cout
+        d = L.ConvDesc(self.dt, n, h, w, cout, 0, cin, 9, L.XF_NONE, L.XF_NONE, L.IN_PLAIN, L.OUT_PLAIN, 0, 0, 0, 0, 0, 0, 0)
+        if not lib.oct_conv_dgrad_bnsums_ok(C.byref(d)):
+            return None
+        dev = dy2.device
+        dwp = self._wgrad(src, dy2, cout, 9, n, h, w)
+        self._unpack(L.PACK_CONV_FPROP, dwp, G[r2.wkey], cout, cin, accumulate)
+        wp = self._pack(r2.wkey, self._P[r2.wkey], L.PACK_CONV_DGRAD, cout, cin)
+        da1 = self._act(n, h, w, cin, dev)
+        parts = torch.empty((lib.oct_conv_dgrad_bnsums_blocks(C.byref(d)), 2, cin), dtype=torch.float32, device=dev)
+        a = L.ConvDgradBnsumsArgs(L.ptr(dy2), L.ptr(wp), L.ptr(da1), L.ptr(r1.y), L.ptr(r1.bn.scale), L.ptr(r1.bn.shift),
+                                  L.ptr(r1.bn.mean), L.ptr(r1.bn.invstd), L.ptr(parts))
+        ev = self._prof_begin()
+        L.check(lib.oct_conv_dgrad_bnsums(C.byref(d), C.byref(a), _stream()), "oct_conv_dgrad_bnsums")
+        self._prof_end(ev, "igemm", (9, cout, cin, n, h, w, L.IN_PLAIN, L.OUT_PLAIN))
+        return da1, parts
+
     def _block_backward(self, name, da, dpool, G, accumulate, need_dx=True, partials=None):
         r1, r2 = self._ctx.convs[name]
         for r in (r1, r2):
@@ -538,7 +562,11 @@
         if fused is not None:
             da1, parts1 = fused
         else:
-            (da1, _), parts1 = self._conv_backward(r2, dy2, G, accumulate), None
+            sums = self._conv_backward_bnsums(r1, r2, dy2, G, accumulate)
+            if sums is not None:
+                da1, parts1 = sums
+            else:
+                (da1, _), parts1 = self._conv_backward(r2, dy2, G, accumulate), None
         first_fused = False
         if not need_dx and r1.src.c1 == 0 and r1.src.bn0 is None:
             qd = L.WgradDesc(self.dt, r1.n, r1.h, r1.w, r1.src.c0, 0, r1.cout, 9, L.XF_NONE, L.XF_NONE, L.IN_PLAIN)
```

New measurement: 1228 B-scans/s. No clear change (-0.1%).
